# dfm/george

Hardware: NVIDIA H100
Metric: gp.compute+log_likelihood N-points/sec (higher is better)
Workload: dtype f64

## Files before the change

george_b200/_lib.py:

```python

import ctypes as C
import os

import numpy as np

from ._spec import HodlrNodeInfo, HodlrOpts, KernelSpec

_HERE = os.path.dirname(os.path.abspath(__file__))
LIB_PATH = os.path.join(_HERE, "lib", "libbgp_b200.so")

BGP_OK, BGP_ERR_INVALID, BGP_ERR_DIM, BGP_ERR_NOT_COMPUTED, BGP_ERR_LINALG = 0, 1, 2, 3, 4
BGP_ERR_CUDA, BGP_ERR_NO_DEVICE, BGP_ERR_RANK_CAPACITY, BGP_ERR_INDEX, BGP_ERR_NOMEM = 5, 6, 7, 8, 9
BGP_PREDICT_VAR, BGP_PREDICT_COV = 0, 1
BGP_SAMPLE_DMMA_ROWS = 8


class BGPError(RuntimeError):
    """CUDA / device failure inside libbgp_b200 (there is no fallback path)."""


class RankCapacityError(BGPError):
    """The ACA rank of a node exceeded the configured per-level capacity."""


_lib = None

_p = C.c_void_p
_dp = C.POINTER(C.c_double)
_i64 = C.c_int64
_i32 = C.c_int32
_specp = C.POINTER(KernelSpec)

SIGNATURES = {
    "bgp_last_error": (C.c_char_p, []),
    "bgp_version": (C.c_int, []),
    "bgp_device_count": (C.c_int, []),
    "bgp_set_device": (C.c_int, [C.c_int]),
    "bgp_launch_count": (C.c_uint64, []),
    "bgp_spec_validate": (C.c_int, [_specp]),
    "bgp_spec_num_params": (C.c_int, [_specp, C.POINTER(C.c_int)]),
    "bgp_spec_paths": (C.c_int, [_specp, C.POINTER(_i32)]),
    "bgp_kmat_symmetric": (C.c_int, [_specp, _p, _i64, _p]),
    "bgp_kmat_general": (C.c_int, [_specp, _p, _i64, _p, _i64, _p]),
    "bgp_kmat_diagonal": (C.c_int, [_specp, _p, _p, _i64, _p]),
    "bgp_kmat_gradient_symmetric": (C.c_int, [_specp, _p, _p, _i64, _p]),
    "bgp_kmat_gradient_general": (C.c_int, [_specp, _p, _p, _i64, _p, _i64, _p]),
    "bgp_kmat_x1_gradient_general": (C.c_int, [_specp, _p, _i64, _p, _i64, _p]),
    "bgp_kmat_x2_gradient_general": (C.c_int, [_specp, _p, _i64, _p, _i64, _p]),
    "bgp_kmat_symmetric_dev": (C.c_int, [_specp, _p, _i64, _p, _p, _i64]),
    "bgp_kmat_general_dev": (C.c_int, [_specp, _p, _i64, _p, _i64, _p, _i64]),
    "bgp_kmat_matvec": (C.c_int, [_specp, _p, _i64, _p, _i64, _p, _p, _i64, _p]),
    "bgp_kmat_matvec_dev": (C.c_int, [_specp, _p, _i64, _p, _i64, _p, _p, _i64, _p]),
    "bgp_kmat_gradient_contract": (C.c_int, [_specp, _p, _p, _i64, _p, _p]),
    "bgp_kmat_x1_gradient_matvec": (C.c_int, [_specp, _p, _i64, _p, _i64, _p, _i64, C.c_double, _i32, _p]),
    "bgp_kmat_x1_gradient_matvec_dev": (C.c_int, [_specp, _p, _i64, _p, _i64, _p, _i64, C.c_double, _i32, _p]),
    "bgp_dense_grad_terms": (C.c_int, [_p, _p, _p, _p, _p, _p]),
    "bgp_hodlr_grad_terms": (C.c_int, [_p, _p, _p, _p, _p, _p]),
    "bgp_hodlr_grad_terms_local_dev": (C.c_int, [_p, _p, _p, _p, _p]),
    "bgp_dense_predict": (C.c_int, [_p, _specp, _p, _i64, _i32, _p]),
    "bgp_hodlr_predict": (C.c_int, [_p, _specp, _p, _i64, _i32, _p]),
    "bgp_dense_predict_grad": (C.c_int, [_p, _specp, _p, _i64, _p, _p]),
    "bgp_hodlr_predict_grad": (C.c_int, [_p, _specp, _p, _i64, _p, _p]),
    "bgp_hodlr_predict_local_dev": (C.c_int, [_p, _specp, _p, _i64, _i32, _p, _i64, _i32, _p]),
    "bgp_mvn_sample": (C.c_int, [_p, _i64, _p, _p, _i64, C.c_double, _p]),
    "bgp_dense_sample": (C.c_int, [_p, _specp, _p, _i64, _p, _p, _i64, C.c_double, _p]),
    "bgp_hodlr_sample": (C.c_int, [_p, _specp, _p, _i64, _p, _p, _i64, C.c_double, _p]),
    "bgp_sample_last_timing": (C.c_int, [_dp]),
    "bgp_dense_batch_create": (C.c_int, [C.POINTER(_p)]),
    "bgp_dense_batch_destroy": (None, [_p]),
    "bgp_dense_batch_log_likelihood": (C.c_int, [_p, _specp, _p, _i64, _i64, _p, _i64, _i32, _p, _p, _p, _p, _p]),
    "bgp_dense_batch_predict": (C.c_int, [_p, _specp, _p, _i64, _i64, _p, _i64, _i32, _p, _p, _p, _i64, _i32, _p, _p,
                                          _p]),
    "bgp_dense_batch_sample": (C.c_int, [_p, _specp, _p, _i64, _i64, _p, _i64, _i32, _p, _p, _p, _i64, _p, _p, _i64,
                                         C.c_double, _p, _p, _p]),
    "bgp_dense_batch_grad_terms": (C.c_int, [_p, _specp, _p, _i64, _i64, _p, _i64, _i32, _p, _p, _p, _p, _p, _p, _p,
                                             _p, _p]),
    "bgp_dense_create": (C.c_int, [C.POINTER(_p)]),
    "bgp_dense_destroy": (None, [_p]),
    "bgp_dense_compute": (C.c_int, [_p, _specp, _p, _i64, _i32, _p]),
    "bgp_dense_computed": (C.c_int, [_p]),
    "bgp_dense_log_determinant": (C.c_int, [_p, _dp]),
    "bgp_dense_apply_inverse": (C.c_int, [_p, _p, _i64, _i64]),
    "bgp_dense_dot_solve": (C.c_int, [_p, _p, _dp]),
    "bgp_dense_apply_sqrt": (C.c_int, [_p, _p, _i64, _p]),
    "bgp_dense_get_inverse": (C.c_int, [_p, _p]),
    "bgp_dense_export_factor": (C.c_int, [_p, _p]),
    "bgp_dense_import_factor": (C.c_int, [_p, _p, _i64, C.c_double]),
    "bgp_dense_last_timing": (C.c_int, [_p, _dp]),
    "bgp_hodlr_default_opts": (None, [C.POINTER(HodlrOpts)]),
    "bgp_hodlr_create": (C.c_int, [C.POINTER(_p)]),
    "bgp_hodlr_destroy": (None, [_p]),
    "bgp_hodlr_compute": (C.c_int, [_p, _specp, _p, _i64, _i32, _p, C.POINTER(HodlrOpts)]),
    "bgp_hodlr_compute_dev": (C.c_int, [_p, _specp, _p, _i64, _i32, _p, C.POINTER(HodlrOpts)]),
    "bgp_hodlr_computed": (C.c_int, [_p]),
    "bgp_hodlr_log_determinant": (C.c_int, [_p, _dp]),
    "bgp_hodlr_apply_inverse": (C.c_int, [_p, _p, _i64, _i64]),
    "bgp_hodlr_dot_solve": (C.c_int, [_p, _p, _dp]),
    "bgp_hodlr_dot_solve_dev": (C.c_int, [_p, _p, _dp]),
    "bgp_hodlr_get_inverse": (C.c_int, [_p, _p]),
    "bgp_hodlr_num_nodes": (C.c_int, [_p, C.POINTER(_i64)]),
    "bgp_hodlr_node_info": (C.c_int, [_p, C.POINTER(HodlrNodeInfo)]),
    "bgp_hodlr_node_pivots": (C.c_int, [_p, _i64, _p, _p]),
    "bgp_hodlr_node_factors": (C.c_int, [_p, _i64, _p]),
    "bgp_hodlr_last_draw_paths": (C.c_int, [_p, C.POINTER(C.c_uint64)]),
    "bgp_hodlr_last_eval_units": (C.c_int, [_p, C.POINTER(C.c_uint64)]),
    "bgp_hodlr_last_timing": (C.c_int, [_p, _dp]),
    "bgp_hodlr_last_grad_timing": (C.c_int, [_p, _dp]),
    "bgp_hodlr_last_work": (C.c_int, [_p, _dp]),
    "bgp_hodlr_set_profiling": (C.c_int, [_p, C.c_int]),
    "bgp_hodlr_last_aca_profile": (C.c_int, [_p, _dp]),
    "bgp_selftest_lu": (C.c_int, [_i32, _i32, _p, _p, _p]),
    "bgp_selftest_gemm": (C.c_int, [_i32, _i32, _i32, _i32, _i32, _p, _i64, _p, _i64, _p, _i64, _i32]),
    "bgp_hodlr_top_panel": (C.c_int, [_p, C.POINTER(_p), C.POINTER(_i64), C.POINTER(_i64), C.POINTER(_i64),
                                      C.POINTER(_i64)]),
    "bgp_hodlr_export_top": (C.c_int, [_p, _p, _i64]),
    "bgp_hodlr_import_top": (C.c_int, [_p, _p, _i64]),
    "bgp_hodlr_shard_rows": (C.c_int, [_p, _i32, C.POINTER(_i64), C.POINTER(_i64)]),
    "bgp_hodlr_finish_top": (C.c_int, [_p]),
    "bgp_comm_unique_id": (C.c_int, [_p, C.c_char_p]),
    "bgp_comm_init": (C.c_int, [_p, C.c_int, C.c_int, C.c_char_p]),
    "bgp_comm_destroy": (C.c_int, []),
    "bgp_comm_size": (C.c_int, []),
    "bgp_hodlr_solve_local_dev": (C.c_int, [_p, _p, _i64, _i64]),
    "bgp_hodlr_solve_top_dev": (C.c_int, [_p, _p, _i64, _i64]),
    "bgp_dev_alloc": (C.c_int, [C.POINTER(_p), C.c_size_t]),
    "bgp_dev_free": (C.c_int, [_p]),
    "bgp_dev_upload": (C.c_int, [_p, _p, C.c_size_t]),
    "bgp_dev_download": (C.c_int, [_p, _p, C.c_size_t]),
    "bgp_dev_synchronize": (C.c_int, []),
    "bgp_host_alloc_pinned": (C.c_int, [C.POINTER(_p), C.c_size_t]),
    "bgp_host_free_pinned": (C.c_int, [_p]),
}


def load():
    global _lib
    if _lib is not None:
        return _lib
    if not os.path.exists(LIB_PATH):
        raise ImportError(
            "george_b200: the CUDA library {0} is missing. Build it with "
            "`python -c 'import __graft_entry__ as g; g.build()'` (nvcc, sm_90a). "
            "There is no CPU fallback.".format(LIB_PATH))
    lib = C.CDLL(LIB_PATH)
    for name, (res, args) in SIGNATURES.items():
        fn = getattr(lib, name)
        fn.restype = res
        fn.argtypes = args
    _lib = lib
    return lib


def last_error():
    msg = load().bgp_last_error()
    return msg.decode("utf-8", "replace") if msg else ""


def check(status):
    if status == BGP_OK:
        return
    msg = last_error()
    if status == BGP_ERR_INVALID:
        raise ValueError(msg or "invalid kernel")
    if status in (BGP_ERR_DIM, BGP_ERR_NOT_COMPUTED):
        raise RuntimeError(msg or "dimension mismatch")
    if status == BGP_ERR_LINALG:
        raise np.linalg.LinAlgError(msg or "matrix is not positive definite")
    if status == BGP_ERR_INDEX:
        raise IndexError(msg)
    if status == BGP_ERR_NOMEM:
        raise MemoryError(msg)
    if status == BGP_ERR_RANK_CAPACITY:
        raise RankCapacityError(msg)
    raise BGPError("libbgp_b200 status {0}: {1}".format(status, msg))


def ptr(a):
    return C.c_void_p(a.ctypes.data)
```

george_b200/csrc/hodlr.cu:

```cuda
#include <algorithm>
#include <cmath>
#include <cstdlib>
#include <cstring>
#include <vector>

#include "common.cuh"
#include "hodlr_kernels.cuh"
#include "hodlr_lu.cuh"
#include "hodlr_aca2.cuh"
#include "hodlr_leaf.cuh"
#include "linalg.cuh"
#include "kernel_eval.cuh"

namespace bgp {
int upload_program(const DevProgram& P, DevBuf<DevProgram>& buf, cudaStream_t s);
int kmat_grad_contract_launch(const DevProgram* dprog, int nd, int np, const unsigned* which_dev, const double* x,
                              int64_t n, const double* M, int64_t ldm, const double* alpha, double ca, double cm,
                              double* g_dev, double* diag_dev, DevBuf<double>& scratch, cudaStream_t s);
int fill_identity_launch(double* A, int64_t n, cudaStream_t s);
int64_t grad_slab_partial_size(int64_t n, int64_t c, int np);
int64_t grad_slab_tile_size(int64_t n, int np);
int kmat_grad_slab_launch(const DevProgram* dprog, int nd, int np, const unsigned* which_dev, const double* x, int64_t n,
                          const double* W, int64_t j0, int64_t nc, int64_t jlo, int64_t jhi, const double* alpha,
                          double* partial, double* tile_part, double* diag_dev, cudaStream_t s);
int kmat_grad_slab_finish(int np, int64_t jlo, int64_t jhi, const double* tile_part, double* g_dev, cudaStream_t s);
int kmat_symmetric_launch_auto(const DevProgram& P, const DevProgram* dprog, const double* x, int64_t n,
                               const double* diag_add, double* out, int64_t ld, cudaStream_t s);
int kmat_general_launch_auto(const DevProgram& P, const DevProgram* dprog, const double* x1, int64_t n1, const double* x2,
                             int64_t n2, double* out, int64_t ld, cudaStream_t s);
int kmat_diagonal_launch(const DevProgram* dprog, const double* x1, const double* x2, int64_t n, double* out,
                         cudaStream_t s, int members = 1, int64_t ostride = 0);
int64_t predict_chunk_cols(int64_t n, int64_t multiple);
int64_t predict_var_partial_size(int64_t n, int64_t c);
int predict_var_launch(const double* B, int64_t ldb, const double* W, int64_t ldw, int64_t n, int64_t c,
                       const double* kdiag, double* var, DevBuf<double>& scratch, cudaStream_t s);
int kmat_x1_grad_matvec_launch(const DevProgram& P, const DevProgram* dprog, const double* x1, int64_t n1,
                               const double* x2, int64_t n2, const double* V, int64_t ldv, double scale, int add_prior,
                               double* out, DevBuf<double>& scratch, cudaStream_t s);
void predict_gemm_plan(int64_t m, int64_t nn, int64_t K, int64_t* nsplit_out, int64_t* klen_out);
int predict_gemm_sub(const double* A, int64_t lda, const double* B, int64_t ldb, int64_t m, int64_t nn, int64_t K,
                     bool lower, double* C, int64_t ldc, DevBuf<double>& slices, DevBuf<GemmDesc>& descs, cudaStream_t s);
bool comm_ready();
int comm_rank();
int comm_world();
int comm_allreduce_sum_f64(double* buf, size_t count, cudaStream_t s);
int comm_allgather_f64(const double* send, double* recv, size_t count, cudaStream_t s);
}
using namespace bgp;

struct HNode {
  int start, size, half, is_leaf, parent, dir, depth;
  int slot;
  int rank = 0, draws = 0, fallback = 0;
  int owned = 1;
  int top = 0;
};

struct PanelSet {
  DevBuf<double> V, U;
  int64_t ld = 0, row_off = 0;
  int vcols = 0, ucols = 0;
  double* vbase() const { return V.p - row_off; }
  double* ubase() const { return U.p - row_off; }
};

struct LevelInfo {
  std::vector<int> nodes;
  int set = 1;
  int cap = 0, max_cap = 0, vcol = 0, r = 0, ucol = 0;
  int max_half = 0, grow = 0;
  int desc_off = 0;
};

struct AcaGraphKey {
  A2Args a;
  int nn, ncc, nrc, shape, grid;
};

struct bgp_hodlr {
  cudaStream_t sA = nullptr, sB = nullptr;
  cudaEvent_t ev[8] = {nullptr};
  int64_t n = 0;
  int ndim = 0;
  bgp_hodlr_opts_t opts;
  bool computed = false;
  double log_det = 0.0;
  DevProgram prog;

  std::vector<HNode> nodes;
  std::vector<int> leaves;
  std::vector<LevelInfo> levels;
  std::vector<int> piv_off;
  std::vector<int> h_piv_rows, h_piv_cols;
  int max_leaf = 0, rtot = 0, vcols = 0, cut_depth = 0;
  int64_t row0 = 0, nloc = 0;
  std::vector<int64_t> shard_row0, shard_rows;
  bool top_pending = false;

  DevBuf<DevProgram> d_prog;
  DevBuf<double> d_x, d_yerr, d_diag, d_L, d_leaf_logdet, d_node_logdet, d_S, d_W, d_scalar, d_rhs;
  PanelSet top, loc;
  const PanelSet& pset(const LevelInfo& L) const { return L.set == 0 ? top : loc; }
  DevBuf<double> d_inv, d_gscratch;
  DevBuf<double> d_xsend, d_xrecv;
  DevBuf<unsigned> d_which;
  LuWorkspace lu_ws;
  DevBuf<GemmDesc> d_gram_desc, d_upd_desc;
  std::vector<NodeDesc> h_nodes;
  std::vector<int> cap_hint;
  int64_t cap_hint_n = -1;
  int cap_hint_min_size = -1;
  DevBuf<LeafDesc> d_leaves;
  DevBuf<AcaDesc> d_aca;
  DevBuf<AcaOut> d_aca_out;
  DevBuf<NodeDesc> d_nodes;
  DevBuf<PanelTile> d_ptiles;
  int small_limit = SS_MAX_N;
  bool leaf_cols_wide = false;
  DevBuf<int> d_idx, d_piv_rows, d_piv_cols, d_ticket, d_chain_done, d_ncols_by_depth;
  DevBuf<uint32_t> d_chain_state;
  DevBuf<A2Node> d_a2nodes;
  DevBuf<A2State> d_a2states;
  DevBuf<MT19937> d_a2rngs;
  DevBuf<A2EPart> d_epart;
  DevBuf<int> d_cand, d_cand_k, d_cand_words, d_cand_L, d_cand_next, d_cand_live, d_cchunk_node, d_rchunk_node, d_nactive;
  DevBuf<double> d_node_box;
  DevBuf<double2> d_cand_xu, d_gbox, d_cbox;
  DevBuf<unsigned long long> d_cmax, d_stats;
  DevBuf<int4> d_work;
  DevBuf<int> d_work_count, d_iter;
  AcaGraphKey aca_key;
  cudaGraph_t aca_graph = nullptr;
  cudaGraphExec_t aca_exec = nullptr;
  cudaStream_t sC = nullptr;
  bool profile = false;
  std::vector<cudaEvent_t> prof_events;
  double prof[12] = {0, 0, 0, 0, 0, 0, 0, 0, 0, 0, 0, 0};
  uint64_t draw_paths[4] = {0, 0, 0, 0};
  uint64_t eval_units[2] = {0, 0};
  DevBuf<double> d_vpart, d_upart, d_vmax;
  int aca_iters = 0;
  size_t w_cap = 0;

  double t_ms[5] = {0, 0, 0, 0, 0};
  double grad_t[4] = {0, 0, 0, 0};
  double work[6] = {0, 0, 0, 0, 0, 0};
};

static int ensure_streams(bgp_hodlr* h) {
  if (!h->sA) {
    BGP_CUDA(cudaStreamCreateWithFlags(&h->sA, cudaStreamNonBlocking));
    BGP_CUDA(cudaStreamCreateWithFlags(&h->sB, cudaStreamNonBlocking));
    for (int i = 0; i < 8; ++i) BGP_CUDA(cudaEventCreate(&h->ev[i]));
  }
  return BGP_OK;
}

static void build_tree(bgp_hodlr* h, int start, int size, int dir, int parent, int depth) {
  HNode nd;
  nd.start = start; nd.size = size; nd.half = size / 2; nd.dir = dir; nd.parent = parent; nd.depth = depth;
  nd.is_leaf = !(nd.half >= h->opts.min_size);
  nd.slot = 0;
  const int id = (int)h->nodes.size();
  h->nodes.push_back(nd);
  if (!nd.is_leaf) {
    build_tree(h, start, nd.half, 0, id, depth + 1);
    build_tree(h, start + nd.half, size - nd.half, 1, id, depth + 1);
  }
}

static int hodlr_solve_dev(bgp_hodlr* h, double* b, int64_t nrhs, int64_t ldb, cudaStream_t s, int part,
                           int64_t eye_row0 = -1);
static int hodlr_exchange_finish(bgp_hodlr* h);

static bool host_exchange(const bgp_hodlr* h) {
  return h->opts.shard_count > 1 &&
         !(comm_ready() && comm_world() == h->opts.shard_count && comm_rank() == h->opts.shard_rank);
}

static int reject_host_exchange(const bgp_hodlr* h, const char* what) {
  if (!host_exchange(h)) return BGP_OK;
  set_error("%s is not available on a host-exchange shard (shard %d of %d without a matching communicator): use "
            "bgp_hodlr_solve_local_dev / bgp_hodlr_solve_top_dev", what, h->opts.shard_rank, h->opts.shard_count);
  return BGP_ERR_INVALID;
}
static int hodlr_finish_top_impl(bgp_hodlr* h, bool allreduce);

constexpr size_t LS_SMEM_MAX = 200 * 1024;
constexpr int LS_MAX_LEAF = (int)(LS_SMEM_MAX / sizeof(double));

static bool leaf_solve_fits(int max_leaf, int cols) { return sizeof(double) * (size_t)max_leaf * cols <= LS_SMEM_MAX; }

static void set_sweep_func_attrs() {
  static std::atomic<uint64_t> done{0};
  int dev = 0;
  cudaGetDevice(&dev);
  const uint64_t bit = dev < 64 ? (1ull << dev) : 0;
  if (bit && (done.load(std::memory_order_relaxed) & bit)) return;
  cudaFuncSetAttribute(leaf_solve_kernel<1>, cudaFuncAttributeMaxDynamicSharedMemorySize, (int)LS_SMEM_MAX);
  cudaFuncSetAttribute(leaf_solve_kernel<2>, cudaFuncAttributeMaxDynamicSharedMemorySize, (int)LS_SMEM_MAX);
  cudaFuncSetAttribute(leaf_solve_kernel<4>, cudaFuncAttributeMaxDynamicSharedMemorySize, (int)LS_SMEM_MAX);
  cudaFuncSetAttribute(leaf_solve_kernel<LS_COLS>, cudaFuncAttributeMaxDynamicSharedMemorySize, (int)LS_SMEM_MAX);
  cudaFuncSetAttribute(leaf_solve_kernel<LS_COLS_WIDE>, cudaFuncAttributeMaxDynamicSharedMemorySize, (int)LS_SMEM_MAX);
  cudaFuncSetAttribute(small_solve_kernel, cudaFuncAttributeMaxDynamicSharedMemorySize, 160 * 1024);
  done.fetch_or(bit, std::memory_order_relaxed);
}

template <int COLS>
static int leaf_solve_launch(bgp_hodlr* h, double* X, int64_t ldx, const int* ncols_by_depth, int ncols_fixed,
                             int max_cols, cudaStream_t s, int l0, int l1) {
  const int ngroups = (max_cols + COLS - 1) / COLS;
  const dim3 grid((unsigned)((size_t)(l1 - l0) * (size_t)ngroups));
  const size_t smem = sizeof(double) * (size_t)h->max_leaf * COLS;
  leaf_solve_kernel<COLS><<<grid, LS_THREADS, smem, s>>>(h->d_leaves.p + l0, h->d_L.p, X, ldx, ncols_by_depth,
                                                         ncols_fixed, h->max_leaf, ngroups);
  BGP_LAUNCH_CHECK();
  return BGP_OK;
}

static int launch_leaf_solve(bgp_hodlr* h, double* X, int64_t ldx, const int* ncols_by_depth, int ncols_fixed,
                             int max_cols, cudaStream_t s, int l0 = 0, int l1 = -1) {
  if (l1 < 0) l1 = (int)h->leaves.size();
  const int nl = l1 - l0;
  if (nl <= 0 || max_cols == 0) return BGP_OK;
  const int m = h->max_leaf;
  if (h->leaf_cols_wide && max_cols > LS_COLS && leaf_solve_fits(m, LS_COLS_WIDE))
    return leaf_solve_launch<LS_COLS_WIDE>(h, X, ldx, ncols_by_depth, ncols_fixed, max_cols, s, l0, l1);
  int cols = max_cols <= 1 ? 1 : max_cols <= 2 ? 2 : max_cols <= 4 ? 4 : LS_COLS;
  while (cols > 1 && !leaf_solve_fits(m, cols)) cols /= 2;
  if (!leaf_solve_fits(m, cols)) {
    set_error("leaf size %d too large for the leaf solve kernel (at most %d rows)", m, LS_MAX_LEAF);
    return BGP_ERR_INVALID;
  }
  switch (cols) {
    case LS_COLS: return leaf_solve_launch<LS_COLS>(h, X, ldx, ncols_by_depth, ncols_fixed, max_cols, s, l0, l1);
    case 4: return leaf_solve_launch<4>(h, X, ldx, ncols_by_depth, ncols_fixed, max_cols, s, l0, l1);
    case 2: return leaf_solve_launch<2>(h, X, ldx, ncols_by_depth, ncols_fixed, max_cols, s, l0, l1);
    default: return leaf_solve_launch<1>(h, X, ldx, ncols_by_depth, ncols_fixed, max_cols, s, l0, l1);
  }
}

static int launch_level_big(bgp_hodlr* h, const LevelInfo& L, double* X, int64_t ldx, int ncolsW, int own_off, int factor,
                            int col_lo, int col_hi, cudaStream_t s, int b0, int b1);

static int launch_level(bgp_hodlr* h, const LevelInfo& L, double* X, int64_t ldx, int ncolsW, int own_off, int factor,
                        int col_lo, int col_hi, cudaStream_t s, int b0 = 0, int b1 = -1) {
  if (b1 < 0) b1 = (int)L.nodes.size();
  const int nn = b1 - b0;
  if (nn <= 0 || L.r == 0) {
    return BGP_OK;
  }
  const int r = L.r;
  const int64_t stride = (int64_t)2 * r * ncolsW;
  const size_t need = (size_t)nn * stride;
  if (need > h->w_cap) { set_error("internal: W workspace too small (%zu > %zu)", need, h->w_cap); return BGP_ERR_CUDA; }
  BGP_CUDA(cudaMemsetAsync(h->d_W.p, 0, sizeof(double) * need, s));
  if (2 * r > h->small_limit) return launch_level_big(h, L, X, ldx, ncolsW, own_off, factor, col_lo, col_hi, s, b0, b1);
  const NodeDesc* nd = h->d_nodes.p + L.desc_off + b0;
  const int max_nh = L.max_half + 1;
  if (r <= GTS_MAX_R) {
    dim3 grid((max_nh + GTS_ROWS - 1) / GTS_ROWS, nn * 2, (ncolsW + GTS_TC - 1) / GTS_TC);
    const double* vb = h->pset(L).vbase();
    const int64_t ldv = h->pset(L).ld;
    if (r <= 2) gram_tn_small_kernel<2><<<grid, GTS_THREADS, 0, s>>>(nd, vb, ldv, X, ldx, ncolsW, h->d_W.p, stride);
    else if (r <= 4) gram_tn_small_kernel<4><<<grid, GTS_THREADS, 0, s>>>(nd, vb, ldv, X, ldx, ncolsW, h->d_W.p, stride);
    else gram_tn_small_kernel<GTS_MAX_R><<<grid, GTS_THREADS, 0, s>>>(nd, vb, ldv, X, ldx, ncolsW, h->d_W.p, stride);
    BGP_LAUNCH_CHECK();
  } else {
    dim3 grid((max_nh + GT_CHUNK - 1) / GT_CHUNK, nn * 2, (ncolsW + GT_TC - 1) / GT_TC);
    gram_tn_kernel<<<grid, GT_THREADS, 0, s>>>(nd, h->pset(L).vbase(), h->pset(L).ld, X, ldx, ncolsW, h->d_W.p, stride);
    BGP_LAUNCH_CHECK();
  }
  {
    const size_t sbytes = sizeof(double) * (size_t)(2 * r) * (2 * r);
    small_solve_kernel<<<nn, SS_THREADS, sbytes, s>>>(nd, h->d_W.p, stride, ncolsW, own_off, factor, h->d_S.p,
                                                      h->d_node_logdet.p, L.desc_off + b0);
    BGP_LAUNCH_CHECK();
  }
  if (col_hi > col_lo) {
    dim3 grid((max_nh + UP_ROWS - 1) / UP_ROWS, nn * 2, (col_hi - col_lo + UP_TC - 1) / UP_TC);
    update_nn_kernel<<<grid, UP_THREADS, 0, s>>>(nd, h->pset(L).ubase(), h->pset(L).ld, X, ldx, col_lo, col_hi, h->d_W.p, stride, 0);
    BGP_LAUNCH_CHECK();
  }
  return BGP_OK;
}

static int launch_level_big(bgp_hodlr* h, const LevelInfo& L, double* X, int64_t ldx, int ncolsW, int own_off, int factor,
                            int col_lo, int col_hi, cudaStream_t s, int b0, int b1) {
  const int nn = b1 - b0;
  const int r = L.r, n2 = 2 * r;
  const int64_t stride = (int64_t)n2 * ncolsW;
  const int64_t ldv = h->pset(L).ld, ldu = h->pset(L).ld;
  double* W = h->d_W.p;
  constexpr int KCHUNK = 4096;
  std::vector<LuNode> lun(nn);
  std::vector<GemmDesc> gram, upd;
  int max_nh = 0;
  for (int k = 0; k < nn; ++k) {
    const int b = b0 + k;
    const HNode& nd = h->nodes[L.nodes[b]];
    const int64_t s_off = h->h_nodes[L.desc_off + b].s_off;
    lun[k].S = h->d_S.p + s_off;
    lun[k].piv = reinterpret_cast<int*>(lun[k].S + (int64_t)n2 * n2);
    lun[k].logdet = h->d_node_logdet.p + L.desc_off + b;
    double* Wn = W + (int64_t)k * stride;
    for (int hh = 0; hh < 2; ++hh) {
      const int rs = nd.start + (hh ? nd.half : 0), nh = hh ? (nd.size - nd.half) : nd.half;
      max_nh = std::max(max_nh, nh);
      for (int k0 = 0; k0 < nh; k0 += KCHUNK) {
        GemmDesc g;
        g.A = h->pset(L).vbase() + (int64_t)L.vcol * ldv + rs + k0; g.lda = ldv;
        g.B = X + rs + k0; g.ldb = ldx;
        g.C = Wn + (hh ? 0 : r); g.ldc = n2;
        g.M = r; g.N = ncolsW; g.K = std::min(KCHUNK, nh - k0); g.mode = GD_ATOMIC_ADD;
        gram.push_back(g);
      }
      if (col_hi > col_lo) {
        GemmDesc g;
        g.A = h->pset(L).ubase() + (int64_t)L.ucol * ldu + rs; g.lda = ldu;
        g.B = Wn + (hh ? r : 0) + (int64_t)col_lo * n2; g.ldb = n2;
        g.C = X + rs + (int64_t)col_lo * ldx; g.ldc = ldx;
        g.M = nh; g.N = col_hi - col_lo; g.K = r; g.mode = GD_SUB;
        upd.push_back(g);
      }
    }
  }
  BGP_TRY(lu_upload(h->d_gram_desc, gram, s));
  BGP_TRY((gemm_dmma_launch<true, true>(h->d_gram_desc.p, (int)gram.size(), r, ncolsW, nullptr, s)));
  if (factor) {
    BGP_TRY(lu_upload(h->lu_ws.d_nodes, lun, s));
    dim3 grid((unsigned)std::min<int64_t>(((int64_t)n2 * n2 + 255) / 256, 4096), nn);
    lu_assemble_kernel<<<grid, 256, 0, s>>>(h->lu_ws.d_nodes.p, W, stride, r, own_off);
    BGP_LAUNCH_CHECK();
    BGP_TRY(lu_factor_batch(h->lu_ws, lun, n2, s));
    if (col_hi > col_lo)
      BGP_TRY(lu_solve_batch(h->lu_ws, lun, n2, W + (int64_t)col_lo * n2, stride, n2, col_hi - col_lo, false, s));
  } else {
    BGP_TRY(lu_solve_batch(h->lu_ws, lun, n2, W, stride, n2, ncolsW, true, s));
  }
  if (!upd.empty()) {
    BGP_TRY(lu_upload(h->d_upd_desc, upd, s));
    BGP_TRY((gemm_dmma_launch<false, true>(h->d_upd_desc.p, (int)upd.size(), max_nh, col_hi - col_lo, nullptr, s)));
  }
  return BGP_OK;
}

static int run_aca2(bgp_hodlr* h, const std::vector<AcaDesc>& descs, std::vector<AcaOut>& houts, cudaStream_t s) {
  const int nn = (int)descs.size();
  if (nn == 0) return BGP_OK;
  std::vector<A2Node> hn(nn);
  std::vector<int> cchunk_node, rchunk_node;
  int64_t cand_total = 0, top_cand_total = 0;
  (void)top_cand_total;
  const bool dist_top = false;
  int capmax = 1;
  for (int i = 0; i < nn; ++i) {
    const AcaDesc& d = descs[i];
    A2Node& a = hn[i];
    a.row0 = d.row0; a.n_rows = d.n_rows; a.col0 = d.col0; a.n_cols = d.n_cols;
    a.vcol = d.vcol; a.cap = d.cap; a.pre_id = d.pre_id; a.node = d.node;
    {
      const PanelSet& ps = h->pset(h->levels[h->nodes[d.pre_id].depth]);
      a.ld = ps.ld;
      a.vbase = ps.vbase() + (int64_t)d.vcol * ps.ld;
    }
    a.idx_off = d.idx_off; a.piv_off = d.piv_off;
    a.cchunk0 = (int)cchunk_node.size(); a.n_cchunks = (d.n_cols + A2_CHUNK - 1) / A2_CHUNK;
    a.rchunk0 = (int)rchunk_node.size(); a.n_rchunks = (d.n_rows + A2_CHUNK - 1) / A2_CHUNK;
    for (int c = 0; c < a.n_cchunks; ++c) cchunk_node.push_back(i);
    for (int c = 0; c < a.n_rchunks; ++c) rchunk_node.push_back(i);
    a.bmax = std::min(A2_BMAX, d.n_rows);
    a.cand_off = cand_total; cand_total += a.bmax;
    a.is_top = (dist_top && h->nodes[d.pre_id].top) ? 1 : 0;
    if (a.is_top) top_cand_total = cand_total;
    capmax = std::max(capmax, d.cap);
  }
  const int ncc = (int)cchunk_node.size(), nrc = (int)rchunk_node.size();
  BGP_TRY(h->d_a2nodes.reserve(nn, s));
  BGP_TRY(h->d_a2states.reserve(nn, s));
  BGP_TRY(h->d_a2rngs.reserve((size_t)2 * nn, s));
  BGP_TRY(h->d_cand.reserve((size_t)cand_total, s));
  BGP_TRY(h->d_cand_k.reserve((size_t)cand_total, s));
  BGP_TRY(h->d_cand_words.reserve((size_t)cand_total, s));
  BGP_TRY(h->d_cand_L.reserve((size_t)cand_total, s));
  BGP_TRY(h->d_cand_next.reserve((size_t)cand_total, s));
  BGP_TRY(h->d_cand_live.reserve((size_t)cand_total, s));
  BGP_TRY(h->d_node_box.reserve((size_t)2 * nn, s));
  BGP_TRY(h->d_cmax.reserve((size_t)cand_total, s));
  BGP_TRY(h->d_epart.reserve((size_t)std::max(ncc, 1) * A2_NSUB, s));
  BGP_TRY(h->d_cchunk_node.reserve(ncc, s));
  BGP_TRY(h->d_rchunk_node.reserve(nrc, s));
  BGP_TRY(h->d_vpart.reserve((size_t)ncc * A2_NSUB * (capmax + 1), s));
  BGP_TRY(h->d_upart.reserve((size_t)nrc * A2_NSUB * (capmax + 1), s));
  const bool cull = shape_has_bound(h->prog.shape) && !getenv("BGP_NO_CULL");
  if (cull) {
    BGP_TRY(h->d_vmax.reserve((size_t)ncc * A2_NGROUP, s));
    BGP_TRY(h->d_cand_xu.reserve((size_t)cand_total, s));
    BGP_TRY(h->d_gbox.reserve((size_t)ncc * A2_NGROUP, s));
    BGP_TRY(h->d_cbox.reserve((size_t)ncc, s));
  }
  BGP_TRY(h->d_nactive.reserve(2, s));
  int n_top = 0;
  for (int i = 0; i < nn; ++i) n_top += hn[i].is_top;
  BGP_TRY(h->d_stats.reserve(A2_NSTATS, s));
  int64_t work_cap = 0;
  for (int i = 0; i < nn; ++i) {
    const int big = (hn[i].bmax + A2_CG * A2_ITEM_CB - 1) / (A2_CG * A2_ITEM_CB);
    const int small = (std::min(hn[i].bmax, 256) + A2_CG - 1) / A2_CG;
    work_cap += (int64_t)hn[i].n_cchunks * std::max(big, small);
  }
  BGP_TRY(h->d_work.reserve((size_t)(2 * work_cap), s));
  BGP_TRY(h->d_work_count.reserve(4, s));
  BGP_TRY(h->d_iter.reserve(1, s));
  BGP_CUDA(cudaMemsetAsync(h->d_iter.p, 0, sizeof(int), s));
  BGP_CUDA(cudaMemsetAsync(h->d_work_count.p, 0, sizeof(int) * 4, s));
  BGP_CUDA(cudaMemsetAsync(h->d_stats.p, 0, sizeof(unsigned long long) * A2_NSTATS, s));
  BGP_CUDA(cudaMemcpyAsync(h->d_a2nodes.p, hn.data(), sizeof(A2Node) * nn, cudaMemcpyHostToDevice, s));
  BGP_CUDA(cudaMemcpyAsync(h->d_cchunk_node.p, cchunk_node.data(), sizeof(int) * ncc, cudaMemcpyHostToDevice, s));
  BGP_CUDA(cudaMemcpyAsync(h->d_rchunk_node.p, rchunk_node.data(), sizeof(int) * nrc, cudaMemcpyHostToDevice, s));
  BGP_CUDA(cudaMemcpyAsync(h->d_nactive.p, &nn, sizeof(int), cudaMemcpyHostToDevice, s));
  A2Args a;
  memset(&a, 0, sizeof(a));
  a.prog = h->d_prog.p; a.x = h->d_x.p; a.nodes = h->d_a2nodes.p; a.states = h->d_a2states.p; a.rngs = h->d_a2rngs.p; a.n_nodes = nn;
  a.tol = h->opts.tol; a.seed = (uint32_t)h->opts.seed; a.exhaust_mode = h->opts.exhaust_mode;
  a.idx_ws = h->d_idx.p; a.piv_rows = h->d_piv_rows.p; a.piv_cols = h->d_piv_cols.p;
  a.cand = h->d_cand.p; a.cand_k = h->d_cand_k.p; a.cand_words = h->d_cand_words.p; a.cmax = h->d_cmax.p; a.epart = h->d_epart.p;
  a.cchunk_node = h->d_cchunk_node.p; a.rchunk_node = h->d_rchunk_node.p; a.vpart = h->d_vpart.p; a.upart = h->d_upart.p;
  a.vmax = cull ? h->d_vmax.p : nullptr;
  a.cand_xu = cull ? h->d_cand_xu.p : nullptr;
  a.gbox = cull ? h->d_gbox.p : nullptr;
  a.cbox = cull ? h->d_cbox.p : nullptr;
  a.cand_L = h->d_cand_L.p; a.cand_next = h->d_cand_next.p; a.cand_live = h->d_cand_live.p; a.node_box = h->d_node_box.p;
  a.capmax = capmax; a.n_active = h->d_nactive.p; a.stats = h->d_stats.p;
  a.work = h->d_work.p; a.work_count = h->d_work_count.p; a.work_cursor = h->d_work_count.p + 2; a.work_cap = (int)work_cap; a.iter_ptr = h->d_iter.p;
  a.shard_rank = dist_top ? h->opts.shard_rank : 0; a.shard_count = dist_top ? h->opts.shard_count : 1;
  if (dist_top) BGP_CUDA(cudaMemcpyAsync(h->d_nactive.p + 1, &n_top, sizeof(int), cudaMemcpyHostToDevice, s));
  cudaFuncSetAttribute(a2_init_kernel, cudaFuncAttributeMaxDynamicSharedMemorySize, (int)sizeof(A2NodeSmem));
    cudaFuncSetAttribute(a2_decide_kernel, cudaFuncAttributeMaxDynamicSharedMemorySize, (int)sizeof(A2NodeSmem));
    cudaFuncSetAttribute(a2_finish_kernel, cudaFuncAttributeMaxDynamicSharedMemorySize, (int)sizeof(A2NodeSmem));
  a2_init_kernel<<<nn, A2_NODE_THREADS, sizeof(A2NodeSmem), s>>>(a);
  BGP_LAUNCH_CHECK();
  int active = nn, iters = 0;
  int eval_minb = A2_EVAL_MINB_DEFAULT;
  if (const char* e = getenv("BGP_EVAL_MINB")) eval_minb = atoi(e) == 3 ? 3 : 2;
  const int eval_grid = num_sms() * 6;
  auto launch_iteration = [&](cudaStream_t st, cudaGraphConditionalHandle hnd, int use_hnd, int it_prof) -> int {
    auto mark = [&](int slot) -> int {
      if (it_prof < 0) return BGP_OK;
      const size_t need = (size_t)7 * (it_prof + 1);
      while (h->prof_events.size() < need) {
        cudaEvent_t e;
        BGP_CUDA(cudaEventCreate(&e));
        h->prof_events.push_back(e);
      }
      BGP_CUDA(cudaEventRecord(h->prof_events[(size_t)7 * it_prof + slot], st));
      return BGP_OK;
    };
    BGP_TRY(mark(0));
    a2_eval_launch(h->prog.shape, dim3(eval_grid), st, a, eval_minb);
    BGP_LAUNCH_CHECK();
    BGP_TRY(mark(1));
    a2_decide_kernel<<<nn, A2_NODE_THREADS, sizeof(A2NodeSmem), st>>>(a);
    BGP_LAUNCH_CHECK();
    BGP_TRY(mark(2));
    a2_vrow_launch(h->prog.shape, dim3(ncc, A2_NSUB), st, a);
    BGP_LAUNCH_CHECK();
    BGP_TRY(mark(3));
    a2_pivot_kernel<<<nn, 32, 0, st>>>(a);
    BGP_LAUNCH_CHECK();
    BGP_TRY(mark(4));
    a2_vnorm_ucol_launch(h->prog.shape, dim3(ncc + nrc, A2_NSUB), st, a, ncc);
    BGP_LAUNCH_CHECK();
    BGP_TRY(mark(5));
    a2_finish_kernel<<<nn, A2_NODE_THREADS, sizeof(A2NodeSmem), st>>>(a);
    BGP_LAUNCH_CHECK();
    BGP_TRY(mark(6));
    a2_tick_kernel<<<1, 1, 0, st>>>(a.iter_ptr, a.n_active, hnd, use_hnd);
    BGP_LAUNCH_CHECK();
    return BGP_OK;
  };
  const bool use_graph = !h->profile && !getenv("BGP_NO_GRAPH");
  if (use_graph) {
    AcaGraphKey key;
    memset(&key, 0, sizeof(key));
    key.a = a; key.nn = nn; key.ncc = ncc; key.nrc = nrc; key.shape = h->prog.shape; key.grid = eval_grid * 4 + eval_minb;
    if (!h->aca_exec || memcmp(&key, &h->aca_key, sizeof(key)) != 0) {
      if (h->aca_exec) { cudaGraphExecDestroy(h->aca_exec); h->aca_exec = nullptr; }
      if (h->aca_graph) { cudaGraphDestroy(h->aca_graph); h->aca_graph = nullptr; }
      BGP_CUDA(cudaGraphCreate(&h->aca_graph, 0));
      cudaGraphConditionalHandle hnd;
      BGP_CUDA(cudaGraphConditionalHandleCreate(&hnd, h->aca_graph, 1, cudaGraphCondAssignDefault));
      cudaGraphNodeParams cp = {};
      cp.type = cudaGraphNodeTypeConditional;
      cp.conditional.handle = hnd;
      cp.conditional.type = cudaGraphCondTypeWhile;
      cp.conditional.size = 1;
      cudaGraphNode_t wnode;
      BGP_CUDA(cudaGraphAddNode(&wnode, h->aca_graph, nullptr, 0, &cp));
      cudaGraph_t body = cp.conditional.phGraph_out[0];
      if (!h->sC) BGP_CUDA(cudaStreamCreateWithFlags(&h->sC, cudaStreamNonBlocking));
      BGP_CUDA(cudaStreamBeginCaptureToGraph(h->sC, body, nullptr, nullptr, 0, cudaStreamCaptureModeRelaxed));
      const int rc = launch_iteration(h->sC, hnd, 1, -1);
      cudaGraph_t captured = nullptr;
      const cudaError_t ce = cudaStreamEndCapture(h->sC, &captured);
      if (rc != BGP_OK) return rc;
      if (ce != cudaSuccess) { set_error("ACA graph capture failed: %s", cudaGetErrorString(ce)); return BGP_ERR_CUDA; }
      BGP_CUDA(cudaGraphInstantiate(&h->aca_exec, h->aca_graph, 0));
      h->aca_key = key;
    }
    BGP_CUDA(cudaGraphLaunch(h->aca_exec, s));
    int it_host = 0, act2[2] = {0, 0};
    BGP_CUDA(cudaMemcpyAsync(&it_host, h->d_iter.p, sizeof(int), cudaMemcpyDeviceToHost, s));
    BGP_CUDA(cudaMemcpyAsync(act2, h->d_nactive.p, sizeof(int) * 2, cudaMemcpyDeviceToHost, s));
    BGP_CUDA(cudaStreamSynchronize(s));
    iters = it_host;
    g_launches.fetch_add((uint64_t)7 * (uint64_t)std::max(iters - 1, 0), std::memory_order_relaxed);
    if (act2[0] > 0) { set_error("ACA did not terminate"); return BGP_ERR_CUDA; }
  } else {
    while (active > 0) {
      for (int rep = 0; rep < 8; ++rep) {
        BGP_TRY(launch_iteration(s, 0, 0, h->profile ? iters : -1));
        iters++;
      }
      int act2[2] = {0, 0};
      BGP_CUDA(cudaMemcpyAsync(act2, h->d_nactive.p, sizeof(int) * 2, cudaMemcpyDeviceToHost, s));
      BGP_CUDA(cudaStreamSynchronize(s));
      active = act2[0];
      if (iters > (1 << 22)) { set_error("ACA did not terminate"); return BGP_ERR_CUDA; }
    }
  }
  h->aca_iters = iters;
  {
    unsigned long long st4[A2_NSTATS] = {0};
    BGP_CUDA(cudaMemcpyAsync(st4, h->d_stats.p, sizeof(st4), cudaMemcpyDeviceToHost, s));
    BGP_CUDA(cudaStreamSynchronize(s));
    for (int k = 0; k < 4; ++k) h->draw_paths[k] = st4[A2_PATH_REDO + k];
    h->eval_units[0] = st4[A2_UNITS_PULLED]; h->eval_units[1] = st4[A2_UNITS_LIVE];
    h->prof[1] = iters; h->prof[2] = (double)st4[0]; h->prof[3] = (double)st4[1]; h->prof[4] = (double)st4[2];
    h->prof[5] = (double)st4[3];
    if (h->profile) {
      double tot[6] = {0, 0, 0, 0, 0, 0};
      for (int i = 0; i < iters; ++i)
        for (int k = 0; k < 6; ++k) {
          float ms = 0;
          cudaEventElapsedTime(&ms, h->prof_events[(size_t)7 * i + k], h->prof_events[(size_t)7 * i + k + 1]);
          tot[k] += ms;
        }
      h->prof[0] = tot[0];
      for (int k = 0; k < 6; ++k) h->prof[6 + k] = tot[k];
    }
  }
  if (h->opts.exhaust_mode == BGP_EXHAUST_DENSE) {
    a2_dense_fill_kernel<<<dim3(nn, 64), 256, 0, s>>>(a);
    BGP_LAUNCH_CHECK();
    a2_dense_rank_kernel<<<(nn + 127) / 128, 128, 0, s>>>(a);
    BGP_LAUNCH_CHECK();
  }
  std::vector<A2State> hs(nn);
  BGP_CUDA(cudaMemcpyAsync(hs.data(), h->d_a2states.p, sizeof(A2State) * nn, cudaMemcpyDeviceToHost, s));
  BGP_CUDA(cudaStreamSynchronize(s));
  for (int i = 0; i < nn; ++i) {
    AcaOut o;
    o.rank = hs[i].rank; o.draws = hs[i].draws; o.fallback = hs[i].fallback; o.status = hs[i].status;
    houts[descs[i].node] = o;
  }
  return BGP_OK;
}

static int hodlr_compute_dev_impl(bgp_hodlr* h, const bgp_kernel_spec_t* spec, const double* x_dev, int64_t n,
                                  int32_t ndim, const double* yerr_dev, const bgp_hodlr_opts_t* opts_in) {
  h->computed = false;
  h->top_pending = false;
  for (uint64_t& c : h->draw_paths) c = 0;
  for (uint64_t& c : h->eval_units) c = 0;
  h->shard_row0.clear(); h->shard_rows.clear();
  BGP_TRY(require_device());
  BGP_TRY(ensure_streams(h));
  BGP_TRY(build_dev_program(spec, &h->prog));
  if (h->prog.ndim != ndim) { set_error("dimension mismatch: kernel ndim %d, input ndim %d", h->prog.ndim, ndim); return BGP_ERR_DIM; }
  if (ndim > ACA_MAX_NDIM) { set_error("HODLR supports at most %d input dimensions", ACA_MAX_NDIM); return BGP_ERR_INVALID; }
  if (n <= 0 || n > (int64_t)0x7fffffff) { set_error("invalid number of points %lld", (long long)n); return BGP_ERR_INVALID; }
  bgp_hodlr_opts_t o;
  if (opts_in) o = *opts_in; else bgp_hodlr_default_opts(&o);
  if (o.min_size < 1) { set_error("min_size must be >= 1"); return BGP_ERR_INVALID; }
  if (o.shard_count < 1) o.shard_count = 1;
  if (o.shard_count & (o.shard_count - 1)) { set_error("shard_count must be a power of two"); return BGP_ERR_INVALID; }
  if (o.shard_rank < 0 || o.shard_rank >= o.shard_count) { set_error("invalid shard_rank"); return BGP_ERR_INVALID; }
  if (o.shard_count > 1 && o.rng_mode == BGP_RNG_REFERENCE) { set_error("rng_mode=reference serialises the tree and cannot be sharded"); return BGP_ERR_INVALID; }
  h->opts = o;
  h->n = n;
  h->ndim = ndim;
  cudaStream_t sA = h->sA, sB = h->sB;
  set_sweep_func_attrs();
  h->small_limit = SS_MAX_N;
  if (const char* e = getenv("BGP_SMALL_RANK_LIMIT")) h->small_limit = std::min(SS_MAX_N, atoi(e));
  h->leaf_cols_wide = false;
  if (const char* e = getenv("BGP_LEAF_COLS")) h->leaf_cols_wide = atoi(e) > LS_COLS;

  h->nodes.clear(); h->leaves.clear(); h->levels.clear();
  h->nodes.reserve(2 * (size_t)(n / std::max(1, o.min_size)) + 8);
  build_tree(h, 0, (int)n, 0, -1, 0);
  int cut = 0;
  while ((1 << cut) < o.shard_count) cut++;
  h->cut_depth = cut;
  int max_depth = 0;
  for (auto& nd : h->nodes) max_depth = std::max(max_depth, nd.depth);
  h->row0 = 0; h->nloc = n;
  if (o.shard_count > 1) {
    int seen = 0; bool found = false;
    for (size_t i = 0; i < h->nodes.size(); ++i) {
      HNode& nd = h->nodes[i];
      if (nd.depth == cut) {
        if (seen == o.shard_rank) { h->row0 = nd.start; h->nloc = nd.size; found = true; }
        h->shard_row0.push_back(nd.start); h->shard_rows.push_back(nd.size);
        seen++;
      }
    }
    if (!found || seen != o.shard_count) {
      h->shard_row0.clear(); h->shard_rows.clear();
      set_error("tree too shallow to shard %d ways (N=%lld, min_size=%d)", o.shard_count, (long long)n, o.min_size);
      return BGP_ERR_INVALID;
    }
    for (auto& nd : h->nodes) {
      nd.top = nd.depth < cut;
      nd.owned = !nd.top && nd.start >= h->row0 && nd.start + nd.size <= h->row0 + h->nloc;
    }
  }
  h->levels.assign(max_depth + 1, LevelInfo());
  for (size_t i = 0; i < h->nodes.size(); ++i) {
    HNode& nd = h->nodes[i];
    if (nd.is_leaf) { if (nd.owned) { nd.slot = (int)h->leaves.size(); h->leaves.push_back((int)i); } continue; }
    if (!(nd.owned || nd.top)) continue;
    LevelInfo& L = h->levels[nd.depth];
    nd.slot = (int)L.nodes.size();
    L.nodes.push_back((int)i);
    L.max_half = std::max(L.max_half, nd.size - nd.half);
  }
  while (!h->levels.empty() && h->levels.back().nodes.empty()) h->levels.pop_back();
  const int nlev = (int)h->levels.size();
  for (int l = 0; l < nlev; ++l) h->levels[l].set = (o.shard_count > 1 && l < cut) ? 0 : 1;
  h->top.ld = n; h->top.row_off = 0;
  h->loc.ld = h->nloc; h->loc.row_off = h->row0;

  const int rcap0 = o.rank_capacity > 0 ? o.rank_capacity : 128;
  for (auto& L : h->levels) {
    int mh = 0;
    for (int id : L.nodes) mh = std::max(mh, h->nodes[id].half);
    L.max_cap = std::max(1, mh);
    L.cap = std::min(rcap0, L.max_cap);
  }
  if (o.rank_capacity <= 0 && h->cap_hint_n == n && h->cap_hint_min_size == o.min_size && (int)h->cap_hint.size() == nlev)
    for (int l = 0; l < nlev; ++l) h->levels[l].cap = std::min(h->levels[l].max_cap, std::max(h->levels[l].cap, h->cap_hint[l]));

  BGP_TRY(upload_program(h->prog, h->d_prog, sA));
  BGP_TRY(h->d_x.reserve((size_t)n * ndim, sA));
  BGP_TRY(h->d_diag.reserve((size_t)n, sA));
  if (x_dev != h->d_x.p) BGP_CUDA(cudaMemcpyAsync(h->d_x.p, x_dev, sizeof(double) * n * ndim, cudaMemcpyDeviceToDevice, sA));
  square_kernel<<<(unsigned)std::min<int64_t>((n + 255) / 256, 1184), 256, 0, sA>>>(yerr_dev, h->d_diag.p, n);
  BGP_LAUNCH_CHECK();
  BGP_CUDA(cudaEventRecord(h->ev[0], sA));

  const int nl = (int)h->leaves.size();
  std::vector<LeafDesc> hleaves(nl);
  int64_t loff = 0;
  h->max_leaf = 0;
  for (int i = 0; i < nl; ++i) {
    const HNode& nd = h->nodes[h->leaves[i]];
    hleaves[i].start = nd.start; hleaves[i].size = nd.size; hleaves[i].depth = nd.depth; hleaves[i]._pad = 0;
    hleaves[i].off = loff;
    loff += (int64_t)nd.size * nd.size;
    h->max_leaf = std::max(h->max_leaf, nd.size);
  }
  if (h->max_leaf > LS_MAX_LEAF) {
    set_error("leaf size %d too large: the leaf solve handles at most %d rows (N=%lld, min_size=%d); lower min_size",
              h->max_leaf, LS_MAX_LEAF, (long long)n, o.min_size);
    return BGP_ERR_INVALID;
  }
  BGP_TRY(h->d_leaves.reserve(std::max(nl, 1), sA));
  BGP_TRY(h->d_L.reserve((size_t)std::max<int64_t>(loff, 1), sA));
  BGP_TRY(h->d_leaf_logdet.reserve(std::max(nl, 1), sA));
  if (nl) {
    BGP_CUDA(cudaMemcpyAsync(h->d_leaves.p, hleaves.data(), sizeof(LeafDesc) * nl, cudaMemcpyHostToDevice, sA));
    const char* lf_env = getenv("BGP_LEAF_FACTOR");
    const bool generic = lf_env && strcmp(lf_env, "generic") == 0;
    if (h->max_leaf <= LF_MAX_LEAF && !generic) {
      leaf_factor_launch(h->prog.shape, nl, h->max_leaf, sA, h->d_prog.p, h->d_x.p, h->d_diag.p, h->d_leaves.p, h->d_L.p,
                         h->d_leaf_logdet.p);
    } else {
      leaf_build_factor_kernel<<<nl, LEAF_THREADS, 0, sA>>>(h->d_prog.p, h->d_x.p, h->d_diag.p, h->d_leaves.p, h->d_L.p,
                                                            h->d_leaf_logdet.p);
    }
    BGP_LAUNCH_CHECK();
  }
  BGP_CUDA(cudaEventRecord(h->ev[1], sA));

  std::vector<AcaDesc> hdesc;
  std::vector<int> desc_node;
  std::vector<AcaOut> houts;
  int64_t idx_total = 0, piv_total = 0;
  int nint = 0;
  BGP_CUDA(cudaStreamWaitEvent(sB, h->ev[1], 0));
  for (int attempt = 0;; ++attempt) {
// ... 239 lines not shown
}

template <class StartSize>
static void rows_meeting(int count, const StartSize& start_size, int64_t lo, int64_t hi, int* first, int* last) {
  int a = 0, b = count;
  while (a < b) {
    const int m = (a + b) / 2;
    int st, sz;
    start_size(m, &st, &sz);
    if ((int64_t)st + sz <= lo) a = m + 1; else b = m;
  }
  *first = a;
  b = count;
  while (a < b) {
    const int m = (a + b) / 2;
    int st, sz;
    start_size(m, &st, &sz);
    if (st < hi) a = m + 1; else b = m;
  }
  *last = a;
}

static bool rows_ordered(const bgp_hodlr* h) {
  auto ordered = [&](const std::vector<int>& ids) {
    for (size_t k = 1; k < ids.size(); ++k) {
      const HNode& a = h->nodes[ids[k - 1]];
      if (a.start + a.size > h->nodes[ids[k]].start) return false;
    }
    return true;
  };
  if (!ordered(h->leaves)) return false;
  for (const LevelInfo& L : h->levels)
    if (!ordered(L.nodes)) return false;
  return true;
}

static int hodlr_solve_dev(bgp_hodlr* h, double* b, int64_t nrhs, int64_t ldb, cudaStream_t s, int part,
                           int64_t eye_row0) {
  const int nlev = (int)h->levels.size();
  const int cut = h->opts.shard_count > 1 ? h->cut_depth : 0;
  const bool native_x = part == 0 && h->opts.shard_count > 1 && !host_exchange(h);
  if (eye_row0 >= 0 && part != 0) {
    set_error("internal: a row-restricted solve runs every part of the solve");
    return BGP_ERR_INVALID;
  }
  for (int64_t c0 = 0; c0 < nrhs; c0 += 64) {
    const int nc = (int)std::min<int64_t>(64, nrhs - c0);
    double* X = b + c0 * ldb;
    if (eye_row0 >= 0) {
      const int64_t lo = std::max(eye_row0 + c0, h->row0), hi = std::min(eye_row0 + c0 + nc, h->row0 + h->nloc);
      if (lo >= hi) continue;
      int l0, l1;
      rows_meeting((int)h->leaves.size(), [&](int k, int* st, int* sz) {
        const HNode& nd = h->nodes[h->leaves[k]]; *st = nd.start; *sz = nd.size; }, lo, hi, &l0, &l1);
      BGP_TRY(launch_leaf_solve(h, X, ldb, nullptr, nc, nc, s, l0, l1));
      for (int l = nlev - 1; l >= 0; --l) {
        const LevelInfo& L = h->levels[l];
        int b0, b1;
        rows_meeting((int)L.nodes.size(), [&](int k, int* st, int* sz) {
          const HNode& nd = h->nodes[L.nodes[k]]; *st = nd.start; *sz = nd.size; }, lo, hi, &b0, &b1);
        BGP_TRY(launch_level(h, L, X, ldb, nc, 0, 0, 0, nc, s, b0, b1));
      }
      continue;
    }
    if (part != 2) {
      BGP_TRY(launch_leaf_solve(h, X, ldb, nullptr, nc, nc, s));
      for (int l = nlev - 1; l >= cut; --l) BGP_TRY(launch_level(h, h->levels[l], X, ldb, nc, 0, 0, 0, nc, s));
    }
    if (native_x) BGP_TRY(exchange_rows(h, X, ldb, nc, s));
    if (part != 1) {
      for (int l = std::min(cut, nlev) - 1; l >= 0; --l) BGP_TRY(launch_level(h, h->levels[l], X, ldb, nc, 0, 0, 0, nc, s));
    }
  }
  return BGP_OK;
}

static int64_t top_cols(const bgp_hodlr_t* h) {
  const int cut = std::min<int>(h->cut_depth, (int)h->levels.size());
  (void)cut;
  return h->top.ucols;
}

static int hodlr_finish_top_impl(bgp_hodlr* h, bool allreduce) {
  cudaStream_t s = h->sA;
  const int nlev = (int)h->levels.size();
  const int cut = std::min(h->cut_depth, nlev);
  for (int l = cut - 1; l >= 0; --l) {
    const LevelInfo& L = h->levels[l];
    BGP_TRY(launch_level(h, L, h->top.U.p, h->n, L.ucol + L.r, L.ucol, 1, 0, L.ucol, s));
  }
  const int nl = (int)h->leaves.size();
  int ndesc = 0;
  for (auto& L : h->levels) ndesc += (int)L.nodes.size();
  std::vector<double> ld_leaf(nl), ld_node(ndesc);
  if (nl) BGP_CUDA(cudaMemcpyAsync(ld_leaf.data(), h->d_leaf_logdet.p, sizeof(double) * nl, cudaMemcpyDeviceToHost, s));
  if (ndesc) BGP_CUDA(cudaMemcpyAsync(ld_node.data(), h->d_node_logdet.p, sizeof(double) * ndesc, cudaMemcpyDeviceToHost, s));
  BGP_CUDA(cudaStreamSynchronize(s));
  double ld = 0.0;
  for (double v : ld_leaf) ld += v;
  for (int l = 0; l < nlev; ++l) {
    const LevelInfo& L = h->levels[l];
    if (l < cut && h->opts.shard_rank != 0) continue;
    for (size_t i = 0; i < L.nodes.size(); ++i) ld += ld_node[L.desc_off + i];
  }
  if (allreduce) {
    BGP_CUDA(cudaMemcpyAsync(h->d_scalar.p, &ld, sizeof(double), cudaMemcpyHostToDevice, s));
    BGP_TRY(comm_allreduce_sum_f64(h->d_scalar.p, 1, s));
    BGP_CUDA(cudaMemcpyAsync(&ld, h->d_scalar.p, sizeof(double), cudaMemcpyDeviceToHost, s));
    BGP_CUDA(cudaStreamSynchronize(s));
  }
  h->log_det = ld;
  h->computed = true;
  return BGP_OK;
}

static int hodlr_exchange_finish(bgp_hodlr* h) {
  BGP_TRY(exchange_rows(h, h->top.U.p, h->n, top_cols(h), h->sA));
  BGP_TRY(hodlr_finish_top_impl(h, true));
  float ms = 0;
  cudaEventElapsedTime(&ms, h->ev[0], h->ev[1]); h->t_ms[0] = ms;
  cudaEventElapsedTime(&ms, h->ev[0], h->ev[2]); h->t_ms[1] = ms;
  cudaEventElapsedTime(&ms, h->ev[6], h->ev[3]); h->t_ms[2] = ms;
  cudaEventElapsedTime(&ms, h->ev[0], h->ev[3]); h->t_ms[3] = ms;
  return BGP_OK;
}

extern "C" {

void bgp_hodlr_default_opts(bgp_hodlr_opts_t* o) {
  o->min_size = 100; o->seed = 42; o->tol = 0.1;
  o->rng_mode = BGP_RNG_REFERENCE;
  o->rank_capacity = 0; o->shard_rank = 0; o->shard_count = 1; o->exhaust_mode = BGP_EXHAUST_DENSE;
}

int bgp_hodlr_create(bgp_hodlr_t** out) {
  *out = new (std::nothrow) bgp_hodlr();
  if (!*out) { set_error("out of host memory"); return BGP_ERR_NOMEM; }
  bgp_hodlr_default_opts(&(*out)->opts);
  return BGP_OK;
}

void bgp_hodlr_destroy(bgp_hodlr_t* h) {
  if (!h) return;
  if (h->sA) {
    cudaStreamSynchronize(h->sA); cudaStreamSynchronize(h->sB);
  }
  h->d_prog.release(); h->d_x.release(); h->d_yerr.release(); h->d_diag.release(); h->d_L.release();
  h->d_leaf_logdet.release(); h->d_node_logdet.release(); h->top.V.release(); h->top.U.release(); h->loc.V.release(); h->loc.U.release(); h->d_S.release();
  h->d_W.release(); h->d_scalar.release(); h->d_rhs.release(); h->d_leaves.release(); h->d_aca.release();
  h->d_aca_out.release(); h->d_nodes.release(); h->d_ptiles.release(); h->d_idx.release(); h->d_piv_rows.release(); h->d_piv_cols.release();
  h->lu_ws.d_nodes.release(); h->lu_ws.d_trsm.release(); h->lu_ws.d_gemm.release(); h->d_gram_desc.release(); h->d_upd_desc.release();
  h->d_ticket.release(); h->d_chain_done.release(); h->d_ncols_by_depth.release(); h->d_chain_state.release();
  h->d_a2nodes.release(); h->d_a2states.release(); h->d_a2rngs.release(); h->d_epart.release(); h->d_cand.release(); h->d_cand_k.release();
  h->d_cand_words.release(); h->d_cand_L.release(); h->d_cand_next.release(); h->d_cand_live.release(); h->d_node_box.release(); h->d_cand_xu.release(); h->d_gbox.release(); h->d_cbox.release(); h->d_cchunk_node.release(); h->d_rchunk_node.release(); h->d_nactive.release();
  h->d_inv.release(); h->d_gscratch.release(); h->d_which.release(); h->d_xsend.release(); h->d_xrecv.release();
  h->d_vpart.release(); h->d_upart.release(); h->d_vmax.release(); h->d_cmax.release(); h->d_stats.release(); h->d_work.release(); h->d_work_count.release();
  for (cudaEvent_t e : h->prof_events) cudaEventDestroy(e);
  h->d_iter.release();
  if (h->aca_exec) cudaGraphExecDestroy(h->aca_exec);
  if (h->aca_graph) cudaGraphDestroy(h->aca_graph);
  if (h->sC) cudaStreamDestroy(h->sC);
  if (h->sA) {
    cudaStreamSynchronize(h->sA); cudaStreamSynchronize(h->sB);
    for (int i = 0; i < 8; ++i) cudaEventDestroy(h->ev[i]);
    cudaStreamDestroy(h->sA); cudaStreamDestroy(h->sB);
  }
  delete h;
}

int bgp_hodlr_compute_dev(bgp_hodlr_t* h, const bgp_kernel_spec_t* spec, const double* x_dev, int64_t n, int32_t ndim,
                          const double* yerr_dev, const bgp_hodlr_opts_t* opts) {
  if (!h) { set_error("null handle"); return BGP_ERR_INVALID; }
  return hodlr_compute_dev_impl(h, spec, x_dev, n, ndim, yerr_dev, opts);
}

int bgp_hodlr_compute(bgp_hodlr_t* h, const bgp_kernel_spec_t* spec, const double* x, int64_t n, int32_t ndim,
                      const double* yerr, const bgp_hodlr_opts_t* opts) {
  if (!h) { set_error("null handle"); return BGP_ERR_INVALID; }
  h->computed = false;
  h->top_pending = false;
  h->shard_row0.clear(); h->shard_rows.clear();
  BGP_TRY(require_device());
  BGP_TRY(ensure_streams(h));
  if (n <= 0 || ndim <= 0) { set_error("invalid input shape (%lld, %d)", (long long)n, ndim); return BGP_ERR_INVALID; }
  BGP_TRY(h->d_x.reserve((size_t)n * ndim, h->sA));
  BGP_TRY(h->d_yerr.reserve((size_t)n, h->sA));
  BGP_CUDA(cudaMemcpyAsync(h->d_x.p, x, sizeof(double) * n * ndim, cudaMemcpyHostToDevice, h->sA));
  BGP_CUDA(cudaMemcpyAsync(h->d_yerr.p, yerr, sizeof(double) * n, cudaMemcpyHostToDevice, h->sA));
  return hodlr_compute_dev_impl(h, spec, h->d_x.p, n, ndim, h->d_yerr.p, opts);
}

int bgp_hodlr_computed(const bgp_hodlr_t* h) { return h && h->computed ? 1 : 0; }

int bgp_hodlr_log_determinant(const bgp_hodlr_t* h, double* out) {
  if (!h || !h->computed) { set_error("the solver has not been computed"); return BGP_ERR_NOT_COMPUTED; }
  *out = h->log_det;
  return BGP_OK;
}

int bgp_hodlr_apply_inverse(bgp_hodlr_t* h, double* b, int64_t nrhs, int64_t ldb) {
  if (!h || !h->computed) { set_error("the solver has not been computed"); return BGP_ERR_NOT_COMPUTED; }
  BGP_TRY(reject_host_exchange(h, "apply_inverse"));
  if (nrhs <= 0) return BGP_OK;
  if (ldb < h->n) { set_error("dimension mismatch: ldb < n"); return BGP_ERR_DIM; }
  cudaStream_t s = h->sA;
  const int64_t n = h->n;
  const int64_t slab = std::max<int64_t>(1, std::min<int64_t>(nrhs, (int64_t)(1ull << 28) / n));
  BGP_TRY(h->d_rhs.reserve((size_t)n * slab, s));
  for (int64_t c0 = 0; c0 < nrhs; c0 += slab) {
    const int64_t nc = std::min(slab, nrhs - c0);
    BGP_CUDA(cudaMemcpy2DAsync(h->d_rhs.p, sizeof(double) * n, b + c0 * ldb, sizeof(double) * ldb, sizeof(double) * n, nc, cudaMemcpyHostToDevice, s));
    BGP_CUDA(cudaEventRecord(h->ev[4], s));
    BGP_TRY(hodlr_solve_dev(h, h->d_rhs.p, nc, n, s, 0));
    BGP_CUDA(cudaEventRecord(h->ev[5], s));
    BGP_CUDA(cudaMemcpy2DAsync(b + c0 * ldb, sizeof(double) * ldb, h->d_rhs.p, sizeof(double) * n, sizeof(double) * n, nc, cudaMemcpyDeviceToHost, s));
    BGP_CUDA(cudaStreamSynchronize(s));
  }
  float ms = 0; cudaEventElapsedTime(&ms, h->ev[4], h->ev[5]); h->t_ms[4] = ms;
  return BGP_OK;
}

int bgp_hodlr_dot_solve_dev(bgp_hodlr_t* h, const double* y_dev, double* out) {
  if (!h || !h->computed) { set_error("the solver has not been computed"); return BGP_ERR_NOT_COMPUTED; }
  BGP_TRY(reject_host_exchange(h, "dot_solve"));
  cudaStream_t s = h->sA;
  const int64_t n = h->n;
  BGP_TRY(h->d_rhs.reserve((size_t)n, s));
  BGP_CUDA(cudaEventRecord(h->ev[4], s));
  BGP_CUDA(cudaMemcpyAsync(h->d_rhs.p, y_dev, sizeof(double) * n, cudaMemcpyDeviceToDevice, s));
  BGP_TRY(hodlr_solve_dev(h, h->d_rhs.p, 1, n, s, 0));
  BGP_CUDA(cudaMemsetAsync(h->d_scalar.p, 0, sizeof(double), s));
  dot_kernel<<<(unsigned)std::min<int64_t>((n + 255) / 256, 592), 256, 0, s>>>(y_dev, h->d_rhs.p, n, h->d_scalar.p);
  BGP_LAUNCH_CHECK();
  BGP_CUDA(cudaEventRecord(h->ev[5], s));
  BGP_CUDA(cudaMemcpyAsync(out, h->d_scalar.p, sizeof(double), cudaMemcpyDeviceToHost, s));
  BGP_CUDA(cudaStreamSynchronize(s));
  float ms = 0; cudaEventElapsedTime(&ms, h->ev[4], h->ev[5]); h->t_ms[4] = ms;
  return BGP_OK;
}

int bgp_hodlr_dot_solve(bgp_hodlr_t* h, const double* y, double* out) {
  if (!h || !h->computed) { set_error("the solver has not been computed"); return BGP_ERR_NOT_COMPUTED; }
  BGP_TRY(reject_host_exchange(h, "dot_solve"));
  cudaStream_t s = h->sA;
  BGP_TRY(h->d_yerr.reserve((size_t)h->n, s));
  BGP_CUDA(cudaMemcpyAsync(h->d_yerr.p, y, sizeof(double) * h->n, cudaMemcpyHostToDevice, s));
  return bgp_hodlr_dot_solve_dev(h, h->d_yerr.p, out);
}

int bgp_hodlr_get_inverse(bgp_hodlr_t* h, double* out) {
  if (!h || !h->computed) { set_error("the solver has not been computed"); return BGP_ERR_NOT_COMPUTED; }
  BGP_TRY(reject_host_exchange(h, "get_inverse"));
  const int64_t n = h->n;
  for (int64_t j = 0; j < n; ++j) {
    double* c = out + j * n;
    memset(c, 0, sizeof(double) * n);
    c[j] = 1.0;
  }
  return bgp_hodlr_apply_inverse(h, out, n, n);
}

__global__ void eye_slab_kernel(double* __restrict__ W, int64_t n, int64_t j0, int64_t nc, int64_t jlo, int64_t jhi) {
  for (int64_t k = (int64_t)blockIdx.x * blockDim.x + threadIdx.x; k < nc; k += (int64_t)gridDim.x * blockDim.x)
    if (j0 + k >= jlo && j0 + k < jhi) W[k * n + j0 + k] = 1.0;
}

constexpr int64_t GRAD_RESIDENT_MAX = (int64_t)1 << 32;
constexpr int64_t GRAD_SLAB_BUDGET = (int64_t)1 << 27;

static int64_t grad_slab_cols(int64_t n, bool* forced) {
  int64_t c = std::max<int64_t>(64, (GRAD_SLAB_BUDGET / std::max<int64_t>(n, 1)) / 64 * 64);
  *forced = false;
  if (const char* e = getenv("BGP_GRAD_CHUNK")) {
    const long v = atol(e);
    if (v >= 1) { c = (v + 63) / 64 * 64; *forced = true; }
  }
  return std::min(c, (n + 63) / 64 * 64);
}

static float event_ms(cudaEvent_t a, cudaEvent_t b) {
  float ms = 0;
  cudaEventElapsedTime(&ms, a, b);
  return ms;
}

static int grad_stream_own_columns(bgp_hodlr* h, int np, const double* alpha, int64_t c, double* dg, double* ddiag,
                                   double* t_solve, double* t_contract) {
  cudaStream_t s = h->sA;
  const int64_t n = h->n, jlo = h->row0, jhi = h->row0 + h->nloc;
  const bool prof = h->profile;
  const int64_t tsize = grad_slab_tile_size(n, np), psize = grad_slab_partial_size(n, c, np);
  BGP_TRY(h->d_inv.reserve((size_t)n * c, s));
  BGP_TRY(h->d_gscratch.reserve((size_t)(tsize + psize), s));
  double* W = h->d_inv.p;
  double* tile_part = h->d_gscratch.p;
  double* partial = h->d_gscratch.p + tsize;
  int64_t slabs = 0;
  for (int64_t j0 = jlo / 64 * 64; j0 < jhi; j0 += c, ++slabs) {
    const int64_t nc = std::min(c, jhi - j0);
    if (prof) BGP_CUDA(cudaEventRecord(h->ev[4], s));
    BGP_CUDA(cudaMemsetAsync(W, 0, sizeof(double) * n * nc, s));
    eye_slab_kernel<<<(unsigned)std::min<int64_t>((nc + 255) / 256, 1184), 256, 0, s>>>(W, n, j0, nc, jlo, jhi);
    BGP_LAUNCH_CHECK();
    BGP_TRY(hodlr_solve_dev(h, W, nc, n, s, 0, j0));
    if (prof) BGP_CUDA(cudaEventRecord(h->ev[5], s));
    BGP_TRY(kmat_grad_slab_launch(h->d_prog.p, h->ndim, np, h->d_which.p, h->d_x.p, n, W, j0, nc, jlo, jhi, alpha,
                                  partial, tile_part, ddiag, s));
    if (prof) {
      BGP_CUDA(cudaEventRecord(h->ev[7], s));
// ... 276 lines not shown
    for (int64_t j0 = 0; j0 < ns; j0 += c) {
      const int64_t nc = std::min(c, ns - j0);
      BGP_CUDA(cudaMemcpyAsync(dxs.p, xs + j0 * nd, sizeof(double) * nc * nd, cudaMemcpyHostToDevice, s));
      BGP_TRY(kmat_general_launch_auto(P, dprog.p, dxs.p, nc, h->d_x.p, n, dB.p, n, s));
      BGP_CUDA(cudaMemcpyAsync(dW.p, dB.p, sizeof(double) * n * nc, cudaMemcpyDeviceToDevice, s));
      BGP_TRY(hodlr_solve_dev(h, dW.p, nc, n, s, 0));
      BGP_TRY(kmat_diagonal_launch(dprog.p, dxs.p, dxs.p, nc, dkd.p, s));
      BGP_TRY(predict_var_launch(dB.p, n, dW.p, n, n, nc, dkd.p, dvar.p, scratch, s));
      BGP_CUDA(cudaMemcpyAsync(out + j0, dvar.p, sizeof(double) * nc, cudaMemcpyDeviceToHost, s));
    }
  } else {
    BGP_TRY(hodlr_predict_cov_dev(h, P, xs, ns, dC));
    BGP_CUDA(cudaMemcpyAsync(out, dC.p, sizeof(double) * ns * ns, cudaMemcpyDeviceToHost, s));
  }
  BGP_CUDA(cudaStreamSynchronize(s));
  return BGP_OK;
}

int bgp_hodlr_predict_grad(bgp_hodlr_t* h, const bgp_kernel_spec_t* spec, const double* xs, int64_t ns, double* var,
                           double* dvar) {
  if (!h || !h->computed) { set_error("the solver has not been computed"); return BGP_ERR_NOT_COMPUTED; }
  if (host_exchange(h) || h->opts.shard_count > 1) { set_error("predict_grad is not available on a sharded factorisation"); return BGP_ERR_INVALID; }
  if (ns < 0) { set_error("negative number of test points"); return BGP_ERR_INVALID; }
  DevProgram P;
  BGP_TRY(build_dev_program(spec, &P));
  if (P.ndim != h->ndim) { set_error("dimension mismatch: kernel ndim %d, input ndim %d", P.ndim, h->ndim); return BGP_ERR_DIM; }
  if (P.ndim > BGP_MAX_DIM) { set_error("input-coordinate gradients support at most %d dimensions (got %d)", BGP_MAX_DIM, P.ndim); return BGP_ERR_INVALID; }
  if (ns == 0) return BGP_OK;
  const int64_t n = h->n;
  const int nd = h->ndim;
  cudaStream_t s = h->sA;
  DevBuf<DevProgram> dprog;
  DevBuf<double> dxs, dB, dW, dkd, dvar_c, ddvar, scratch;
  BGP_TRY(upload_program(P, dprog, s));
  const int64_t c = std::min(ns, predict_chunk_cols(n, 64));
  BGP_TRY(dW.alloc((size_t)n * c, s));
  BGP_TRY(dxs.alloc((size_t)c * nd, s));
  BGP_TRY(dB.alloc((size_t)n * c, s));
  BGP_TRY(dkd.alloc((size_t)c, s));
  BGP_TRY(dvar_c.alloc((size_t)c, s));
  BGP_TRY(ddvar.alloc((size_t)c * nd, s));
  for (int64_t j0 = 0; j0 < ns; j0 += c) {
    const int64_t nc = std::min(c, ns - j0);
    BGP_CUDA(cudaMemcpyAsync(dxs.p, xs + j0 * nd, sizeof(double) * nc * nd, cudaMemcpyHostToDevice, s));
    BGP_TRY(kmat_general_launch_auto(P, dprog.p, dxs.p, nc, h->d_x.p, n, dB.p, n, s));
    BGP_CUDA(cudaMemcpyAsync(dW.p, dB.p, sizeof(double) * n * nc, cudaMemcpyDeviceToDevice, s));
    BGP_TRY(hodlr_solve_dev(h, dW.p, nc, n, s, 0));
    BGP_TRY(kmat_diagonal_launch(dprog.p, dxs.p, dxs.p, nc, dkd.p, s));
    BGP_TRY(predict_var_launch(dB.p, n, dW.p, n, n, nc, dkd.p, dvar_c.p, scratch, s));
    BGP_CUDA(cudaMemcpyAsync(var + j0, dvar_c.p, sizeof(double) * nc, cudaMemcpyDeviceToHost, s));
    BGP_TRY(kmat_x1_grad_matvec_launch(P, dprog.p, dxs.p, nc, h->d_x.p, n, dW.p, n, -2.0, 1, ddvar.p, scratch, s));
    BGP_CUDA(cudaMemcpyAsync(dvar + j0 * nd, ddvar.p, sizeof(double) * nc * nd, cudaMemcpyDeviceToHost, s));
  }
  BGP_CUDA(cudaStreamSynchronize(s));
  return BGP_OK;
}

int bgp_hodlr_sample(bgp_hodlr_t* h, const bgp_kernel_spec_t* spec, const double* xs, int64_t ns, const double* mean,
                     const double* z, int64_t size, double jitter, double* out) {
  if (!h || !h->computed) { set_error("the solver has not been computed"); return BGP_ERR_NOT_COMPUTED; }
  if (h->opts.shard_count > 1) { set_error("sample is not available on a sharded factorisation"); return BGP_ERR_INVALID; }
  BGP_TRY(mvn_sample_check(ns, size, jitter));
  DevProgram P;
  BGP_TRY(build_dev_program(spec, &P));
  if (P.ndim != h->ndim) { set_error("dimension mismatch: kernel ndim %d, input ndim %d", P.ndim, h->ndim); return BGP_ERR_DIM; }
  if (ns == 0 || size == 0) return BGP_OK;
  DevBuf<double> dC;
  BGP_TRY(sample_mark(0, h->sA));
  BGP_TRY(hodlr_predict_cov_dev(h, P, xs, ns, dC));
  return mvn_draw_host_io(dC.p, ns, mean, z, size, jitter, out, h->sA);
}

int bgp_hodlr_num_nodes(const bgp_hodlr_t* h, int64_t* out) {
  if (!h) { set_error("null handle"); return BGP_ERR_INVALID; }
  *out = (int64_t)h->nodes.size();
  return BGP_OK;
}

int bgp_hodlr_node_info(const bgp_hodlr_t* h, bgp_hodlr_node_info_t* out) {
  if (!h) { set_error("null handle"); return BGP_ERR_INVALID; }
  for (size_t i = 0; i < h->nodes.size(); ++i) {
    const HNode& nd = h->nodes[i];
    out[i].start = nd.start; out[i].size = nd.size; out[i].half = nd.half; out[i].is_leaf = nd.is_leaf;
    out[i].parent = nd.parent; out[i].direction = nd.dir; out[i].depth = nd.depth; out[i].rank = nd.rank;
    out[i].rng_draws = nd.draws; out[i].dense_fallback = nd.fallback;
  }
  return BGP_OK;
}

int bgp_hodlr_node_pivots(const bgp_hodlr_t* hc, int64_t node, int32_t* rows, int32_t* cols) {
  bgp_hodlr_t* h = const_cast<bgp_hodlr_t*>(hc);
  if (!h || node < 0 || node >= (int64_t)h->nodes.size()) { set_error("node index out of range"); return BGP_ERR_INDEX; }
  const HNode& nd = h->nodes[node];
  if (nd.is_leaf || h->piv_off[node] < 0 || nd.rank == 0 ||
      (nd.fallback && h->opts.exhaust_mode == BGP_EXHAUST_DENSE))
    return BGP_OK;
  BGP_CUDA(cudaMemcpy(rows, h->d_piv_rows.p + h->piv_off[node], sizeof(int) * nd.rank, cudaMemcpyDeviceToHost));
  BGP_CUDA(cudaMemcpy(cols, h->d_piv_cols.p + h->piv_off[node], sizeof(int) * nd.rank, cudaMemcpyDeviceToHost));
  return BGP_OK;
}

int bgp_hodlr_node_factors(const bgp_hodlr_t* h, int64_t node, double* out) {
  if (!h) { set_error("null handle"); return BGP_ERR_INVALID; }
  if (!h->computed) { set_error("the solver has not been computed"); return BGP_ERR_NOT_COMPUTED; }
  if (h->opts.shard_count > 1) { set_error("node factors are not available on a sharded factorisation"); return BGP_ERR_INVALID; }
  if (node < 0 || node >= (int64_t)h->nodes.size() || h->nodes[node].is_leaf) {
    set_error("node %lld is not an internal node", (long long)node);
    return BGP_ERR_INDEX;
  }
  const HNode& nd = h->nodes[node];
  if (nd.rank == 0) return BGP_OK;
  const LevelInfo& L = h->levels[nd.depth];
  const PanelSet& ps = h->pset(L);
  const double* src = ps.vbase() + (int64_t)L.vcol * ps.ld + nd.start;
  BGP_CUDA(cudaMemcpy2D(out, sizeof(double) * nd.size, src, sizeof(double) * ps.ld, sizeof(double) * nd.size, nd.rank,
                        cudaMemcpyDeviceToHost));
  return BGP_OK;
}

int bgp_hodlr_last_draw_paths(const bgp_hodlr_t* h, uint64_t* out4) {
  if (!h) { set_error("null handle"); return BGP_ERR_INVALID; }
  if (!h->computed) { set_error("the solver has not been computed"); return BGP_ERR_NOT_COMPUTED; }
  for (int i = 0; i < 4; ++i) out4[i] = h->draw_paths[i];
  return BGP_OK;
}

int bgp_hodlr_last_eval_units(const bgp_hodlr_t* h, uint64_t* out2) {
  if (!h) { set_error("null handle"); return BGP_ERR_INVALID; }
  if (!h->computed) { set_error("the solver has not been computed"); return BGP_ERR_NOT_COMPUTED; }
  for (int i = 0; i < 2; ++i) out2[i] = h->eval_units[i];
  return BGP_OK;
}

int bgp_hodlr_last_timing(const bgp_hodlr_t* h, double* ms5) {
  if (!h) { set_error("null handle"); return BGP_ERR_INVALID; }
  for (int i = 0; i < 5; ++i) ms5[i] = h->t_ms[i];
  return BGP_OK;
}
int bgp_hodlr_last_grad_timing(const bgp_hodlr_t* h, double* out4) {
  if (!h) { set_error("null handle"); return BGP_ERR_INVALID; }
  for (int i = 0; i < 4; ++i) out4[i] = h->grad_t[i];
  return BGP_OK;
}
int bgp_hodlr_set_profiling(bgp_hodlr_t* h, int on) {
  if (!h) { set_error("null handle"); return BGP_ERR_INVALID; }
  h->profile = on != 0;
  return BGP_OK;
}
int bgp_hodlr_last_aca_profile(const bgp_hodlr_t* h, double* p12) {
  if (!h) { set_error("null handle"); return BGP_ERR_INVALID; }
  for (int i = 0; i < 12; ++i) p12[i] = h->prof[i];
  return BGP_OK;
}
int bgp_hodlr_last_work(const bgp_hodlr_t* h, double* w6) {
  if (!h) { set_error("null handle"); return BGP_ERR_INVALID; }
  for (int i = 0; i < 6; ++i) w6[i] = h->work[i];
  return BGP_OK;
}

int bgp_selftest_lu(int32_t n, int32_t nrhs, const double* S_host, double* R_host, double* logdet) {
  BGP_TRY(require_device());
  if (n <= 0 || nrhs < 0) { set_error("bgp_selftest_lu: bad sizes"); return BGP_ERR_INVALID; }
  cudaStream_t s = 0;
  DevBuf<double> dS, dR, dld;
  LuWorkspace ws;
  BGP_TRY(dS.alloc((size_t)n * n + n, s));
  BGP_TRY(dR.alloc(std::max<size_t>((size_t)n * nrhs, 1), s));
  BGP_TRY(dld.alloc(1, s));
  BGP_CUDA(cudaMemcpyAsync(dS.p, S_host, sizeof(double) * n * n, cudaMemcpyHostToDevice, s));
  if (nrhs) BGP_CUDA(cudaMemcpyAsync(dR.p, R_host, sizeof(double) * n * nrhs, cudaMemcpyHostToDevice, s));
  std::vector<LuNode> nodes(1);
  nodes[0].S = dS.p; nodes[0].piv = reinterpret_cast<int*>(dS.p + (size_t)n * n); nodes[0].logdet = dld.p;
  BGP_TRY(lu_factor_batch(ws, nodes, n, s));
  BGP_TRY(lu_solve_batch(ws, nodes, n, dR.p, 0, n, nrhs, false, s));
  if (nrhs) BGP_CUDA(cudaMemcpyAsync(R_host, dR.p, sizeof(double) * n * nrhs, cudaMemcpyDeviceToHost, s));
  BGP_CUDA(cudaMemcpyAsync(logdet, dld.p, sizeof(double), cudaMemcpyDeviceToHost, s));
  BGP_CUDA(cudaStreamSynchronize(s));
  return BGP_OK;
}

int bgp_selftest_gemm(int32_t a_kcontig, int32_t b_kcontig, int32_t m, int32_t n, int32_t k, const double* A_host,
                      int64_t lda, const double* B_host, int64_t ldb, double* C_host, int64_t ldc, int32_t mode) {
  BGP_TRY(require_device());
  if (m <= 0 || n <= 0 || k <= 0) { set_error("bgp_selftest_gemm: bad sizes"); return BGP_ERR_INVALID; }
  if (mode & ~(GD_ATOMIC_ADD | GD_LOWER)) { set_error("bgp_selftest_gemm: bad mode %d", mode); return BGP_ERR_INVALID; }
  if (a_kcontig && !b_kcontig) { set_error("bgp_selftest_gemm: the (A K-contiguous) x (B N-contiguous) variant is not built"); return BGP_ERR_INVALID; }
  cudaStream_t s = 0;
  const size_t na = (size_t)(a_kcontig ? m : k) * lda, nb = (size_t)(b_kcontig ? n : k) * ldb, nc = (size_t)n * ldc;
  DevBuf<double> dA, dB, dC;
  DevBuf<GemmDesc> dd;
  BGP_TRY(dA.alloc(na, s)); BGP_TRY(dB.alloc(nb, s)); BGP_TRY(dC.alloc(nc, s)); BGP_TRY(dd.alloc(1, s));
  BGP_CUDA(cudaMemcpyAsync(dA.p, A_host, sizeof(double) * na, cudaMemcpyHostToDevice, s));
  BGP_CUDA(cudaMemcpyAsync(dB.p, B_host, sizeof(double) * nb, cudaMemcpyHostToDevice, s));
  BGP_CUDA(cudaMemcpyAsync(dC.p, C_host, sizeof(double) * nc, cudaMemcpyHostToDevice, s));
  GemmDesc g;
  g.A = dA.p; g.B = dB.p; g.C = dC.p; g.M = m; g.N = n; g.K = k; g.mode = mode;
  g.lda = lda; g.ldb = ldb; g.ldc = ldc;
  BGP_CUDA(cudaMemcpyAsync(dd.p, &g, sizeof(g), cudaMemcpyHostToDevice, s));
  if (a_kcontig) BGP_TRY((gemm_dmma_launch<true, true>(dd.p, 1, m, n, nullptr, s)));
  else if (b_kcontig) BGP_TRY((gemm_dmma_launch<false, true>(dd.p, 1, m, n, nullptr, s)));
  else BGP_TRY((gemm_dmma_launch<false, false>(dd.p, 1, m, n, nullptr, s)));
  BGP_CUDA(cudaMemcpyAsync(C_host, dC.p, sizeof(double) * nc, cudaMemcpyDeviceToHost, s));
  BGP_CUDA(cudaStreamSynchronize(s));
  return BGP_OK;
}

int bgp_hodlr_top_panel(bgp_hodlr_t* h, double** ptr_dev, int64_t* row0, int64_t* rows, int64_t* cols, int64_t* ld) {
  if (!h) { set_error("null handle"); return BGP_ERR_INVALID; }
  const int cut = std::min<int>(h->cut_depth, (int)h->levels.size());
  *ptr_dev = h->top.U.p;
  *row0 = h->row0; *rows = h->nloc;
  (void)cut;
  *cols = h->top.ucols;
  *ld = h->n;
  return BGP_OK;
}


int bgp_hodlr_shard_rows(const bgp_hodlr_t* h, int32_t s, int64_t* row0, int64_t* rows) {
  if (!h || s < 0 || s >= (int)h->shard_rows.size()) { set_error("shard index out of range"); return BGP_ERR_INDEX; }
  *row0 = h->shard_row0[s]; *rows = h->shard_rows[s];
  return BGP_OK;
}

static int require_top_pending(const bgp_hodlr* h, const char* what) {
  if (h->top_pending) return BGP_OK;
  if (!h->computed) {
    set_error("%s: no sharded factorisation is waiting for its top levels (the solver has not been computed)", what);
    return BGP_ERR_NOT_COMPUTED;
  }
  set_error("%s: the factorisation is complete (unsharded, or finish_top was already called)", what);
  return BGP_ERR_INVALID;
}

int bgp_hodlr_export_top(bgp_hodlr_t* h, double* buf_dev, int64_t rows_pad) {
  if (!h) { set_error("null handle"); return BGP_ERR_INVALID; }
  BGP_TRY(require_top_pending(h, "export_top"));
  if (rows_pad < h->nloc) {
    set_error("rows_pad %lld smaller than this shard (%lld rows)", (long long)rows_pad, (long long)h->nloc);
    return BGP_ERR_INVALID;
  }
  const int64_t cols = top_cols(h);
  if (cols == 0 || h->nloc == 0) return BGP_OK;
  pack_rows_kernel<<<1184, 256, 0, h->sA>>>(h->top.U.p, h->n, h->row0, h->nloc, cols, buf_dev, rows_pad);
  BGP_LAUNCH_CHECK();
  BGP_CUDA(cudaStreamSynchronize(h->sA));
  return BGP_OK;
}

int bgp_hodlr_import_top(bgp_hodlr_t* h, const double* all_buf_dev, int64_t rows_pad) {
  if (!h) { set_error("null handle"); return BGP_ERR_INVALID; }
  BGP_TRY(require_top_pending(h, "import_top"));
  int64_t max_rows = 0;
  for (int64_t r : h->shard_rows) max_rows = std::max(max_rows, r);
  if (rows_pad < max_rows) {
    set_error("rows_pad %lld smaller than the largest shard (%lld rows)", (long long)rows_pad, (long long)max_rows);
    return BGP_ERR_INVALID;
  }
  const int64_t cols = top_cols(h);
  if (cols == 0) return BGP_OK;
  for (size_t s = 0; s < h->shard_rows.size(); ++s) {
    if ((int)s == h->opts.shard_rank) continue;
    unpack_rows_kernel<<<1184, 256, 0, h->sA>>>(h->top.U.p, h->n, h->shard_row0[s], h->shard_rows[s], cols,
                                                all_buf_dev + (int64_t)s * cols * rows_pad, rows_pad);
    BGP_LAUNCH_CHECK();
  }
  BGP_CUDA(cudaStreamSynchronize(h->sA));
  return BGP_OK;
}

int bgp_hodlr_finish_top(bgp_hodlr_t* h) {
  if (!h) { set_error("null handle"); return BGP_ERR_INVALID; }
  BGP_TRY(require_top_pending(h, "finish_top"));
  h->top_pending = false;
  return hodlr_finish_top_impl(h, false);
}

int bgp_hodlr_solve_local_dev(bgp_hodlr_t* h, double* b_dev, int64_t nrhs, int64_t ldb) {
  if (!h || !h->computed) { set_error("the solver has not been computed"); return BGP_ERR_NOT_COMPUTED; }
  BGP_TRY(hodlr_solve_dev(h, b_dev, nrhs, ldb, h->sA, 1));
  BGP_CUDA(cudaStreamSynchronize(h->sA));
  return BGP_OK;
}
int bgp_hodlr_solve_top_dev(bgp_hodlr_t* h, double* b_dev, int64_t nrhs, int64_t ldb) {
  if (!h || !h->computed) { set_error("the solver has not been computed"); return BGP_ERR_NOT_COMPUTED; }
  BGP_TRY(hodlr_solve_dev(h, b_dev, nrhs, ldb, h->sA, 2));
  BGP_CUDA(cudaStreamSynchronize(h->sA));
  return BGP_OK;
}

}
```

george_b200/csrc/hodlr_aca2.cuh:

```cuda
#pragma once

#include "hodlr_kernels.cuh"

namespace bgp {

constexpr int A2_CHUNK = 1024;
constexpr int A2_THREADS = 256;
constexpr int A2_NODE_THREADS = 1024;
constexpr int A2_EPT = A2_CHUNK / A2_THREADS;
constexpr int A2_CG = 4;
constexpr int A2_ITEM_CB = 8;
constexpr int A2_BMAX = 8192;
constexpr int A2_EVAL_MINB_DEFAULT = 3;
constexpr int A2_BGROW = 8;
constexpr int A2_NSUB = 4;
constexpr int A2_GROUP = A2_CHUNK / (A2_THREADS / 32);
constexpr int A2_NGROUP = A2_CHUNK / A2_GROUP;
static_assert(A2_NSUB * A2_THREADS == A2_CHUNK, "sub-chunks tile a chunk");
constexpr int A2_HASH = 16384;
static_assert(A2_BMAX <= 65536, "multimap values are 16-bit draw numbers");
constexpr int A2_XWORDS = 64;
constexpr int A2_PUB_BLOCKS = A2_BMAX / (A2_CG * A2_ITEM_CB);
static_assert(256 / A2_CG <= A2_PUB_BLOCKS, "blocks of A2_CG candidates (batches of up to 256 live ones) fit too");

struct A2Node {
  int row0, n_rows, col0, n_cols;
  int vcol, cap, pre_id, node;
  int cchunk0, n_cchunks, rchunk0, n_rchunks;
  int bmax, is_top;
  int64_t idx_off, piv_off, cand_off;
  double* vbase;
  int64_t ld;
};

struct A2State {
  int rank, draws, n_index, fallback, status, active;
  int phase;
  int B, ncand, piv_i, piv_j;
  int end_words;
  int deferred;
  double pivot, norm;
};

struct A2EPart {
  double val;
  int idx;
  int _pad;
};

enum { A2_SELECT = 0, A2_ACCEPT = 1, A2_DONE = 2, A2_LATE_REJECT = 3 };

__device__ __forceinline__ void mt_copy(MT19937* dst, const MT19937* src) {
  const uint32_t* s = reinterpret_cast<const uint32_t*>(src);
  uint32_t* d = reinterpret_cast<uint32_t*>(dst);
  for (int i = threadIdx.x; i < (int)(sizeof(MT19937) / 4); i += blockDim.x) d[i] = s[i];
}

__device__ __forceinline__ void mt_twist_coop(MT19937& g) {
  auto value = [&](uint32_t a, uint32_t b, uint32_t m) {
    const uint32_t y = (a & 0x80000000u) | (b & 0x7fffffffu);
    return m ^ (y >> 1) ^ ((y & 1u) ? 0x9908b0dfu : 0u);
  };
  auto phase = [&](int lo, int hi, int moff) {
    for (int base = lo; base < hi; base += blockDim.x) {
      const int i = base + threadIdx.x;
      uint32_t v = 0;
      if (i < hi) v = value(g.mt[i], g.mt[i + 1], g.mt[i + moff]);
      __syncthreads();
      if (i < hi) g.mt[i] = v;
      __syncthreads();
    }
  };
  phase(0, 227, 397);
  phase(227, 454, -227);
  phase(454, 623, -227);
  if (threadIdx.x == 0) { g.mt[623] = value(g.mt[623], g.mt[0], g.mt[396]); g.idx = 0; }
  __syncthreads();
}
__device__ __forceinline__ uint32_t mt_temper(uint32_t y) {
  y ^= (y >> 11);
  y ^= (y << 7) & 0x9d2c5680u;
  y ^= (y << 15) & 0xefc60000u;
  y ^= (y >> 18);
  return y;
}
__device__ inline void mt_fill_coop(MT19937& g, uint32_t* out, int n) {
  int done = 0;
  __syncthreads();
  while (done < n) {
    if (g.idx >= 624) mt_twist_coop(g);
    const int idx = g.idx;
    const int take = min(n - done, 624 - idx);
    for (int t = threadIdx.x; t < take; t += blockDim.x) out[done + t] = mt_temper(g.mt[idx + t]);
    __syncthreads();
    if (threadIdx.x == 0) g.idx = idx + take;
    __syncthreads();
    done += take;
  }
}
__device__ inline void mt_skip_coop(MT19937& g, int n) {
  __syncthreads();
  while (n > 0) {
    if (g.idx >= 624) mt_twist_coop(g);
    const int idx = g.idx;
    const int take = min(n, 624 - idx);
    __syncthreads();
    if (threadIdx.x == 0) g.idx = idx + take;
    __syncthreads();
    n -= take;
  }
}

struct A2Args {
  const DevProgram* prog;
  const double* x;
  const A2Node* nodes;
  A2State* states;
  MT19937* rngs;
  int n_nodes;
  double tol;
  uint32_t seed;
  int exhaust_mode;
  int* idx_ws;
  int* piv_rows;
  int* piv_cols;
  int* cand;
  int* cand_k;
  int* cand_words;
  int* cand_L;
  int* cand_next;
  int* cand_live;
  double* node_box;
  unsigned long long* cmax;
  A2EPart* epart;
  const int* cchunk_node;
  const int* rchunk_node;
  double* vpart;
  double* upart;
  double* vmax;
  double2* cand_xu;
  double2* gbox;
  double2* cbox;
  int capmax;
  int* n_active;
  int4* work;
  int* work_count;
  int* work_cursor;
  int work_cap;
  int* iter_ptr;
  int shard_rank, shard_count;
  unsigned long long* stats;
};
enum {
  A2_PATH_REDO = 4,
  A2_PATH_TRUNCATED = 5,
  A2_PATH_SEQUENTIAL = 6,
  A2_PATH_PARTIAL = 7,
  A2_UNITS_PULLED = 8,
  A2_UNITS_LIVE = 9,
  A2_NSTATS = 10
};

struct A2NodeSmem {
  MT19937 rng;
  int k[A2_BMAX];
  int ol[A2_BMAX];
  int hkey[A2_HASH];
  unsigned short hval[A2_HASH];
  uint32_t raw[A2_BMAX + A2_XWORDS];
  double red[32];
  int redi[32];
  int flag;
  int n_live;
  int extra;
};
static_assert(sizeof(int) * A2_HASH >= sizeof(double) * (3 * A2_PUB_BLOCKS + 1), "a2_generate's per-block ranges fit in hkey");

__device__ __forceinline__ unsigned a2_hash(int pos) { return ((unsigned)pos * 2654435761u) & (A2_HASH - 1); }
__device__ __forceinline__ int a2_prev_writer(const A2NodeSmem& S, int pos, int c) {
  int best = -1;
  unsigned h = a2_hash(pos);
  while (true) {
    const int key = S.hkey[h];
    if (key == -1) break;
    if (key == pos) { const int v = S.hval[h]; if (v < c && v > best) best = v; }
    h = (h + 1) & (A2_HASH - 1);
  }
  return best;
}
__device__ __forceinline__ int a2_next_writer(const A2NodeSmem& S, int pos, int c) {
  int best = 0x7fffffff;
  unsigned h = a2_hash(pos);
  while (true) {
    const int key = S.hkey[h];
    if (key == -1) break;
    if (key == pos) { const int v = S.hval[h]; if (v > c && v < best) best = v; }
    h = (h + 1) & (A2_HASH - 1);
  }
  return best;
}

__device__ __forceinline__ double program_bound(const DevProgram* g, double gap, double far) {
  switch (g->shape) {
    case BGP_SHAPE_EXPSQ: return ScaledProfile1D<BGP_SHAPE_EXPSQ>(*g).bound(gap, far);
    case BGP_SHAPE_M32: return ScaledProfile1D<BGP_SHAPE_M32>(*g).bound(gap, far);
    case BGP_SHAPE_M52: return ScaledProfile1D<BGP_SHAPE_M52>(*g).bound(gap, far);
    case BGP_SHAPE_EXP: return ScaledProfile1D<BGP_SHAPE_EXP>(*g).bound(gap, far);
    case BGP_SHAPE_PROD_EXPSQ_ES2: return ScaledProfile1D<BGP_SHAPE_PROD_EXPSQ_ES2>(*g).bound(gap, far);
    case BGP_SHAPE_PROD_M32_ES2: return ScaledProfile1D<BGP_SHAPE_PROD_M32_ES2>(*g).bound(gap, far);
    default: return __longlong_as_double(0x7ff0000000000000ll);
  }
}

__device__ __forceinline__ int a2_block_scan(int v, int* s_warp, int& total) {
  const int lane = threadIdx.x & 31, warp = threadIdx.x >> 5, nw = blockDim.x >> 5;
  int inc = v;
#pragma unroll
  for (int o = 1; o < 32; o <<= 1) {
    const int t = __shfl_up_sync(0xffffffffu, inc, o);
    if (lane >= o) inc += t;
  }
  __syncthreads();
  if (lane == 31) s_warp[warp] = inc;
  __syncthreads();
  int before = 0;
  total = 0;
  for (int w = 0; w < nw; ++w) {
    const int t = s_warp[w];
    before += (w < warp) ? t : 0;
    total += t;
  }
  return before + inc - v;
}

__device__ inline void a2_generate(const A2Args& a, A2State& st, A2NodeSmem& S, const A2Node& nd, int nid, int nb) {
  int* __restrict__ index = a.idx_ws + nd.idx_off;
  int* __restrict__ cand = a.cand + nd.cand_off;
  int* __restrict__ cand_k = a.cand_k + nd.cand_off;
  int* __restrict__ words = a.cand_words + nd.cand_off;
  int* __restrict__ cand_L = a.cand_L + nd.cand_off;
  int* __restrict__ cand_next = a.cand_next + nd.cand_off;
  int* __restrict__ live = a.cand_live + nd.cand_off;
  unsigned long long* __restrict__ cmax = a.cmax + nd.cand_off;
  const int n_index = st.n_index;
  int B = min(min(st.B, nd.bmax), n_index);
  MT19937* rng_commit = a.rngs + 2 * (int64_t)nid;
  MT19937* rng_end = rng_commit + 1;
  if (threadIdx.x == 0) { S.flag = 0x7fffffff; S.n_live = 0; S.extra = 0; }
  mt_fill_coop(S.rng, S.raw, B);
  int start = 0;
  bool truncated = false;
  while (true) {
    const int extra = S.extra;
    for (int c = start + threadIdx.x; c < B; c += blockDim.x) {
      const uint32_t srange = (uint32_t)(n_index - c);
      const uint64_t prod = (uint64_t)S.raw[c + extra] * (uint64_t)srange;
      const uint32_t low = (uint32_t)prod;
      if (low < srange && low < (0u - srange) % srange) atomicMin(&S.flag, c);
      S.k[c] = (int)(prod >> 32);
      words[c] = c + 1 + extra;
      cmax[c] = 0ull;
    }
    __syncthreads();
    const int c0 = S.flag;
    if (c0 == 0x7fffffff) break;
    __syncthreads();
    if (threadIdx.x == 0) {
      atomicAdd(a.stats + A2_PATH_REDO, 1ull);
      const uint32_t srange = (uint32_t)(n_index - c0);
      const uint32_t thr = (0u - srange) % srange;
      int e = extra;
      int kk = -1;
      while (e + 1 < A2_XWORDS && c0 + e + 1 < B + extra) {
        ++e;
        const uint64_t prod = (uint64_t)S.raw[c0 + e] * (uint64_t)srange;
        if ((uint32_t)prod >= thr) { kk = (int)(prod >> 32); break; }
      }
      if (kk >= 0) { S.k[c0] = kk; words[c0] = c0 + 1 + e; S.extra = e; S.flag = 0x7fffffff; }
      else S.flag = -1 - c0;
    }
    __syncthreads();
    if (S.flag < 0) {
      const int c0t = -1 - S.flag;
      __syncthreads();
      if (c0t > 0) {
        if (threadIdx.x == 0) atomicAdd(a.stats + A2_PATH_TRUNCATED, 1ull);
        B = c0t; truncated = true; break;
      }
      mt_copy(&S.rng, rng_commit);
      __syncthreads();
      if (threadIdx.x == 0) {
        atomicAdd(a.stats + A2_PATH_SEQUENTIAL, 1ull);
        int w = 0; S.k[0] = mt_uniform(S.rng, (uint32_t)n_index, &w); words[0] = w; cmax[0] = 0ull; S.extra = -1;
      }
      __syncthreads();
      B = 1;
      break;
    }
    {
      const int grown = S.extra - extra;
      mt_fill_coop(S.rng, S.raw + B + extra, grown);
    }
    start = c0 + 1;
  }
  __syncthreads();
  mt_copy(rng_end, &S.rng);
  if (threadIdx.x == 0) {
    st.ncand = B;
    st.end_words = (!truncated && S.extra >= 0 && B > 0 && words[B - 1] == B + S.extra) ? B + S.extra : -1;
  }
  for (int t = threadIdx.x; t < A2_HASH; t += blockDim.x) S.hkey[t] = -1;
  __syncthreads();
  for (int c = threadIdx.x; c < B; c += blockDim.x) {
    const int pos = S.k[c];
    S.ol[c] = index[n_index - 1 - c];
    unsigned h = a2_hash(pos);
    while (atomicCAS(&S.hkey[h], -1, pos) != -1) h = (h + 1) & (A2_HASH - 1);
    S.hval[h] = (unsigned short)c;
  }
  __syncthreads();
  int* wl = reinterpret_cast<int*>(S.raw);
  for (int c = threadIdx.x; c < B; c += blockDim.x) wl[c] = a2_prev_writer(S, n_index - 1 - c, c);
  __syncthreads();
  auto last_value = [&](int c) {
    int w = wl[c];
    while (w >= 0) { c = w; w = wl[c]; }
    return S.ol[c];
  };
  for (int c = threadIdx.x; c < B; c += blockDim.x) {
    const int pos = S.k[c];
    const int wk = a2_prev_writer(S, pos, c);
    const int row = (wk < 0) ? index[pos] : last_value(wk);
    cand[c] = row;
    cand_k[c] = pos;
    cand_L[c] = last_value(c);
    cand_next[c] = a2_next_writer(S, pos, c);
  }
  const bool cull = a.vmax != nullptr;
  const int rank = st.rank;
  if (!cull) {
    for (int c = threadIdx.x; c < B; c += blockDim.x) live[c] = c;
    if (threadIdx.x == 0) S.n_live = B;
  } else {
    const double clo = a.node_box[2 * nid], chi = a.node_box[2 * nid + 1];
    const double* Ucol = nd.vbase + nd.row0;
    const double* xr = a.x + nd.row0;
    constexpr int G = 4;
    for (int t0 = 0; t0 < B; t0 += G * blockDim.x) {
      const int c0 = t0 + threadIdx.x;
      int row[G];
      double xi[G], b[G];
#pragma unroll
      for (int j = 0; j < G; ++j) { const int c = c0 + j * blockDim.x; row[j] = (c < B) ? cand[c] : 0; }
#pragma unroll
      for (int j = 0; j < G; ++j) xi[j] = xr[row[j]];
#pragma unroll
      for (int j = 0; j < G; ++j) b[j] = 0.0;
      for (int q = 0; q < rank; ++q) {
        double u[G];
#pragma unroll
        for (int j = 0; j < G; ++j) u[j] = __ldcg(Ucol + (int64_t)q * nd.ld + row[j]);
#pragma unroll
        for (int j = 0; j < G; ++j) b[j] += fabs(u[j]);
      }
      unsigned keep = 0u;
#pragma unroll
      for (int j = 0; j < G; ++j) {
        const int c = c0 + j * blockDim.x;
        if (c < B) {
          const double bb = b[j] + program_bound(a.prog, fmax(0.0, fmax(clo - xi[j], xi[j] - chi)), fmax(xi[j] - clo, chi - xi[j]));
          if (!(bb * 1.000001 < 1e-14)) keep |= 1u << j;
        }
      }
      const int base = S.n_live;
      int total;
      int pos = base + a2_block_scan(__popc(keep), S.redi, total);
#pragma unroll
      for (int j = 0; j < G; ++j) {
        if (keep & (1u << j)) {
          const int c = c0 + j * blockDim.x;
          live[pos++] = c;
          a.cand_xu[nd.cand_off + c] = make_double2(xi[j], b[j]);
        }
      }
      if (threadIdx.x == 0) S.n_live = base + total;
      __syncthreads();
    }
  }
  __syncthreads();
  {
    int n_live = S.n_live;
    const bool defer = (B == 1 && n_live == 1);
    if (threadIdx.x == 0) st.deferred = defer ? 1 : 0;
    if (defer) n_live = 0;
    const int ipc = (n_live <= 256) ? A2_CG : A2_CG * A2_ITEM_CB;
    const int per_chunk = (n_live + ipc - 1) / ipc;
    int my_chunks = nd.n_cchunks;
    const bool split = nd.is_top && a.shard_count > 1;
    if (split) my_chunks = (nd.n_cchunks - a.shard_rank + a.shard_count - 1) / a.shard_count;
    const int n_items = my_chunks * per_chunk;
    int4* work_next = a.work + (int64_t)nb * a.work_cap;
    auto item = [&](int t) {
      const int ci = t / per_chunk, pi = t % per_chunk;
      const int lc = split ? (a.shard_rank + ci * a.shard_count) : ci;
      const int c0 = pi * ipc;
      return make_int4(nd.cchunk0 + lc, c0, min(ipc, n_live - c0), nid);
    };
    __syncthreads();
    if (!cull) {
      if (threadIdx.x == 0) {
        S.flag = n_items ? atomicAdd(a.work_count + nb, n_items) : 0;
        if (S.flag + n_items > a.work_cap) st.status = 2;
      }
      __syncthreads();
      const int base = S.flag;
      for (int t = threadIdx.x; t < n_items; t += blockDim.x)
        if (base + t < a.work_cap) work_next[base + t] = item(t);
    } else {
      double* s_blo = reinterpret_cast<double*>((reinterpret_cast<uintptr_t>(S.hkey) + 7) & ~uintptr_t(7));
      double* s_bhi = s_blo + A2_PUB_BLOCKS;
      double* s_bu = s_bhi + A2_PUB_BLOCKS;
      for (int p0 = 0; p0 < per_chunk * ipc; p0 += blockDim.x) {
        const int p = p0 + threadIdx.x;
        double lo = __longlong_as_double(0x7ff0000000000000ll), hi = -lo, u = 0.0;
        bool bnan = false;
        if (p < n_live) {
          const double2 xu = a.cand_xu[nd.cand_off + live[p]];
          lo = hi = xu.x; u = xu.y;
          bnan = (xu.x != xu.x) || (xu.y != xu.y);
        }
        for (int o = 1; o < ipc; o <<= 1) {
          lo = fmin(lo, __shfl_xor_sync(0xffffffffu, lo, o));
          hi = fmax(hi, __shfl_xor_sync(0xffffffffu, hi, o));
          u = fmax(u, __shfl_xor_sync(0xffffffffu, u, o));
          bnan |= __shfl_xor_sync(0xffffffffu, (int)bnan, o) != 0;
        }
        if (bnan) lo = hi = u = __longlong_as_double(0x7ff8000000000000ll);
        if (p % ipc == 0 && p < n_live) { s_blo[p / ipc] = lo; s_bhi[p / ipc] = hi; s_bu[p / ipc] = u; }
      }
      __syncthreads();
      constexpr int R = 32;
      for (int r0 = 0; r0 < n_items; r0 += R * blockDim.x) {
        unsigned keep = 0u;
        for (int k = 0; k < R; ++k) {
          const int t = r0 + k * blockDim.x + threadIdx.x;
          if (t >= n_items) break;
          const int4 w = item(t);
          const int lc = w.x - nd.cchunk0, pi = w.y / ipc;
          const double2 cb = __ldcg(a.cbox + w.x);
          double vm = 0.0;
          bool vnan = false;
          for (int g = 0; g < A2_NGROUP && lc * A2_CHUNK + g * A2_GROUP < nd.n_cols; ++g) {
            const double v = __ldcg(a.vmax + ((int64_t)w.x * A2_NGROUP + g));
            vm = fmax(vm, v); vnan |= (v != v);
          }
          if (vnan) vm = __longlong_as_double(0x7ff8000000000000ll);
          const double lo = s_blo[pi], hi = s_bhi[pi];
          const double bb = program_bound(a.prog, fmax(0.0, fmax(cb.x - hi, lo - cb.y)), fmax(hi - cb.x, cb.y - lo)) + s_bu[pi] * vm;
          if (!(bb * 1.00001 < 1e-14)) keep |= 1u << k;
        }
        int total;
        const int off = a2_block_scan(__popc(keep), S.redi, total);
        if (threadIdx.x == 0) {
          S.flag = total ? atomicAdd(a.work_count + nb, total) : 0;
          if (S.flag + total > a.work_cap) st.status = 2;
        }
        __syncthreads();
        int q = S.flag + off;
        for (int k = 0; k < R; ++k) {
          if (keep & (1u << k)) {
            if (q < a.work_cap) work_next[q] = item(r0 + k * blockDim.x + threadIdx.x);
            ++q;
          }
        }
        __syncthreads();
      }
    }
  }
  __syncthreads();
}

__global__ void __launch_bounds__(A2_NODE_THREADS) a2_init_kernel(A2Args a) {
  extern __shared__ __align__(16) unsigned char a2_smem_raw[];
  A2NodeSmem& S = *reinterpret_cast<A2NodeSmem*>(a2_smem_raw);
  const int nid = blockIdx.x;
  const A2Node nd = a.nodes[nid];
  A2State& st = a.states[nid];
  int* index = a.idx_ws + nd.idx_off;
  for (int n = threadIdx.x; n < nd.n_rows; n += blockDim.x) index[n] = n;
  if (threadIdx.x == 0) {
    mt_seed(S.rng, node_seed(a.seed, nd.pre_id));
    st.rank = 0; st.draws = 0; st.n_index = nd.n_rows; st.fallback = 0; st.status = 0; st.active = 1;
    st.phase = A2_SELECT; st.B = 4; st.norm = 0.0; st.pivot = 0.0; st.piv_i = 0; st.piv_j = 0; st.ncand = 0;
  }
  __syncthreads();
  mt_copy(a.rngs + 2 * (int64_t)nid, &S.rng);
  __syncthreads();
  if (nd.cap <= 0) {
    if (threadIdx.x == 0) { st.status = 1; st.phase = A2_DONE; st.active = 0; { atomicSub(a.n_active, 1); if (nd.is_top) atomicSub(a.n_active + 1, 1); } }
    return;
  }
  if (a.vmax) {
    double lo = __longlong_as_double(0x7ff0000000000000ll), hi = -lo;
    bool has_nan = false;
    for (int n = threadIdx.x; n < nd.n_cols; n += blockDim.x) { const double xv = a.x[nd.col0 + n]; lo = fmin(lo, xv); hi = fmax(hi, xv); has_nan |= (xv != xv); }
    lo = -block_max_signed(-lo, S.red);
    hi = block_max_signed(hi, S.red);
    if (__syncthreads_or(has_nan)) lo = hi = __longlong_as_double(0x7ff8000000000000ll);
    if (threadIdx.x == 0) { a.node_box[2 * nid] = lo; a.node_box[2 * nid + 1] = hi; }
    const int lane = threadIdx.x & 31, nw = blockDim.x >> 5;
    for (int g = threadIdx.x >> 5; g < nd.n_cchunks * A2_NGROUP; g += nw) {
      const int w_lo = g * A2_GROUP;
      const int w_n = min(A2_GROUP, nd.n_cols - w_lo);
      if (w_n <= 0) break;
      double glo = __longlong_as_double(0x7ff0000000000000ll), ghi = -glo;
      bool gnan = false;
      for (int n = lane; n < w_n; n += 32) { const double xv = a.x[nd.col0 + w_lo + n]; glo = fmin(glo, xv); ghi = fmax(ghi, xv); gnan |= (xv != xv); }
#pragma unroll
      for (int o = 16; o > 0; o >>= 1) {
        glo = fmin(glo, __shfl_xor_sync(0xffffffffu, glo, o));
        ghi = fmax(ghi, __shfl_xor_sync(0xffffffffu, ghi, o));
      }
      if (__any_sync(0xffffffffu, gnan)) glo = ghi = __longlong_as_double(0x7ff8000000000000ll);
      if (lane == 0) a.gbox[(int64_t)nd.cchunk0 * A2_NGROUP + g] = make_double2(glo, ghi);
    }
    __syncthreads();
    for (int c = threadIdx.x; c < nd.n_cchunks; c += blockDim.x) {
      double clo = __longlong_as_double(0x7ff0000000000000ll), chi = -clo;
      bool cnan = false;
      for (int g = 0; g < A2_NGROUP && c * A2_CHUNK + g * A2_GROUP < nd.n_cols; ++g) {
        const double2 b = a.gbox[(int64_t)(nd.cchunk0 + c) * A2_NGROUP + g];
        clo = fmin(clo, b.x); chi = fmax(chi, b.y); cnan |= (b.x != b.x);
      }
      if (cnan) clo = chi = __longlong_as_double(0x7ff8000000000000ll);
      a.cbox[nd.cchunk0 + c] = make_double2(clo, chi);
    }
    __syncthreads();
  }
  a2_generate(a, st, S, nd, nid, 0);
}

template <class KFn, bool CULL>
__device__ __forceinline__ void a2_eval_body(const A2Args& a, const A2Node& nd, int rank, int chunk, int c_first,
                                             int c_count, int ndim, KFn fn, int warp, unsigned long long& n_eval,
                                             unsigned long long& n_fma, unsigned& n_live_units) {
  const int lc = chunk - nd.cchunk0;
  const int lane = threadIdx.x & 31;
  const int w_lo = lc * A2_CHUNK + warp * A2_GROUP;
  const int w_n = min(A2_GROUP, nd.n_cols - w_lo);
  if (w_n <= 0) return;
  const double* Vcols = nd.vbase;
  const double* xr = a.x + (int64_t)nd.row0 * ndim;
  const double* xc = a.x + (int64_t)(nd.col0 + w_lo) * ndim;
  const int* cand = a.cand + nd.cand_off;
  const int* live_list = a.cand_live + nd.cand_off;
  unsigned long long* cmax = a.cmax + nd.cand_off;
  int ncol[A2_EPT];
#pragma unroll
  for (int e = 0; e < A2_EPT; ++e) ncol[e] = min(lane + 32 * e, w_n - 1);

  double glo = 0.0, ghi = 0.0;
  const double* vmaxg = nullptr;
  const bool cull = CULL && a.vmax != nullptr;
  double vg = 0.0;
  if constexpr (CULL) if (cull) {
    const double2 gb = __ldcg(a.gbox + ((int64_t)chunk * A2_NGROUP + warp));
    glo = gb.x; ghi = gb.y;
    vmaxg = a.vmax + ((int64_t)chunk * A2_NGROUP + warp);
    vg = __ldcg(vmaxg);
  }

  const int ncand = c_first + c_count;
  bool unit_live = false;
  for (int cb0 = c_first; cb0 < ncand; cb0 += 32) {
    const bool valid = cb0 + lane < ncand;
    const int myc = valid ? live_list[cb0 + lane] : 0;
    const int myrow = valid ? cand[myc] : 0;
    unsigned live = __ballot_sync(0xffffffffu, valid);
    if constexpr (CULL) if (cull) {
      bool keep = valid;
      if (valid) {
        const double2 xu = __ldcg(a.cand_xu + nd.cand_off + myc);
        const double gap = fmax(0.0, fmax(glo - xu.x, xu.x - ghi));
        const double b = fn.bound(gap, fmax(xu.x - glo, ghi - xu.x)) + xu.y * vg;
        keep = !(b * 1.000001 < 1e-14);
      }
      live = __ballot_sync(0xffffffffu, keep);
    }
    unit_live |= (live != 0u);
    n_eval += (unsigned long long)__popc(live) * (unsigned long long)w_n;
    n_fma += (unsigned long long)__popc(live) * (unsigned long long)w_n * (unsigned long long)rank;
    while (live) {
      int sel[A2_CG], row[A2_CG], cidx[A2_CG];
      int ncb = 0;
#pragma unroll
      for (int c = 0; c < A2_CG; ++c) {
        if (live) { sel[c] = __ffs(live) - 1; live &= live - 1; ncb = c + 1; }
        else sel[c] = sel[0];
        row[c] = __shfl_sync(0xffffffffu, myrow, sel[c]);
        cidx[c] = __shfl_sync(0xffffffffu, myc, sel[c]);
      }
      double vals[A2_CG][A2_EPT];
#pragma unroll
      for (int e = 0; e < A2_EPT; ++e) {
        const double* x2 = xc + (int64_t)ncol[e] * ndim;
#pragma unroll
        for (int c = 0; c < A2_CG; ++c) vals[c][e] = fn(xr + (int64_t)row[c] * ndim, x2);
      }
      int k = 0;
      for (; k + 2 <= rank; k += 2) {
        const double* vc0 = Vcols + (int64_t)k * nd.ld;
        const double* vc1 = vc0 + nd.ld;
        double vk0[A2_EPT], vk1[A2_EPT], u0[A2_CG], u1[A2_CG];
#pragma unroll
        for (int c = 0; c < A2_CG; ++c) { u0[c] = __ldcg(vc0 + nd.row0 + row[c]); u1[c] = __ldcg(vc1 + nd.row0 + row[c]); }
#pragma unroll
        for (int e = 0; e < A2_EPT; ++e) { vk0[e] = vc0[nd.col0 + w_lo + ncol[e]]; vk1[e] = vc1[nd.col0 + w_lo + ncol[e]]; }
#pragma unroll
        for (int c = 0; c < A2_CG; ++c)
#pragma unroll
          for (int e = 0; e < A2_EPT; ++e) { vals[c][e] -= u0[c] * vk0[e]; vals[c][e] -= u1[c] * vk1[e]; }
      }
      for (; k < rank; ++k) {
        const double* vcol = Vcols + (int64_t)k * nd.ld;
        double vk[A2_EPT], u[A2_CG];
#pragma unroll
        for (int c = 0; c < A2_CG; ++c) u[c] = __ldcg(vcol + nd.row0 + row[c]);
#pragma unroll
        for (int e = 0; e < A2_EPT; ++e) vk[e] = vcol[nd.col0 + w_lo + ncol[e]];
#pragma unroll
        for (int c = 0; c < A2_CG; ++c)
#pragma unroll
          for (int e = 0; e < A2_EPT; ++e) vals[c][e] -= u[c] * vk[e];
      }
#pragma unroll
      for (int c = 0; c < A2_CG; ++c) {
        double best = 0.0;
        bool isnan_any = false;
#pragma unroll
        for (int e = 0; e < A2_EPT; ++e) {
          const double av = fabs(vals[c][e]);
          if (lane + 32 * e < w_n) { best = fmax(best, av); isnan_any |= (av != av); }
        }
        if (isnan_any) best = __longlong_as_double(0x7ff8000000000000ll);
        unsigned long long bits = (unsigned long long)__double_as_longlong(best);
#pragma unroll
        for (int o = 16; o > 0; o >>= 1) {
          const unsigned long long ob = __shfl_xor_sync(0xffffffffu, bits, o);
          bits = ob > bits ? ob : bits;
        }
        if (lane == 0 && c < ncb && bits != 0ull) atomicMax(cmax + cidx[c], bits);
      }
    }
  }
  n_live_units += unit_live ? 1u : 0u;
}

template <int SHAPE, int MINB>
__global__ void __launch_bounds__(A2_THREADS, MINB) a2_eval_kernel(A2Args a) {
  __shared__ DevProgram P;
  const int buf = *a.iter_ptr & 1;
  const int n_items = min(a.work_count[buf], a.work_cap);
  const int4* items = a.work + (int64_t)buf * a.work_cap;
  if (blockIdx.x == 0 && threadIdx.x == 0) a.work_count[buf ^ 1] = 0;
  if constexpr (SHAPE == BGP_SHAPE_GENERIC) {
    stage_program(&P, a.prog);
    __syncthreads();
  }
  const auto fn = ShapeEval<SHAPE>::make(&P, a.prog);
  constexpr bool CULL = shape_has_bound(SHAPE);
  unsigned long long n_eval = 0ull, n_fma = 0ull;
  unsigned n_pulled = 0u, n_live_units = 0u;
  int* cursor = a.work_cursor + buf;
  if (blockIdx.x == 0 && threadIdx.x == 0) a.work_cursor[buf ^ 1] = 0;
  const int n_units = n_items * A2_NGROUP;
  while (true) {
    int u = 0;
    if ((threadIdx.x & 31) == 0) u = atomicAdd(cursor, 1);
    u = __shfl_sync(0xffffffffu, u, 0);
    if (u >= n_units) break;
    ++n_pulled;
    const int4 w = items[u / A2_NGROUP];
    const int grp = u % A2_NGROUP;
    const A2Node& nd = a.nodes[w.w];
    const int rank = a.states[w.w].rank;
    if constexpr (SHAPE == BGP_SHAPE_GENERIC) a2_eval_body<decltype(fn), false>(a, nd, rank, w.x, w.y, w.z, P.ndim, fn, grp, n_eval, n_fma, n_live_units);
    else a2_eval_body<decltype(fn), CULL>(a, nd, rank, w.x, w.y, w.z, 1, fn, grp, n_eval, n_fma, n_live_units);
  }
  if ((threadIdx.x & 31) == 0 && n_eval) { atomicAdd(a.stats + 3, n_eval); atomicAdd(a.stats + 1, n_fma); }
  if ((threadIdx.x & 31) == 0 && n_pulled) {
    atomicAdd(a.stats + A2_UNITS_PULLED, (unsigned long long)n_pulled);
    atomicAdd(a.stats + A2_UNITS_LIVE, (unsigned long long)n_live_units);
  }
}
inline void a2_eval_launch(int shape, dim3 grid, cudaStream_t s, const A2Args& a, int minb) {
  if (minb == 3 && shape != BGP_SHAPE_GENERIC) {
    BGP_SHAPE_SWITCH(shape, (a2_eval_kernel<SHAPE, (SHAPE == BGP_SHAPE_GENERIC ? 2 : 3)><<<grid, A2_THREADS, 0, s>>>(a)));
  } else {
    BGP_SHAPE_SWITCH(shape, (a2_eval_kernel<SHAPE, 2><<<grid, A2_THREADS, 0, s>>>(a)));
  }
}

__global__ void __launch_bounds__(A2_NODE_THREADS) a2_decide_kernel(A2Args a) {
  extern __shared__ __align__(16) unsigned char a2_smem_raw[];
  A2NodeSmem& S = *reinterpret_cast<A2NodeSmem*>(a2_smem_raw);
  __shared__ int s_winner;
  const int nid = blockIdx.x;
  A2State& st = a.states[nid];
  if (st.phase != A2_SELECT || !st.active) return;
  const A2Node nd = a.nodes[nid];
  const int ncand = st.ncand;
  int* cand = a.cand + nd.cand_off;
  int* cand_k = a.cand_k + nd.cand_off;
  int* words = a.cand_words + nd.cand_off;
  int* index = a.idx_ws + nd.idx_off;
  const int lane = threadIdx.x & 31, warp = threadIdx.x >> 5;
  if (threadIdx.x == 0) {
    s_winner = 0x7fffffff;
  }
  __syncthreads();
  const bool deferred = st.deferred != 0;
  if (deferred) {
    if (threadIdx.x == 0) { s_winner = 0; atomicAdd(a.stats + 3, (unsigned long long)nd.n_cols); }
  } else {
    const unsigned long long* cmax = a.cmax + nd.cand_off;
    int mine = 0x7fffffff;
    for (int c = threadIdx.x; c < ncand; c += blockDim.x) {
      const double m = __longlong_as_double((long long)cmax[c]);
      if (!(m < 1e-14)) { mine = c; break; }
    }
    if (mine != 0x7fffffff) atomicMin(&s_winner, mine);
  }
  __syncthreads();
  const int p = s_winner;
  {
    MT19937* rng_commit = a.rngs + 2 * (int64_t)nid;
    const int w = (p != 0x7fffffff) ? words[p] : (ncand > 0 ? words[ncand - 1] : 0);
    if (w == st.end_words) {
      mt_copy(&S.rng, rng_commit + 1);
    } else {
      if (threadIdx.x == 0) atomicAdd(a.stats + A2_PATH_PARTIAL, 1ull);
      mt_copy(&S.rng, rng_commit);
      __syncthreads();
      mt_skip_coop(S.rng, w);
    }
    if (threadIdx.x == 0) st.draws += w;
    __syncthreads();
    mt_copy(rng_commit, &S.rng);
  }
  {
    const int last = (p != 0x7fffffff) ? p : ncand - 1;
    if (threadIdx.x == 0) {
      atomicAdd(a.stats + 0, (unsigned long long)(last + 1) * (unsigned long long)nd.n_cols);
      atomicAdd(a.stats + 2, (unsigned long long)(last + 1));
    }
    const int* cand_L = a.cand_L + nd.cand_off;
    const int* cand_next = a.cand_next + nd.cand_off;
    for (int c = threadIdx.x; c <= last; c += blockDim.x)
      if (cand_next[c] > last) index[cand_k[c]] = cand_L[c];
  }
  __syncthreads();
  if (p != 0x7fffffff) {
    if (threadIdx.x == 0) {
      st.n_index -= (p + 1);
      st.piv_i = cand[p];
      st.phase = A2_ACCEPT;
      st.B = (p == 0) ? 1 : max(1, min(st.B, 2 * (p + 1)));
    }
    return;
  }
  if (threadIdx.x == 0) {
    st.n_index -= ncand;
    st.B = min(A2_BGROW * st.B, A2_BMAX);
    if (st.n_index == 0) {
      st.fallback = 1;
      st.phase = A2_DONE; st.active = 0;
      { atomicSub(a.n_active, 1); if (nd.is_top) atomicSub(a.n_active + 1, 1); }
    }
  }
  __syncthreads();
  if (st.n_index == 0) return;
  a2_generate(a, st, S, nd, nid, (*a.iter_ptr + 1) & 1);
}

constexpr int A2_KU = 8;
template <class KFn>
__device__ __forceinline__ double a2_resid_entry(const KFn& fn, const double* xa, const double* xb, int rank,
                                                 const double* __restrict__ pcol,
                                                 int64_t ld, const double* __restrict__ coef_g,
                                                 double* s_coef, bool active) {
  double val = active ? fn(xa, xb) : 0.0;
  for (int k0 = 0; k0 < rank; k0 += 128) {
    const int nk = min(128, rank - k0);
    __syncthreads();
    for (int k = threadIdx.x; k < nk; k += A2_THREADS) s_coef[k] = __ldcg(coef_g + (int64_t)(k0 + k) * ld);
    __syncthreads();
    if (active) {
      const double* pc = pcol + (int64_t)k0 * ld;
      int k = 0;
      for (; k + A2_KU <= nk; k += A2_KU) {
        double pv[A2_KU];
#pragma unroll
        for (int q = 0; q < A2_KU; ++q) pv[q] = pc[(int64_t)(k + q) * ld];
#pragma unroll
        for (int q = 0; q < A2_KU; ++q) val -= s_coef[k + q] * pv[q];
      }
      for (; k < nk; ++k) val -= s_coef[k] * pc[(int64_t)k * ld];
    }
  }
  return val;
}

__device__ __forceinline__ bool a2_pivot_better(double v, int i, double bv, int bi) {
  const double k = aca_pivot_key(v), bk = aca_pivot_key(bv);
  return bi == 0x7fffffff || k > bk || (k == bk && i < bi);
}

template <int SHAPE>
__global__ void __launch_bounds__(A2_THREADS) a2_vrow_kernel(A2Args a) {
  __shared__ DevProgram P;
  __shared__ double s_x[ACA_MAX_NDIM];
  __shared__ double s_u[128];
  __shared__ double s_red[A2_THREADS / 32];
  __shared__ int s_redi[A2_THREADS / 32];
  const int chunk = blockIdx.x, sub = blockIdx.y;
  const int nid = a.cchunk_node[chunk];
  const A2State& st = a.states[nid];
  if (st.phase != A2_ACCEPT || !st.active) return;
  const A2Node nd = a.nodes[nid];
  const int lc = chunk - nd.cchunk0;
  const int c_lo = lc * A2_CHUNK + sub * A2_THREADS;
  if (c_lo >= nd.n_cols) return;
  if constexpr (SHAPE == BGP_SHAPE_GENERIC) stage_program(&P, a.prog);
  const int ndim = a.prog->ndim;
  const int rank = st.rank;
  const int c_n = min(A2_THREADS, nd.n_cols - c_lo);
  double* Vcols = nd.vbase;
  const int i = st.piv_i;
  for (int q = threadIdx.x; q < ndim; q += A2_THREADS) s_x[q] = a.x[(int64_t)(nd.row0 + i) * ndim + q];
  __syncthreads();
  const auto fn = ShapeEval<SHAPE>::make(&P, a.prog);
  const int n = threadIdx.x;
  const bool act = n < c_n;
  const int nn = act ? n : 0;
  const double val = a2_resid_entry(fn, s_x, a.x + (int64_t)(nd.col0 + c_lo + nn) * ndim, rank, Vcols + nd.col0 + c_lo + nn,
                                    nd.ld, Vcols + nd.row0 + i, s_u, act);
  double best = -1.0, bval = 0.0;
  int bidx = 0x7fffffff;
  if (act) {
    Vcols[(int64_t)rank * nd.ld + nd.col0 + c_lo + n] = val;
    best = aca_pivot_key(val); bidx = c_lo + n; bval = val;
  }
  const int lane = threadIdx.x & 31, warp = threadIdx.x >> 5;
#pragma unroll
  for (int o = 16; o > 0; o >>= 1) {
    const double ob = __shfl_xor_sync(0xffffffffu, best, o);
    const double ov = __shfl_xor_sync(0xffffffffu, bval, o);
    const int oi = __shfl_xor_sync(0xffffffffu, bidx, o);
    if (ob > best || (ob == best && oi < bidx)) { best = ob; bidx = oi; bval = ov; }
  }
  if (lane == 0) { s_red[warp] = bval; s_redi[warp] = bidx; }
  __syncthreads();
  if (threadIdx.x == 0) {
    for (int w = 1; w < A2_THREADS / 32; ++w) {
      const double ov = s_red[w];
      const int oi = s_redi[w];
      if (oi == 0x7fffffff) continue;
      if (a2_pivot_better(ov, oi, bval, bidx)) { bval = ov; bidx = oi; }
    }
    A2EPart p;
    p.val = bval; p.idx = bidx; p._pad = 0;
    a.epart[(int64_t)(nd.cchunk0 + lc) * A2_NSUB + sub] = p;
  }
}

__global__ void __launch_bounds__(32) a2_pivot_kernel(A2Args a) {
  const int nid = blockIdx.x;
  A2State& st = a.states[nid];
  if (st.phase != A2_ACCEPT || !st.active) return;
  const A2Node nd = a.nodes[nid];
  const int lane = threadIdx.x;
  double bval = 0.0;
  int bidx = 0x7fffffff;
  const int nsub = (nd.n_cols + A2_THREADS - 1) / A2_THREADS;
  for (int ch = lane; ch < nsub; ch += 32) {
    const A2EPart q = a.epart[(int64_t)nd.cchunk0 * A2_NSUB + ch];
    if (q.idx == 0x7fffffff) continue;
    if (a2_pivot_better(q.val, q.idx, bval, bidx)) { bval = q.val; bidx = q.idx; }
  }
#pragma unroll
  for (int o = 16; o > 0; o >>= 1) {
    const double ov = __shfl_xor_sync(0xffffffffu, bval, o);
    const int oi = __shfl_xor_sync(0xffffffffu, bidx, o);
    if (oi == 0x7fffffff) continue;
    if (a2_pivot_better(ov, oi, bval, bidx)) { bval = ov; bidx = oi; }
  }
  if (lane == 0) {
    st.piv_j = bidx; st.pivot = bval;
    if (a.vmax && !(fabs(bval) <= DBL_MAX)) a.node_box[2 * nid] = a.node_box[2 * nid + 1] = __longlong_as_double(0x7ff8000000000000ll);
    if (st.deferred && fabs(bval) < 1e-14) st.phase = A2_LATE_REJECT;
  }
}

__device__ __forceinline__ void a2_partial_dots(const double* __restrict__ pbase, int64_t ld, int rank, const double* s_vec,
                                                int cnt, double* __restrict__ part) {
  const int lane = threadIdx.x & 31, warp = threadIdx.x >> 5;
  constexpr int W = A2_THREADS / 32, QU = 4;
  for (int q0 = warp * QU; q0 < rank; q0 += W * QU) {
    double acc[QU];
#pragma unroll
    for (int u = 0; u < QU; ++u) acc[u] = 0.0;
    for (int n = lane; n < cnt; n += 32) {
      const double sv = s_vec[n];
      double pv[QU];
#pragma unroll
      for (int u = 0; u < QU; ++u) pv[u] = (q0 + u < rank) ? pbase[(int64_t)(q0 + u) * ld + n] : 0.0;
#pragma unroll
      for (int u = 0; u < QU; ++u) acc[u] += pv[u] * sv;
    }
#pragma unroll
    for (int u = 0; u < QU; ++u) {
      const double r = warp_sum(acc[u]);
      if (lane == 0 && q0 + u < rank) part[1 + q0 + u] = r;
    }
  }
}

__device__ __forceinline__ void a2_vnorm_body(const A2Args& a, int chunk, int sub, double* s_v, double* red) {
  const int nid = a.cchunk_node[chunk];
  const A2State& st = a.states[nid];
  if (st.phase != A2_ACCEPT || !st.active) return;
  const A2Node nd = a.nodes[nid];
  const int rank = st.rank;
  const int lc = chunk - nd.cchunk0;
  const int c_lo = lc * A2_CHUNK + sub * A2_THREADS;
  if (c_lo >= nd.n_cols) return;
  const int c_n = min(A2_THREADS, nd.n_cols - c_lo);
  double* Vcols = nd.vbase;
  const double pivot = st.pivot;
  const int lane = threadIdx.x & 31, warp = threadIdx.x >> 5;
  double vn2 = 0.0, av = 0.0;
  {
    const int n = threadIdx.x;
    double v = 0.0;
    if (n < c_n) {
      double* pv = Vcols + (int64_t)rank * nd.ld + nd.col0 + c_lo + n;
      v = *pv / pivot;
      *pv = v;
      vn2 = v * v;
      av = fabs(v);
      if (v != v) av = __longlong_as_double(0x7ff0000000000000ll);
    }
    s_v[n] = v;
  }
  if (a.vmax) {
    av = warp_max(av);
    if (lane == 0) red[16 + warp] = av;
  }
  vn2 = block_sum(vn2, red);
  if (a.vmax && threadIdx.x < 2) {
    const int g = threadIdx.x;
    const double m = fmax(fmax(red[16 + 4 * g], red[17 + 4 * g]), fmax(red[18 + 4 * g], red[19 + 4 * g]));
    double* slot = a.vmax + ((int64_t)chunk * A2_NGROUP + sub * 2 + g);
    if (rank == 0 || m > *slot || m != m) *slot = m;
  }
  double* part = a.vpart + ((int64_t)chunk * A2_NSUB + sub) * (a.capmax + 1);
  if (threadIdx.x == 0) part[0] = vn2;
  a2_partial_dots(Vcols + nd.col0 + c_lo, nd.ld, rank, s_v, c_n, part);
}

template <int SHAPE>
__global__ void __launch_bounds__(A2_THREADS) a2_vnorm_ucol_kernel(A2Args a, int n_cchunks_total) {
  __shared__ DevProgram P;
  __shared__ double s_x[ACA_MAX_NDIM];
  __shared__ double s_vr[128];
  __shared__ double s_u[A2_THREADS];
  __shared__ double red[32];
  const int sub = blockIdx.y;
  if ((int)blockIdx.x < n_cchunks_total) { a2_vnorm_body(a, blockIdx.x, sub, s_u, red); return; }
  const int chunk = blockIdx.x - n_cchunks_total;
  const int nid = a.rchunk_node[chunk];
  const A2State& st = a.states[nid];
  if (st.phase != A2_ACCEPT || !st.active) return;
  const A2Node nd = a.nodes[nid];
  const int lr = chunk - nd.rchunk0;
  const int r_lo = lr * A2_CHUNK + sub * A2_THREADS;
  if (r_lo >= nd.n_rows) return;
  if constexpr (SHAPE == BGP_SHAPE_GENERIC) stage_program(&P, a.prog);
  const int ndim = a.prog->ndim;
  const int rank = st.rank;
  const int r_n = min(A2_THREADS, nd.n_rows - r_lo);
  double* Vcols = nd.vbase;
  const int j = st.piv_j;
  for (int q = threadIdx.x; q < ndim; q += A2_THREADS) s_x[q] = a.x[(int64_t)(nd.col0 + j) * ndim + q];
  __syncthreads();
  const auto fn = ShapeEval<SHAPE>::make(&P, a.prog);
  const int n = threadIdx.x;
  const bool act = n < r_n;
  const int nn = act ? n : 0;
  const double val = a2_resid_entry(fn, a.x + (int64_t)(nd.row0 + r_lo + nn) * ndim, s_x, rank, Vcols + nd.row0 + r_lo + nn, nd.ld,
                                    Vcols + nd.col0 + j, s_vr, act);
  double un2 = 0.0;
  if (act) {
    Vcols[(int64_t)rank * nd.ld + nd.row0 + r_lo + n] = val;
    un2 = val * val;
  }
  s_u[n] = act ? val : 0.0;
  un2 = block_sum(un2, red);
  double* part = a.upart + ((int64_t)chunk * A2_NSUB + sub) * (a.capmax + 1);
  if (threadIdx.x == 0) part[0] = un2;
  a2_partial_dots(Vcols + nd.row0 + r_lo, nd.ld, rank, s_u, r_n, part);
}
inline void a2_vrow_launch(int shape, dim3 grid, cudaStream_t s, const A2Args& a) {
  BGP_SHAPE_SWITCH(shape, (a2_vrow_kernel<SHAPE><<<grid, A2_THREADS, 0, s>>>(a)));
}
inline void a2_vnorm_ucol_launch(int shape, dim3 grid, cudaStream_t s, const A2Args& a, int ncc) {
  BGP_SHAPE_SWITCH(shape, (a2_vnorm_ucol_kernel<SHAPE><<<grid, A2_THREADS, 0, s>>>(a, ncc)));
}

__global__ void __launch_bounds__(A2_NODE_THREADS) a2_finish_kernel(A2Args a) {
  extern __shared__ __align__(16) unsigned char a2_smem_raw[];
  A2NodeSmem& S = *reinterpret_cast<A2NodeSmem*>(a2_smem_raw);
  __shared__ int s_done;
  const int nid = blockIdx.x;
  A2State& st = a.states[nid];
  if (!st.active) return;
  if (st.phase == A2_LATE_REJECT) {
    const A2Node nd = a.nodes[nid];
    __syncthreads();
    if (threadIdx.x == 0) {
      st.B = min(A2_BGROW * st.B, A2_BMAX);
      if (st.n_index == 0) {
        st.fallback = 1;
        st.phase = A2_DONE; st.active = 0;
        { atomicSub(a.n_active, 1); if (nd.is_top) atomicSub(a.n_active + 1, 1); }
      } else {
        st.phase = A2_SELECT;
      }
    }
    __syncthreads();
    if (st.phase == A2_DONE) return;
    mt_copy(&S.rng, a.rngs + 2 * (int64_t)nid);
    __syncthreads();
    a2_generate(a, st, S, nd, nid, (*a.iter_ptr + 1) & 1);
    return;
  }
  if (st.phase != A2_ACCEPT) return;
  const A2Node nd = a.nodes[nid];
  const int rank = st.rank;
  double vn2 = 0.0, un2 = 0.0;
  const int nvs = (nd.n_cols + A2_THREADS - 1) / A2_THREADS, nus = (nd.n_rows + A2_THREADS - 1) / A2_THREADS;
  const double* vp0 = a.vpart + (int64_t)nd.cchunk0 * A2_NSUB * (a.capmax + 1);
  const double* up0 = a.upart + (int64_t)nd.rchunk0 * A2_NSUB * (a.capmax + 1);
  for (int c = threadIdx.x; c < nvs; c += blockDim.x) vn2 += vp0[(int64_t)c * (a.capmax + 1)];
  for (int c = threadIdx.x; c < nus; c += blockDim.x) un2 += up0[(int64_t)c * (a.capmax + 1)];
  vn2 = block_sum(vn2, S.red);
  un2 = block_sum(un2, S.red);
  double vdot = 0.0, udot = 0.0;
  for (int k = threadIdx.x; k < rank; k += blockDim.x) {
    double sv = 0.0, su = 0.0;
    for (int c = 0; c < nvs; ++c) sv += vp0[(int64_t)c * (a.capmax + 1) + 1 + k];
    for (int c = 0; c < nus; ++c) su += up0[(int64_t)c * (a.capmax + 1) + 1 + k];
    vdot = fmax(vdot, fabs(sv));
    udot = fmax(udot, fabs(su));
  }
  vdot = block_max(vdot, S.red);
  udot = block_max(udot, S.red);
  mt_copy(&S.rng, a.rngs + 2 * (int64_t)nid);
  if (threadIdx.x == 0) {
    a.piv_rows[nd.piv_off + rank] = st.piv_i;
    a.piv_cols[nd.piv_off + rank] = st.piv_j;
    const int new_rank = rank + 1;
    st.rank = new_rank;
    const int max_rank = min(nd.n_rows, nd.n_cols);
    bool done = false;
    if (new_rank >= max_rank) done = true;
    else {
      const double rowcol = un2 * vn2;
      if (rowcol < a.tol * a.tol * st.norm) done = true;
      else {
        st.norm += rowcol;
        if (new_rank > 1) st.norm += 2.0 * udot + 2.0 * vdot;
        if (new_rank >= nd.cap) { st.status = 1; done = true; }
        else if (st.n_index == 0) { st.fallback = 1; done = true; }
      }
    }
    if (done) {
      st.phase = A2_DONE; st.active = 0;
      { atomicSub(a.n_active, 1); if (nd.is_top) atomicSub(a.n_active + 1, 1); }
    } else {
      st.phase = A2_SELECT;
    }
    s_done = done ? 1 : 0;
  }
  __syncthreads();
  if (s_done) return;
  a2_generate(a, st, S, nd, nid, (*a.iter_ptr + 1) & 1);
}

__global__ void a2_tick_kernel(int* iter_ptr, const int* n_active, cudaGraphConditionalHandle handle, int use_handle) {
  const int it = *iter_ptr + 1;
  *iter_ptr = it;
  if (use_handle) cudaGraphSetConditional(handle, (*n_active > 0 && it < (1 << 22)) ? 1u : 0u);
}

__global__ void __launch_bounds__(256) a2_dense_fill_kernel(A2Args a) {
  __shared__ DevProgram P;
  const int nid = blockIdx.x;
  A2State& st = a.states[nid];
  if (!st.fallback || a.exhaust_mode != BGP_EXHAUST_DENSE || st.status) return;
  const A2Node nd = a.nodes[nid];
  const int max_rank = min(nd.n_rows, nd.n_cols);
  if (max_rank > nd.cap) {
    if (blockIdx.y == 0 && threadIdx.x == 0) st.status = 1;
    return;
  }
  stage_program(&P, a.prog);
  __syncthreads();
  const int ndim = P.ndim;
  const double* xr = a.x + (int64_t)nd.row0 * ndim;
  const double* xc = a.x + (int64_t)nd.col0 * ndim;
  for (int m = blockIdx.y; m < nd.n_cols; m += gridDim.y) {
    double* vc = nd.vbase + (int64_t)m * nd.ld;
    for (int n = threadIdx.x; n < nd.n_cols; n += blockDim.x) vc[nd.col0 + n] = (n == m) ? 1.0 : 0.0;
    for (int n = threadIdx.x; n < nd.n_rows; n += blockDim.x)
      vc[nd.row0 + n] = kernel_value(P, xr + (int64_t)n * ndim, xc + (int64_t)m * ndim);
  }
}
__global__ void a2_dense_rank_kernel(A2Args a) {
  const int nid = blockIdx.x * blockDim.x + threadIdx.x;
  if (nid >= a.n_nodes) return;
  A2State& st = a.states[nid];
  if (st.fallback && a.exhaust_mode == BGP_EXHAUST_DENSE && !st.status) {
    const A2Node nd = a.nodes[nid];
    st.rank = min(nd.n_rows, nd.n_cols);
  }
}

}
```

george_b200/solvers/_hodlr.py:

```python

import ctypes as C

import numpy as np

from .. import _lib
from .._spec import HodlrNodeInfo, HodlrOpts, flatten
from .basic import BasicSolver

RNG_MODES = {"pernode": 0, "reference": 1}


def resolve_rng_mode(rng_mode, tol):
    if rng_mode is None:
        return "reference" if tol > 1e-6 else "pernode"
    return rng_mode
EXHAUST_MODES = {"dense": 0, "lowrank": 1}


class HODLRSolver(object):

    _parked = []
    _max_parked = 2

    def __init__(self):
# ... 23 lines not shown
        lib = _lib.load()
        while cls._parked:
            lib.bgp_hodlr_destroy(cls._parked.pop())

    @property
    def computed(self):
        if self._fresh:
            return 0
        return int(self._lib.bgp_hodlr_computed(self._ptr))

    @property
    def log_determinant(self):
        if self._fresh:
            raise RuntimeError("the solver has not been computed")
        out = C.c_double()
        _lib.check(self._lib.bgp_hodlr_log_determinant(self._ptr, C.byref(out)))
        return out.value

    def _opts(self, min_size, tol, seed, rng_mode, rank_capacity, shard_rank=0, shard_count=1, exhaust="dense"):
        o = HodlrOpts()
        self._lib.bgp_hodlr_default_opts(C.byref(o))
        o.min_size, o.tol, o.seed = int(min_size), float(tol), int(seed)
        o.rng_mode = RNG_MODES[rng_mode] if isinstance(rng_mode, str) else int(rng_mode)
        o.rank_capacity = int(rank_capacity)
        o.shard_rank, o.shard_count = int(shard_rank), int(shard_count)
        o.exhaust_mode = EXHAUST_MODES[exhaust] if isinstance(exhaust, str) else int(exhaust)
        return o

    def compute(self, kernel_spec, x, yerr, min_size=100, tol=0.1, seed=42, rng_mode=None, rank_capacity=0,
                shard_rank=0, shard_count=1, exhaust="dense"):
        rng_mode = "pernode" if shard_count > 1 and rng_mode is None else resolve_rng_mode(rng_mode, tol)
        x = np.ascontiguousarray(x, dtype=np.float64)
        if x.ndim != 2:
            raise ValueError("array has incorrect number of dimensions: {0}; expected 2".format(x.ndim))
        yerr = np.ascontiguousarray(yerr, dtype=np.float64)
        if yerr.shape != (x.shape[0],):
            raise ValueError("dimension mismatch")
        spec = flatten(kernel_spec)
        o = self._opts(min_size, tol, seed, rng_mode, rank_capacity, shard_rank, shard_count, exhaust)
        self._n = x.shape[0]
        self.shard_count = int(shard_count)
        self._fresh = False
        _lib.check(self._lib.bgp_hodlr_compute(self._ptr, C.byref(spec), _lib.ptr(x), x.shape[0], x.shape[1],
                                               _lib.ptr(yerr), C.byref(o)))
        return 0

    def _require_computed(self):
        if self._fresh:
            raise RuntimeError("the solver has not been computed")

    def apply_inverse(self, x, in_place=False):
        self._require_computed()
        x = np.asarray(x)
        if in_place and x.dtype == np.float64 and x.flags.f_contiguous and x.flags.writeable and x.ndim == 2:
            b = x
        else:
            b = np.array(x, dtype=np.float64, order="F")
            if b.ndim == 1:
                b = b.reshape(-1, 1, order="F")
        if b.shape[0] != self._n:
            raise ValueError("dimension mismatch")
        _lib.check(self._lib.bgp_hodlr_apply_inverse(self._ptr, _lib.ptr(b), b.shape[1], self._n))
        if in_place and b is not x:
            x[...] = b.reshape(x.shape)
        return b

    def dot_solve(self, x):
        self._require_computed()
        x = np.ascontiguousarray(x, dtype=np.float64)
        if x.shape != (self._n,):
            raise ValueError("dimension mismatch")
        out = C.c_double()
        _lib.check(self._lib.bgp_hodlr_dot_solve(self._ptr, _lib.ptr(x), C.byref(out)))
        return out.value

    def get_inverse(self):
        self._require_computed()
        out = np.empty((self._n, self._n), dtype=np.float64)
        _lib.check(self._lib.bgp_hodlr_get_inverse(self._ptr, _lib.ptr(out)))
        return out.T

    def nodes(self):
        n = C.c_int64()
        _lib.check(self._lib.bgp_hodlr_num_nodes(self._ptr, C.byref(n)))
        arr = (HodlrNodeInfo * n.value)()
        _lib.check(self._lib.bgp_hodlr_node_info(self._ptr, arr))
        names = [f[0] for f in HodlrNodeInfo._fields_]
        return [dict((k, getattr(a, k)) for k in names) for a in arr]

    def pivots(self, node, rank):
        rows = np.zeros(max(rank, 1), dtype=np.int32)
        cols = np.zeros(max(rank, 1), dtype=np.int32)
        _lib.check(self._lib.bgp_hodlr_node_pivots(self._ptr, node, _lib.ptr(rows), _lib.ptr(cols)))
        return rows[:rank], cols[:rank]

    def factors(self, node):
        self._require_computed()
        nodes = self.nodes()
        if not 0 <= node < len(nodes):
            raise IndexError("node index out of range")
        nd = nodes[node]
        out = np.zeros((nd["size"], nd["rank"]), dtype=np.float64, order="F")
        _lib.check(self._lib.bgp_hodlr_node_factors(self._ptr, node, _lib.ptr(out)))
        return out[:nd["half"]], out[nd["half"]:]

    def draw_paths(self):
        self._require_computed()
        c = (C.c_uint64 * 4)()
        _lib.check(self._lib.bgp_hodlr_last_draw_paths(self._ptr, c))
        return dict(zip(("lemire_redos", "truncated_batches", "sequential_draws", "partial_commits"), (int(v) for v in c)))

    def eval_units(self):
        self._require_computed()
        c = (C.c_uint64 * 2)()
        _lib.check(self._lib.bgp_hodlr_last_eval_units(self._ptr, c))
        return dict(zip(("pulled", "live"), (int(v) for v in c)))

    def timing(self):
        t = (C.c_double * 5)()
        _lib.check(self._lib.bgp_hodlr_last_timing(self._ptr, t))
        return dict(zip(("leaves_ms", "aca_ms", "upsweep_ms", "compute_ms", "solve_ms"), list(t)))

    def grad_timing(self):
        t = (C.c_double * 4)()
        _lib.check(self._lib.bgp_hodlr_last_grad_timing(self._ptr, t))
        out = dict(zip(("solve_ms", "contract_ms", "slabs", "slab_cols"), list(t)))
        out["slabs"], out["slab_cols"] = int(out["slabs"]), int(out["slab_cols"])
        return out

    def grad_terms_local(self, alpha_dev, which, diag_dev=None):
        self._require_computed()
        which = np.ascontiguousarray(which, dtype=np.uint32)
        g = np.zeros(max(which.size, 1), dtype=np.float64)
        _lib.check(self._lib.bgp_hodlr_grad_terms_local_dev(self._ptr, _lib.ptr(which), alpha_dev, _lib.ptr(g),
                                                            diag_dev))
        return g[:which.size]

    def predict_local(self, kernel, xs, what, w_dev, ldw, add_prior):
        self._require_computed()

        def call(ptr, spec, xs_p, ns, kind, out):
            return self._lib.bgp_hodlr_predict_local_dev(ptr, spec, xs_p, ns, kind, w_dev, int(ldw),
                                                         1 if add_prior else 0, out)
        return BasicSolver._predictive_call(call, self._ptr, kernel, xs, what)

    def set_profiling(self, on=True):
        _lib.check(self._lib.bgp_hodlr_set_profiling(self._ptr, 1 if on else 0))

    def aca_profile(self):
        p = (C.c_double * 12)()
        _lib.check(self._lib.bgp_hodlr_last_aca_profile(self._ptr, p))
        out = dict(zip(("eval_ms", "eval_launches", "evals", "update_fmas", "candidates", "evaluated"), list(p)[:6]))
        out["kernel_ms"] = dict(zip(("a2_eval", "a2_decide", "a2_vrow", "a2_pivot", "a2_vnorm_ucol", "a2_finish"), list(p)[6:]))
        return out

    def work(self):
        w = (C.c_double * 6)()
        _lib.check(self._lib.bgp_hodlr_last_work(self._ptr, w))
        return dict(zip(("evals", "bytes", "flops", "R", "leaf", "levels"), list(w)))
```

include/bgp.h:

```cpp
#ifndef BGP_B200_H_
#define BGP_B200_H_

#include <stdint.h>
#include <stddef.h>

#ifdef __cplusplus
extern "C" {
#endif

enum {
  BGP_OK = 0,
  BGP_ERR_INVALID = 1,
  BGP_ERR_DIM = 2,
  BGP_ERR_NOT_COMPUTED = 3,
  BGP_ERR_LINALG = 4,
  BGP_ERR_CUDA = 5,
  BGP_ERR_NO_DEVICE = 6,
  BGP_ERR_RANK_CAPACITY = 7,
  BGP_ERR_INDEX = 8,
  BGP_ERR_NOMEM = 9
};

const char* bgp_last_error(void);
int bgp_version(void);
// ... 50 lines not shown
                                double* out );
int bgp_kmat_gradient_general(const bgp_kernel_spec_t* spec, const uint32_t* which, const double* x1, int64_t n1,
                              const double* x2, int64_t n2, double* out );
int bgp_kmat_x1_gradient_general(const bgp_kernel_spec_t* spec, const double* x1, int64_t n1, const double* x2,
                                 int64_t n2, double* out );
int bgp_kmat_x2_gradient_general(const bgp_kernel_spec_t* spec, const double* x1, int64_t n1, const double* x2,
                                 int64_t n2, double* out );
int bgp_kmat_symmetric_dev(const bgp_kernel_spec_t* spec, const double* x_dev, int64_t n, const double* diag_add_dev,
                           double* out_dev, int64_t ld);
int bgp_kmat_general_dev(const bgp_kernel_spec_t* spec, const double* x1_dev, int64_t n1, const double* x2_dev,
                         int64_t n2, double* out_dev, int64_t ld);

int bgp_kmat_matvec(const bgp_kernel_spec_t* spec, const double* x1, int64_t n1, const double* x2, int64_t n2,
                    const double* diag, const double* v, int64_t nrhs, double* out);
int bgp_kmat_matvec_dev(const bgp_kernel_spec_t* spec, const double* x1_dev, int64_t n1, const double* x2_dev,
                        int64_t n2, const double* diag_dev, const double* v_dev, int64_t nrhs, double* out_dev);
int bgp_kmat_gradient_contract(const bgp_kernel_spec_t* spec, const uint32_t* which, const double* x, int64_t n,
                               const double* A, double* out );
int bgp_kmat_x1_gradient_matvec(const bgp_kernel_spec_t* spec, const double* x1, int64_t n1, const double* x2,
                                int64_t n2, const double* v, int64_t ldv, double scale, int32_t add_prior,
                                double* out );
int bgp_kmat_x1_gradient_matvec_dev(const bgp_kernel_spec_t* spec, const double* x1_dev, int64_t n1,
                                    const double* x2_dev, int64_t n2, const double* v_dev, int64_t ldv, double scale,
                                    int32_t add_prior, double* out_dev);

typedef struct bgp_dense bgp_dense_t;
int bgp_dense_create(bgp_dense_t** out);
void bgp_dense_destroy(bgp_dense_t* h);
int bgp_dense_compute(bgp_dense_t* h, const bgp_kernel_spec_t* spec, const double* x, int64_t n, int32_t ndim,
                      const double* yerr);
int bgp_dense_computed(const bgp_dense_t* h);
int bgp_dense_log_determinant(const bgp_dense_t* h, double* out);
int bgp_dense_apply_inverse(bgp_dense_t* h, double* b, int64_t nrhs, int64_t ldb);
int bgp_dense_dot_solve(bgp_dense_t* h, const double* y, double* out);
int bgp_dense_apply_sqrt(bgp_dense_t* h, const double* r, int64_t nr, double* out);
int bgp_dense_get_inverse(bgp_dense_t* h, double* out);
int bgp_dense_export_factor(bgp_dense_t* h, double* out);
int bgp_dense_import_factor(bgp_dense_t* h, const double* factor, int64_t n, double log_det);
int bgp_dense_grad_terms(bgp_dense_t* h, const uint32_t* which, const double* r, double* alpha_out, double* g_out,
                         double* diag_out);
int bgp_dense_last_timing(const bgp_dense_t* h, double* ms2);

enum { BGP_PREDICT_VAR = 0, BGP_PREDICT_COV = 1 };
int bgp_dense_predict(bgp_dense_t* h, const bgp_kernel_spec_t* spec, const double* xs, int64_t ns, int32_t what,
                      double* out);
int bgp_dense_predict_grad(bgp_dense_t* h, const bgp_kernel_spec_t* spec, const double* xs, int64_t ns, double* var,
                           double* dvar);

typedef struct bgp_dense_batch bgp_dense_batch_t;
int bgp_dense_batch_create(bgp_dense_batch_t** out);
void bgp_dense_batch_destroy(bgp_dense_batch_t* h);
int bgp_dense_batch_log_likelihood(bgp_dense_batch_t* h, const bgp_kernel_spec_t* spec, const double* params,
                                   int64_t B, int64_t P, const double* x, int64_t n, int32_t ndim,
                                   const double* yerr, const double* r,
                                   double* log_det, double* quad, int32_t* info);
int bgp_dense_batch_grad_terms(bgp_dense_batch_t* h, const bgp_kernel_spec_t* spec, const double* params,
                               int64_t B, int64_t P, const double* x, int64_t n, int32_t ndim,
                               const double* yerr, const double* r,
                               const uint32_t* which,
                               double* log_det, double* quad,
                               double* alpha, double* diag,
                               double* g,
                               int32_t* info);
int bgp_dense_batch_predict(bgp_dense_batch_t* h, const bgp_kernel_spec_t* spec, const double* params,
                            int64_t B, int64_t P, const double* x, int64_t n, int32_t ndim,
                            const double* yerr, const double* r,
                            const double* xs, int64_t ns, int32_t what,
                            double* mean,
                            double* out,
                            int32_t* info);
int bgp_dense_batch_sample(bgp_dense_batch_t* h, const bgp_kernel_spec_t* spec, const double* params,
                           int64_t B, int64_t P, const double* x, int64_t n, int32_t ndim,
                           const double* yerr, const double* r,
                           const double* xs, int64_t ns,
                           const double* mean_add,
                           const double* z, int64_t size, double jitter,
                           double* draws,
                           int32_t* info, int32_t* draw_info);

typedef struct bgp_hodlr bgp_hodlr_t;

enum {
  BGP_RNG_PER_NODE = 0,
  BGP_RNG_REFERENCE = 1
};

typedef struct bgp_hodlr_opts {
  int32_t min_size;
  int32_t seed;
  double  tol;
  int32_t rng_mode;
  int32_t rank_capacity;
  int32_t shard_rank;
  int32_t shard_count;
  int32_t exhaust_mode;
} bgp_hodlr_opts_t;
enum { BGP_EXHAUST_DENSE = 0, BGP_EXHAUST_LOWRANK = 1 };

void bgp_hodlr_default_opts(bgp_hodlr_opts_t* o);
int bgp_hodlr_create(bgp_hodlr_t** out);
void bgp_hodlr_destroy(bgp_hodlr_t* h);
int bgp_hodlr_compute(bgp_hodlr_t* h, const bgp_kernel_spec_t* spec, const double* x, int64_t n, int32_t ndim,
                      const double* yerr, const bgp_hodlr_opts_t* opts);
int bgp_hodlr_compute_dev(bgp_hodlr_t* h, const bgp_kernel_spec_t* spec, const double* x_dev, int64_t n,
                          int32_t ndim, const double* yerr_dev, const bgp_hodlr_opts_t* opts);
int bgp_hodlr_computed(const bgp_hodlr_t* h);
int bgp_hodlr_log_determinant(const bgp_hodlr_t* h, double* out);
int bgp_hodlr_apply_inverse(bgp_hodlr_t* h, double* b, int64_t nrhs, int64_t ldb);
int bgp_hodlr_dot_solve(bgp_hodlr_t* h, const double* y, double* out);
int bgp_hodlr_dot_solve_dev(bgp_hodlr_t* h, const double* y_dev, double* out);
int bgp_hodlr_get_inverse(bgp_hodlr_t* h, double* out);

int bgp_hodlr_grad_terms(bgp_hodlr_t* h, const uint32_t* which, const double* r, double* alpha_out, double* g_out,
                         double* diag_out);
int bgp_hodlr_grad_terms_local_dev(bgp_hodlr_t* h, const uint32_t* which, const double* alpha_dev, double* g_part_out,
                                   double* diag_dev);
int bgp_hodlr_predict(bgp_hodlr_t* h, const bgp_kernel_spec_t* spec, const double* xs, int64_t ns, int32_t what,
                      double* out);
int bgp_hodlr_predict_grad(bgp_hodlr_t* h, const bgp_kernel_spec_t* spec, const double* xs, int64_t ns, double* var,
                           double* dvar);
int bgp_hodlr_predict_local_dev(bgp_hodlr_t* h, const bgp_kernel_spec_t* spec, const double* xs, int64_t ns,
                                int32_t what, const double* w_dev, int64_t ldw, int32_t add_prior, double* out);

#define BGP_SAMPLE_DMMA_ROWS 8
int bgp_mvn_sample(const double* cov, int64_t ns, const double* mean, const double* z, int64_t size, double jitter,
                   double* out);
int bgp_dense_sample(bgp_dense_t* h, const bgp_kernel_spec_t* spec, const double* xs, int64_t ns, const double* mean,
                     const double* z, int64_t size, double jitter, double* out);
int bgp_hodlr_sample(bgp_hodlr_t* h, const bgp_kernel_spec_t* spec, const double* xs, int64_t ns, const double* mean,
                     const double* z, int64_t size, double jitter, double* out);
int bgp_sample_last_timing(double* ms3);

typedef struct bgp_hodlr_node_info {
  int32_t start, size, half;
  int32_t is_leaf;
  int32_t parent;
  int32_t direction;
  int32_t depth;
  int32_t rank;
  int32_t rng_draws;
  int32_t dense_fallback;
} bgp_hodlr_node_info_t;
int bgp_hodlr_num_nodes(const bgp_hodlr_t* h, int64_t* out);
int bgp_hodlr_node_info(const bgp_hodlr_t* h, bgp_hodlr_node_info_t* out );
int bgp_hodlr_node_pivots(const bgp_hodlr_t* h, int64_t node, int32_t* rows, int32_t* cols);
int bgp_hodlr_node_factors(const bgp_hodlr_t* h, int64_t node, double* out);
int bgp_hodlr_last_draw_paths(const bgp_hodlr_t* h, uint64_t* out4);
int bgp_hodlr_last_eval_units(const bgp_hodlr_t* h, uint64_t* out2);
int bgp_hodlr_last_timing(const bgp_hodlr_t* h, double* ms5);
int bgp_hodlr_last_grad_timing(const bgp_hodlr_t* h, double* out4);
int bgp_hodlr_last_work(const bgp_hodlr_t* h, double* w6);
int bgp_hodlr_set_profiling(bgp_hodlr_t* h, int on);
int bgp_hodlr_last_aca_profile(const bgp_hodlr_t* h, double* p12);

int bgp_selftest_lu(int32_t n, int32_t nrhs, const double* S_host, double* R_host, double* logdet);
int bgp_selftest_gemm(int32_t a_kcontig, int32_t b_kcontig, int32_t m, int32_t n, int32_t k, const double* A_host,
                      int64_t lda, const double* B_host, int64_t ldb, double* C_host, int64_t ldc, int32_t mode);

int bgp_hodlr_top_panel(bgp_hodlr_t* h, double** ptr_dev, int64_t* row0, int64_t* rows, int64_t* cols, int64_t* ld);
int bgp_hodlr_export_top(bgp_hodlr_t* h, double* buf_dev, int64_t rows_pad);
int bgp_hodlr_import_top(bgp_hodlr_t* h, const double* all_buf_dev, int64_t rows_pad);
int bgp_hodlr_shard_rows(const bgp_hodlr_t* h, int32_t s, int64_t* row0, int64_t* rows);
int bgp_hodlr_finish_top(bgp_hodlr_t* h);
int bgp_comm_unique_id(void* out128, const char* nccl_path);
int bgp_comm_init(const void* id128, int rank, int world, const char* nccl_path);
int bgp_comm_destroy(void);
int bgp_comm_size(void);
int bgp_hodlr_solve_local_dev(bgp_hodlr_t* h, double* b_dev, int64_t nrhs, int64_t ldb);
int bgp_hodlr_solve_top_dev(bgp_hodlr_t* h, double* b_dev, int64_t nrhs, int64_t ldb);

int bgp_dev_alloc(void** ptr_dev, size_t bytes);
int bgp_dev_free(void* ptr_dev);
int bgp_dev_upload(void* dst_dev, const void* src_host, size_t bytes);
int bgp_dev_download(void* dst_host, const void* src_dev, size_t bytes);
int bgp_dev_synchronize(void);
int bgp_host_alloc_pinned(void** ptr, size_t bytes);
int bgp_host_free_pinned(void* ptr);

#ifdef __cplusplus
}
#endif
#endif
```

Measured before the change: 22.68 million.

## Rewrite MT19937 fill as ring-buffer recurrence and precompute per-chunk vmax for culling

Replaces the cooperative Mersenne Twister twist/fill/skip with a single ring-buffer recurrence that produces 227 words per synchronised step instead of twisting the whole state in phases. Skipping now goes through the same path. The change also maintains a per-chunk max vnorm (cvmax), updated with atomicMax, so the culling test reads one value instead of looping over groups. It adds a row_xu accumulator and per-iteration profiling instrumentation (a census kernel, clock stamps and a Python accessor), and adds a larger shared-memory ring per node block, which may reduce occupancy.

```diff
diff --git a/george_b200/_lib.py b/george_b200/_lib.py
--- a/george_b200/_lib.py
+++ b/george_b200/_lib.py
@@ -109,8 +109,10 @@
     "bgp_hodlr_last_work": (C.c_int, [_p, _dp]),
     "bgp_hodlr_set_profiling": (C.c_int, [_p, C.c_int]),
     "bgp_hodlr_last_aca_profile": (C.c_int, [_p, _dp]),
+    "bgp_hodlr_last_aca_iterations": (C.c_int, [_p, _i32, _dp, C.POINTER(_i32)]),
     "bgp_selftest_lu": (C.c_int, [_i32, _i32, _p, _p, _p]),
     "bgp_selftest_gemm": (C.c_int, [_i32, _i32, _i32, _i32, _i32, _p, _i64, _p, _i64, _p, _i64, _i32]),
+    "bgp_selftest_mt_fill": (C.c_int, [C.c_uint32, _i32, _p, _p, _p]),
     "bgp_hodlr_top_panel": (C.c_int, [_p, C.POINTER(_p), C.POINTER(_i64), C.POINTER(_i64), C.POINTER(_i64),
                                       C.POINTER(_i64)]),
     "bgp_hodlr_export_top": (C.c_int, [_p, _p, _i64]),
diff --git a/george_b200/csrc/hodlr.cu b/george_b200/csrc/hodlr.cu
--- a/george_b200/csrc/hodlr.cu
+++ b/george_b200/csrc/hodlr.cu
@@ -125,8 +125,9 @@
   DevBuf<A2EPart> d_epart;
   DevBuf<int> d_cand, d_cand_k, d_cand_words, d_cand_L, d_cand_next, d_cand_live, d_cchunk_node, d_rchunk_node, d_nactive;
   DevBuf<double> d_node_box;
-  DevBuf<double2> d_cand_xu, d_gbox, d_cbox;
-  DevBuf<unsigned long long> d_cmax, d_stats;
+  DevBuf<double2> d_cand_xu, d_row_xu, d_gbox, d_cbox;
+  DevBuf<unsigned long long> d_cmax, d_stats, d_cvmax, d_clk;
+  DevBuf<int> d_census;
   DevBuf<int4> d_work;
   DevBuf<int> d_work_count, d_iter;
   AcaGraphKey aca_key;
@@ -136,6 +137,7 @@
   bool profile = false;
   std::vector<cudaEvent_t> prof_events;
   double prof[12] = {0, 0, 0, 0, 0, 0, 0, 0, 0, 0, 0, 0};
+  std::vector<double> prof_iters;
   uint64_t draw_paths[4] = {0, 0, 0, 0};
   uint64_t eval_units[2] = {0, 0};
   DevBuf<double> d_vpart, d_upart, d_vmax;
@@ -396,8 +398,10 @@
   if (cull) {
     BGP_TRY(h->d_vmax.reserve((size_t)ncc * A2_NGROUP, s));
     BGP_TRY(h->d_cand_xu.reserve((size_t)cand_total, s));
+    BGP_TRY(h->d_row_xu.reserve((size_t)nrc * A2_CHUNK, s));
     BGP_TRY(h->d_gbox.reserve((size_t)ncc * A2_NGROUP, s));
     BGP_TRY(h->d_cbox.reserve((size_t)ncc, s));
+    BGP_TRY(h->d_cvmax.reserve((size_t)ncc, s));
   }
   BGP_TRY(h->d_nactive.reserve(2, s));
   int n_top = 0;
@@ -428,8 +432,10 @@
   a.cchunk_node = h->d_cchunk_node.p; a.rchunk_node = h->d_rchunk_node.p; a.vpart = h->d_vpart.p; a.upart = h->d_upart.p;
   a.vmax = cull ? h->d_vmax.p : nullptr;
   a.cand_xu = cull ? h->d_cand_xu.p : nullptr;
+  a.row_xu = cull ? h->d_row_xu.p : nullptr;
   a.gbox = cull ? h->d_gbox.p : nullptr;
   a.cbox = cull ? h->d_cbox.p : nullptr;
+  a.cvmax = cull ? h->d_cvmax.p : nullptr;
   a.cand_L = h->d_cand_L.p; a.cand_next = h->d_cand_next.p; a.cand_live = h->d_cand_live.p; a.node_box = h->d_node_box.p;
   a.capmax = capmax; a.n_active = h->d_nactive.p; a.stats = h->d_stats.p;
   a.work = h->d_work.p; a.work_count = h->d_work_count.p; a.work_cursor = h->d_work_count.p + 2; a.work_cap = (int)work_cap; a.iter_ptr = h->d_iter.p;
@@ -475,11 +481,29 @@
     a2_finish_kernel<<<nn, A2_NODE_THREADS, sizeof(A2NodeSmem), st>>>(a);
     BGP_LAUNCH_CHECK();
     BGP_TRY(mark(6));
+    if (it_prof >= 0) {
+      a2_census_kernel<<<1, 1024, 0, st>>>(a, h->d_census.p + 2 * (it_prof % A2_CLK_ROWS));
+      BGP_LAUNCH_CHECK();
+    }
     a2_tick_kernel<<<1, 1, 0, st>>>(a.iter_ptr, a.n_active, hnd, use_hnd);
     BGP_LAUNCH_CHECK();
     return BGP_OK;
   };
   const bool use_graph = !h->profile && !getenv("BGP_NO_GRAPH");
+  std::vector<int> census;
+  std::vector<unsigned long long> slow;
+  const size_t clk_row = (size_t)nn * A2_CLK_STAMPS;
+  std::vector<unsigned long long> clk_host;
+  h->prof_iters.clear();
+  if (h->profile) {
+    BGP_TRY(h->d_census.reserve((size_t)2 * A2_CLK_ROWS, s));
+#ifdef BGP_ACA_CLOCKS
+    BGP_TRY(h->d_clk.reserve(A2_CLK_ROWS * clk_row, s));
+    BGP_CUDA(cudaMemsetAsync(h->d_clk.p, 0, sizeof(unsigned long long) * A2_CLK_ROWS * clk_row, s));
+    a.clk = h->d_clk.p;
+    clk_host.resize(A2_CLK_ROWS * clk_row);
+#endif
+  }
   if (use_graph) {
     AcaGraphKey key;
     memset(&key, 0, sizeof(key));
@@ -518,12 +542,36 @@
     if (act2[0] > 0) { set_error("ACA did not terminate"); return BGP_ERR_CUDA; }
   } else {
     while (active > 0) {
+      const int it0 = iters;
       for (int rep = 0; rep < 8; ++rep) {
         BGP_TRY(launch_iteration(s, 0, 0, h->profile ? iters : -1));
         iters++;
       }
       int act2[2] = {0, 0};
       BGP_CUDA(cudaMemcpyAsync(act2, h->d_nactive.p, sizeof(int) * 2, cudaMemcpyDeviceToHost, s));
+      if (h->profile) {
+        int c16[2 * A2_CLK_ROWS];
+        BGP_CUDA(cudaMemcpyAsync(c16, h->d_census.p, sizeof(c16), cudaMemcpyDeviceToHost, s));
+        if (a.clk) {
+          BGP_CUDA(cudaMemcpyAsync(clk_host.data(), a.clk, sizeof(unsigned long long) * clk_host.size(), cudaMemcpyDeviceToHost, s));
+          BGP_CUDA(cudaStreamSynchronize(s));
+          BGP_CUDA(cudaMemsetAsync(a.clk, 0, sizeof(unsigned long long) * clk_host.size(), s));
+        }
+        BGP_CUDA(cudaStreamSynchronize(s));
+        for (int i = it0; i < iters; ++i) {
+          census.push_back(c16[2 * (i % A2_CLK_ROWS)]);
+          census.push_back(c16[2 * (i % A2_CLK_ROWS) + 1]);
+          unsigned long long best[A2_CLK_STAMPS] = {0, 0, 0, 0, 0, 0, 0, 0};
+          if (a.clk) {
+            const unsigned long long* rows = clk_host.data() + (size_t)((i + 1) % A2_CLK_ROWS) * clk_row;
+            for (int n = 0; n < nn; ++n) {
+              const unsigned long long* r = rows + (size_t)n * A2_CLK_STAMPS;
+              if (r[0] && r[6] - r[0] > best[6] - best[0]) std::copy(r, r + A2_CLK_STAMPS, best);
+            }
+          }
+          slow.insert(slow.end(), best, best + A2_CLK_STAMPS);
+        }
+      }
       BGP_CUDA(cudaStreamSynchronize(s));
       active = act2[0];
       if (iters > (1 << 22)) { set_error("ACA did not terminate"); return BGP_ERR_CUDA; }
@@ -548,6 +596,19 @@
         }
       h->prof[0] = tot[0];
       for (int k = 0; k < 6; ++k) h->prof[6 + k] = tot[k];
+      h->prof_iters.assign((size_t)iters * BGP_ACA_ITER_COLS, 0.0);
+      for (int i = 0; i < iters; ++i) {
+        double* row = h->prof_iters.data() + (size_t)i * BGP_ACA_ITER_COLS;
+        for (int k = 0; k < 6; ++k) {
+          float ms = 0;
+          cudaEventElapsedTime(&ms, h->prof_events[(size_t)7 * i + k], h->prof_events[(size_t)7 * i + k + 1]);
+          row[k] = ms;
+        }
+        row[6] = census[2 * i]; row[7] = census[2 * i + 1];
+        const unsigned long long* b = slow.data() + (size_t)i * A2_CLK_STAMPS;
+        row[8] = (double)b[7];
+        for (int k = 0; k < 6; ++k) row[9 + k] = b[0] ? (double)(b[k + 1] - b[k]) : 0.0;
+      }
     }
   }
   if (h->opts.exhaust_mode == BGP_EXHAUST_DENSE) {
@@ -1093,9 +1154,9 @@
   h->lu_ws.d_nodes.release(); h->lu_ws.d_trsm.release(); h->lu_ws.d_gemm.release(); h->d_gram_desc.release(); h->d_upd_desc.release();
   h->d_ticket.release(); h->d_chain_done.release(); h->d_ncols_by_depth.release(); h->d_chain_state.release();
   h->d_a2nodes.release(); h->d_a2states.release(); h->d_a2rngs.release(); h->d_epart.release(); h->d_cand.release(); h->d_cand_k.release();
-  h->d_cand_words.release(); h->d_cand_L.release(); h->d_cand_next.release(); h->d_cand_live.release(); h->d_node_box.release(); h->d_cand_xu.release(); h->d_gbox.release(); h->d_cbox.release(); h->d_cchunk_node.release(); h->d_rchunk_node.release(); h->d_nactive.release();
+  h->d_cand_words.release(); h->d_cand_L.release(); h->d_cand_next.release(); h->d_cand_live.release(); h->d_node_box.release(); h->d_cand_xu.release(); h->d_row_xu.release(); h->d_gbox.release(); h->d_cbox.release(); h->d_cchunk_node.release(); h->d_rchunk_node.release(); h->d_nactive.release();
   h->d_inv.release(); h->d_gscratch.release(); h->d_which.release(); h->d_xsend.release(); h->d_xrecv.release();
-  h->d_vpart.release(); h->d_upart.release(); h->d_vmax.release(); h->d_cmax.release(); h->d_stats.release(); h->d_work.release(); h->d_work_count.release();
+  h->d_vpart.release(); h->d_upart.release(); h->d_vmax.release(); h->d_cvmax.release(); h->d_clk.release(); h->d_census.release(); h->d_cmax.release(); h->d_stats.release(); h->d_work.release(); h->d_work_count.release();
   for (cudaEvent_t e : h->prof_events) cudaEventDestroy(e);
   h->d_iter.release();
   if (h->aca_exec) cudaGraphExecDestroy(h->aca_exec);
@@ -1678,6 +1739,14 @@
   for (int i = 0; i < 12; ++i) p12[i] = h->prof[i];
   return BGP_OK;
 }
+int bgp_hodlr_last_aca_iterations(const bgp_hodlr_t* h, int32_t cap, double* rows, int32_t* n_iters) {
+  if (!h || !n_iters || (cap > 0 && !rows)) { set_error("bgp_hodlr_last_aca_iterations: null argument"); return BGP_ERR_INVALID; }
+  const int32_t n = (int32_t)(h->prof_iters.size() / BGP_ACA_ITER_COLS);
+  *n_iters = n;
+  const size_t m = (size_t)std::min(std::max(cap, 0), n) * BGP_ACA_ITER_COLS;
+  std::copy(h->prof_iters.begin(), h->prof_iters.begin() + m, rows);
+  return BGP_OK;
+}
 int bgp_hodlr_last_work(const bgp_hodlr_t* h, double* w6) {
   if (!h) { set_error("null handle"); return BGP_ERR_INVALID; }
   for (int i = 0; i < 6; ++i) w6[i] = h->work[i];
@@ -1701,6 +1770,42 @@
   BGP_TRY(lu_solve_batch(ws, nodes, n, dR.p, 0, n, nrhs, false, s));
   if (nrhs) BGP_CUDA(cudaMemcpyAsync(R_host, dR.p, sizeof(double) * n * nrhs, cudaMemcpyDeviceToHost, s));
   BGP_CUDA(cudaMemcpyAsync(logdet, dld.p, sizeof(double), cudaMemcpyDeviceToHost, s));
+  BGP_CUDA(cudaStreamSynchronize(s));
+  return BGP_OK;
+}
+
+__global__ void __launch_bounds__(A2_NODE_THREADS) a2_selftest_mt_fill_kernel(uint32_t seed, int n_calls, const int* lens,
+                                                                              uint32_t* words, uint32_t* state) {
+  __shared__ MT19937 g;
+  __shared__ uint32_t ring[A2_RING];
+  if (threadIdx.x == 0) mt_seed(g, seed);
+  int64_t off = 0;
+  for (int i = 0; i < n_calls; ++i) {
+    const int n = lens[i];
+    mt_fill_coop(g, ring, n >= 0 ? words + off : nullptr, n >= 0 ? n : -n);
+    if (n > 0) off += n;
+  }
+  __syncthreads();
+  for (int i = threadIdx.x; i < 624; i += blockDim.x) state[i] = g.mt[i];
+  if (threadIdx.x == 0) state[624] = (uint32_t)g.idx;
+}
+int bgp_selftest_mt_fill(uint32_t seed, int32_t n_calls, const int32_t* lens, uint32_t* words, uint32_t* state) {
+  BGP_TRY(require_device());
+  if (n_calls < 0 || (n_calls && !lens) || !state) { set_error("bgp_selftest_mt_fill: bad arguments"); return BGP_ERR_INVALID; }
+  int64_t n_out = 0;
+  for (int i = 0; i < n_calls; ++i) n_out += std::max(lens[i], 0);
+  if (n_out && !words) { set_error("bgp_selftest_mt_fill: null words"); return BGP_ERR_INVALID; }
+  cudaStream_t s = 0;
+  DevBuf<int> dl;
+  DevBuf<uint32_t> dw, ds;
+  BGP_TRY(dl.alloc(std::max(n_calls, 1), s));
+  BGP_TRY(dw.alloc((size_t)std::max<int64_t>(n_out, 1), s));
+  BGP_TRY(ds.alloc(625, s));
+  if (n_calls) BGP_CUDA(cudaMemcpyAsync(dl.p, lens, sizeof(int) * n_calls, cudaMemcpyHostToDevice, s));
+  a2_selftest_mt_fill_kernel<<<1, A2_NODE_THREADS, 0, s>>>(seed, n_calls, dl.p, dw.p, ds.p);
+  BGP_LAUNCH_CHECK();
+  if (n_out) BGP_CUDA(cudaMemcpyAsync(words, dw.p, sizeof(uint32_t) * n_out, cudaMemcpyDeviceToHost, s));
+  BGP_CUDA(cudaMemcpyAsync(state, ds.p, sizeof(uint32_t) * 625, cudaMemcpyDeviceToHost, s));
   BGP_CUDA(cudaStreamSynchronize(s));
   return BGP_OK;
 }
diff --git a/george_b200/csrc/hodlr_aca2.cuh b/george_b200/csrc/hodlr_aca2.cuh
--- a/george_b200/csrc/hodlr_aca2.cuh
+++ b/george_b200/csrc/hodlr_aca2.cuh
@@ -56,27 +56,6 @@
   for (int i = threadIdx.x; i < (int)(sizeof(MT19937) / 4); i += blockDim.x) d[i] = s[i];
 }
 
-__device__ __forceinline__ void mt_twist_coop(MT19937& g) {
-  auto value = [&](uint32_t a, uint32_t b, uint32_t m) {
-    const uint32_t y = (a & 0x80000000u) | (b & 0x7fffffffu);
-    return m ^ (y >> 1) ^ ((y & 1u) ? 0x9908b0dfu : 0u);
-  };
-  auto phase = [&](int lo, int hi, int moff) {
-    for (int base = lo; base < hi; base += blockDim.x) {
-      const int i = base + threadIdx.x;
-      uint32_t v = 0;
-      if (i < hi) v = value(g.mt[i], g.mt[i + 1], g.mt[i + moff]);
-      __syncthreads();
-      if (i < hi) g.mt[i] = v;
-      __syncthreads();
-    }
-  };
-  phase(0, 227, 397);
-  phase(227, 454, -227);
-  phase(454, 623, -227);
-  if (threadIdx.x == 0) { g.mt[623] = value(g.mt[623], g.mt[0], g.mt[396]); g.idx = 0; }
-  __syncthreads();
-}
 __device__ __forceinline__ uint32_t mt_temper(uint32_t y) {
   y ^= (y >> 11);
   y ^= (y << 7) & 0x9d2c5680u;
@@ -84,31 +63,35 @@
   y ^= (y >> 18);
   return y;
 }
-__device__ inline void mt_fill_coop(MT19937& g, uint32_t* out, int n) {
-  int done = 0;
-  __syncthreads();
-  while (done < n) {
-    if (g.idx >= 624) mt_twist_coop(g);
-    const int idx = g.idx;
-    const int take = min(n - done, 624 - idx);
-    for (int t = threadIdx.x; t < take; t += blockDim.x) out[done + t] = mt_temper(g.mt[idx + t]);
-    __syncthreads();
-    if (threadIdx.x == 0) g.idx = idx + take;
-    __syncthreads();
-    done += take;
-  }
-}
-__device__ inline void mt_skip_coop(MT19937& g, int n) {
-  __syncthreads();
-  while (n > 0) {
-    if (g.idx >= 624) mt_twist_coop(g);
-    const int idx = g.idx;
-    const int take = min(n, 624 - idx);
-    __syncthreads();
-    if (threadIdx.x == 0) g.idx = idx + take;
-    __syncthreads();
-    n -= take;
-  }
+constexpr int A2_RING = 1024;
+static_assert(A2_RING >= 624 + 227 && (A2_RING & (A2_RING - 1)) == 0, "one step of the recurrence fits the ring");
+__device__ inline void mt_fill_coop(MT19937& g, uint32_t* ring, uint32_t* out, int n) {
+  __syncthreads();
+  if (n <= 0) return;
+  const int idx0 = g.idx;
+  const int end = idx0 + n;
+  const int gens = (end - 1) / 624;
+  for (int i = threadIdx.x; i < 624; i += blockDim.x) {
+    const uint32_t v = g.mt[i];
+    ring[i] = v;
+    if (out && i >= idx0 && i < end) out[i - idx0] = mt_temper(v);
+  }
+  __syncthreads();
+  const int gend = 624 * (gens + 1);
+  for (int m0 = 624; m0 < gend; m0 += 227) {
+    const int m = m0 + (int)threadIdx.x;
+    if (threadIdx.x < 227 && m < gend) {
+      const uint32_t y = (ring[(m - 624) & (A2_RING - 1)] & 0x80000000u) | (ring[(m - 623) & (A2_RING - 1)] & 0x7fffffffu);
+      const uint32_t v = ring[(m - 227) & (A2_RING - 1)] ^ (y >> 1) ^ ((y & 1u) ? 0x9908b0dfu : 0u);
+      ring[m & (A2_RING - 1)] = v;
+      if (out && m >= idx0 && m < end) out[m - idx0] = mt_temper(v);
+    }
+    __syncthreads();
+  }
+  if (gens > 0)
+    for (int i = threadIdx.x; i < 624; i += blockDim.x) g.mt[i] = ring[(624 * gens + i) & (A2_RING - 1)];
+  if (threadIdx.x == 0) g.idx = end - 624 * gens;
+  __syncthreads();
 }
 
 struct A2Args {
@@ -138,7 +121,9 @@
   double* vpart;
   double* upart;
   double* vmax;
+  unsigned long long* cvmax;
   double2* cand_xu;
+  double2* row_xu;
   double2* gbox;
   double2* cbox;
   int capmax;
@@ -149,6 +134,7 @@
   int work_cap;
   int* iter_ptr;
   int shard_rank, shard_count;
+  unsigned long long* clk;
   unsigned long long* stats;
 };
 enum {
@@ -163,6 +149,7 @@
 
 struct A2NodeSmem {
   MT19937 rng;
+  uint32_t ring[A2_RING];
   int k[A2_BMAX];
   int ol[A2_BMAX];
   int hkey[A2_HASH];
@@ -233,7 +220,17 @@
   return before + inc - v;
 }
 
-__device__ inline void a2_generate(const A2Args& a, A2State& st, A2NodeSmem& S, const A2Node& nd, int nid, int nb) {
+#ifdef BGP_ACA_CLOCKS
+#define A2_CLK(k) do { __syncthreads(); if (threadIdx.x == 0) clk[k] = clock64(); } while (0)
+#else
+#define A2_CLK(k) do { } while (0)
+#endif
+constexpr int A2_CLK_ROWS = 16, A2_CLK_STAMPS = 8;
+__device__ inline void a2_generate(const A2Args& a, A2State& st, A2NodeSmem& S, const A2Node& nd, int nid, int it) {
+  const int nb = (it + 1) & 1;
+#ifdef BGP_ACA_CLOCKS
+  unsigned long long clk[7] = {0, 0, 0, 0, 0, 0, 0};
+#endif
   int* __restrict__ index = a.idx_ws + nd.idx_off;
   int* __restrict__ cand = a.cand + nd.cand_off;
   int* __restrict__ cand_k = a.cand_k + nd.cand_off;
@@ -247,7 +244,9 @@
   MT19937* rng_commit = a.rngs + 2 * (int64_t)nid;
   MT19937* rng_end = rng_commit + 1;
   if (threadIdx.x == 0) { S.flag = 0x7fffffff; S.n_live = 0; S.extra = 0; }
-  mt_fill_coop(S.rng, S.raw, B);
+  A2_CLK(0);
+  mt_fill_coop(S.rng, S.ring, S.raw, B);
+  A2_CLK(1);
   int start = 0;
   bool truncated = false;
   while (true) {
@@ -299,11 +298,12 @@
     }
     {
       const int grown = S.extra - extra;
-      mt_fill_coop(S.rng, S.raw + B + extra, grown);
+      mt_fill_coop(S.rng, S.ring, S.raw + B + extra, grown);
     }
     start = c0 + 1;
   }
   __syncthreads();
+  A2_CLK(2);
   mt_copy(rng_end, &S.rng);
   if (threadIdx.x == 0) {
     st.ncand = B;
@@ -319,6 +319,7 @@
     S.hval[h] = (unsigned short)c;
   }
   __syncthreads();
+  A2_CLK(3);
   int* wl = reinterpret_cast<int*>(S.raw);
   for (int c = threadIdx.x; c < B; c += blockDim.x) wl[c] = a2_prev_writer(S, n_index - 1 - c, c);
   __syncthreads();
@@ -336,15 +337,14 @@
     cand_L[c] = last_value(c);
     cand_next[c] = a2_next_writer(S, pos, c);
   }
+  A2_CLK(4);
   const bool cull = a.vmax != nullptr;
-  const int rank = st.rank;
   if (!cull) {
     for (int c = threadIdx.x; c < B; c += blockDim.x) live[c] = c;
     if (threadIdx.x == 0) S.n_live = B;
   } else {
     const double clo = a.node_box[2 * nid], chi = a.node_box[2 * nid + 1];
-    const double* Ucol = nd.vbase + nd.row0;
-    const double* xr = a.x + nd.row0;
+    const double2* rxu = a.row_xu + (int64_t)nd.rchunk0 * A2_CHUNK;
     constexpr int G = 4;
     for (int t0 = 0; t0 < B; t0 += G * blockDim.x) {
       const int c0 = t0 + threadIdx.x;
@@ -353,16 +353,7 @@
 #pragma unroll
       for (int j = 0; j < G; ++j) { const int c = c0 + j * blockDim.x; row[j] = (c < B) ? cand[c] : 0; }
 #pragma unroll
-      for (int j = 0; j < G; ++j) xi[j] = xr[row[j]];
-#pragma unroll
-      for (int j = 0; j < G; ++j) b[j] = 0.0;
-      for (int q = 0; q < rank; ++q) {
-        double u[G];
-#pragma unroll
-        for (int j = 0; j < G; ++j) u[j] = __ldcg(Ucol + (int64_t)q * nd.ld + row[j]);
-#pragma unroll
-        for (int j = 0; j < G; ++j) b[j] += fabs(u[j]);
-      }
+      for (int j = 0; j < G; ++j) { const double2 xu = __ldcg(rxu + row[j]); xi[j] = xu.x; b[j] = xu.y; }
       unsigned keep = 0u;
 #pragma unroll
       for (int j = 0; j < G; ++j) {
@@ -388,6 +379,7 @@
     }
   }
   __syncthreads();
+  A2_CLK(5);
   {
     int n_live = S.n_live;
     const bool defer = (B == 1 && n_live == 1);
@@ -445,16 +437,9 @@
         for (int k = 0; k < R; ++k) {
           const int t = r0 + k * blockDim.x + threadIdx.x;
           if (t >= n_items) break;
-          const int4 w = item(t);
-          const int lc = w.x - nd.cchunk0, pi = w.y / ipc;
-          const double2 cb = __ldcg(a.cbox + w.x);
-          double vm = 0.0;
-          bool vnan = false;
-          for (int g = 0; g < A2_NGROUP && lc * A2_CHUNK + g * A2_GROUP < nd.n_cols; ++g) {
-            const double v = __ldcg(a.vmax + ((int64_t)w.x * A2_NGROUP + g));
-            vm = fmax(vm, v); vnan |= (v != v);
-          }
-          if (vnan) vm = __longlong_as_double(0x7ff8000000000000ll);
+          const int ch = item(t).x, pi = t % per_chunk;
+          const double2 cb = __ldcg(a.cbox + ch);
+          const double vm = __longlong_as_double((long long)__ldcg(a.cvmax + ch));
           const double lo = s_blo[pi], hi = s_bhi[pi];
           const double bb = program_bound(a.prog, fmax(0.0, fmax(cb.x - hi, lo - cb.y)), fmax(hi - cb.x, cb.y - lo)) + s_bu[pi] * vm;
           if (!(bb * 1.00001 < 1e-14)) keep |= 1u << k;
@@ -478,7 +463,16 @@
     }
   }
   __syncthreads();
-}
+#ifdef BGP_ACA_CLOCKS
+  A2_CLK(6);
+  if (threadIdx.x == 0 && a.clk) {
+    unsigned long long* row = a.clk + ((int64_t)((it + 1) % A2_CLK_ROWS) * a.n_nodes + nid) * A2_CLK_STAMPS;
+    for (int k = 0; k < 7; ++k) row[k] = clk[k];
+    row[7] = (unsigned long long)B;
+  }
+#endif
+}
+#undef A2_CLK
 
 __global__ void __launch_bounds__(A2_NODE_THREADS) a2_init_kernel(A2Args a) {
   extern __shared__ __align__(16) unsigned char a2_smem_raw[];
@@ -488,6 +482,9 @@
   A2State& st = a.states[nid];
   int* index = a.idx_ws + nd.idx_off;
   for (int n = threadIdx.x; n < nd.n_rows; n += blockDim.x) index[n] = n;
+  if (a.row_xu)
+    for (int n = threadIdx.x; n < nd.n_rows; n += blockDim.x)
+      a.row_xu[(int64_t)nd.rchunk0 * A2_CHUNK + n] = make_double2(a.x[nd.row0 + n], 0.0);
   if (threadIdx.x == 0) {
     mt_seed(S.rng, node_seed(a.seed, nd.pre_id));
     st.rank = 0; st.draws = 0; st.n_index = nd.n_rows; st.fallback = 0; st.status = 0; st.active = 1;
@@ -534,10 +531,18 @@
       }
       if (cnan) clo = chi = __longlong_as_double(0x7ff8000000000000ll);
       a.cbox[nd.cchunk0 + c] = make_double2(clo, chi);
-    }
-    __syncthreads();
-  }
-  a2_generate(a, st, S, nd, nid, 0);
+      double vm = 0.0;
+      bool vnan = false;
+      for (int g = 0; g < A2_NGROUP && c * A2_CHUNK + g * A2_GROUP < nd.n_cols; ++g) {
+        const double v = a.vmax[(int64_t)(nd.cchunk0 + c) * A2_NGROUP + g];
+        vm = fmax(vm, v); vnan |= (v != v);
+      }
+      if (vnan) vm = __longlong_as_double(0x7ff8000000000000ll);
+      a.cvmax[nd.cchunk0 + c] = (unsigned long long)__double_as_longlong(vm);
+    }
+    __syncthreads();
+  }
+  a2_generate(a, st, S, nd, nid, -1);
 }
 
 template <class KFn, bool CULL>
@@ -742,7 +747,7 @@
       if (threadIdx.x == 0) atomicAdd(a.stats + A2_PATH_PARTIAL, 1ull);
       mt_copy(&S.rng, rng_commit);
       __syncthreads();
-      mt_skip_coop(S.rng, w);
+      mt_fill_coop(S.rng, S.ring, nullptr, w);
     }
     if (threadIdx.x == 0) st.draws += w;
     __syncthreads();
@@ -780,7 +785,7 @@
   }
   __syncthreads();
   if (st.n_index == 0) return;
-  a2_generate(a, st, S, nd, nid, (*a.iter_ptr + 1) & 1);
+  a2_generate(a, st, S, nd, nid, *a.iter_ptr);
 }
 
 constexpr int A2_KU = 8;
@@ -895,11 +900,16 @@
     if (oi == 0x7fffffff) continue;
     if (a2_pivot_better(ov, oi, bval, bidx)) { bval = ov; bidx = oi; }
   }
+  bool late_reject = false;
   if (lane == 0) {
     st.piv_j = bidx; st.pivot = bval;
     if (a.vmax && !(fabs(bval) <= DBL_MAX)) a.node_box[2 * nid] = a.node_box[2 * nid + 1] = __longlong_as_double(0x7ff8000000000000ll);
-    if (st.deferred && fabs(bval) < 1e-14) st.phase = A2_LATE_REJECT;
-  }
+    late_reject = st.deferred && fabs(bval) < 1e-14;
+    if (late_reject) st.phase = A2_LATE_REJECT;
+  }
+  late_reject = __shfl_sync(0xffffffffu, late_reject, 0);
+  if (a.vmax && st.rank == 0 && !late_reject)
+    for (int c = lane; c < nd.n_cchunks; c += 32) a.cvmax[nd.cchunk0 + c] = 0ull;
 }
 
 __device__ __forceinline__ void a2_partial_dots(const double* __restrict__ pbase, int64_t ld, int rank, const double* s_vec,
@@ -963,6 +973,7 @@
     const double m = fmax(fmax(red[16 + 4 * g], red[17 + 4 * g]), fmax(red[18 + 4 * g], red[19 + 4 * g]));
     double* slot = a.vmax + ((int64_t)chunk * A2_NGROUP + sub * 2 + g);
     if (rank == 0 || m > *slot || m != m) *slot = m;
+    atomicMax(a.cvmax + chunk, (unsigned long long)__double_as_longlong(m));
   }
   double* part = a.vpart + ((int64_t)chunk * A2_NSUB + sub) * (a.capmax + 1);
   if (threadIdx.x == 0) part[0] = vn2;
@@ -1004,6 +1015,7 @@
   if (act) {
     Vcols[(int64_t)rank * nd.ld + nd.row0 + r_lo + n] = val;
     un2 = val * val;
+    if (a.row_xu) a.row_xu[(int64_t)nd.rchunk0 * A2_CHUNK + r_lo + n].y += fabs(val);
   }
   s_u[n] = act ? val : 0.0;
   un2 = block_sum(un2, red);
@@ -1042,7 +1054,7 @@
     if (st.phase == A2_DONE) return;
     mt_copy(&S.rng, a.rngs + 2 * (int64_t)nid);
     __syncthreads();
-    a2_generate(a, st, S, nd, nid, (*a.iter_ptr + 1) & 1);
+    a2_generate(a, st, S, nd, nid, *a.iter_ptr);
     return;
   }
   if (st.phase != A2_ACCEPT) return;
@@ -1095,7 +1107,19 @@
   }
   __syncthreads();
   if (s_done) return;
-  a2_generate(a, st, S, nd, nid, (*a.iter_ptr + 1) & 1);
+  a2_generate(a, st, S, nd, nid, *a.iter_ptr);
+}
+
+__global__ void __launch_bounds__(1024) a2_census_kernel(A2Args a, int* out) {
+  __shared__ int s_n, s_b;
+  if (threadIdx.x == 0) { s_n = 0; s_b = 0; }
+  __syncthreads();
+  for (int n = threadIdx.x; n < a.n_nodes; n += blockDim.x) {
+    const A2State& st = a.states[n];
+    if (st.active) { atomicAdd(&s_n, 1); atomicMax(&s_b, st.ncand); }
+  }
+  __syncthreads();
+  if (threadIdx.x == 0) { out[0] = s_n; out[1] = s_b; }
 }
 
 __global__ void a2_tick_kernel(int* iter_ptr, const int* n_active, cudaGraphConditionalHandle handle, int use_handle) {
diff --git a/george_b200/solvers/_hodlr.py b/george_b200/solvers/_hodlr.py
--- a/george_b200/solvers/_hodlr.py
+++ b/george_b200/solvers/_hodlr.py
@@ -199,7 +199,24 @@
         _lib.check(self._lib.bgp_hodlr_last_aca_profile(self._ptr, p))
         out = dict(zip(("eval_ms", "eval_launches", "evals", "update_fmas", "candidates", "evaluated"), list(p)[:6]))
         out["kernel_ms"] = dict(zip(("a2_eval", "a2_decide", "a2_vrow", "a2_pivot", "a2_vnorm_ucol", "a2_finish"), list(p)[6:]))
+        out["iterations"] = self._aca_iterations()
         return out
+
+    ACA_ITER_KERNELS = ("a2_eval", "a2_decide", "a2_vrow", "a2_pivot", "a2_vnorm_ucol", "a2_finish")
+    ACA_GENERATE_PHASES = ("rng_fill", "lemire", "multimap", "chains", "bound_live", "publish")
+
+    def _aca_iterations(self):
+        n = C.c_int32(0)
+        _lib.check(self._lib.bgp_hodlr_last_aca_iterations(self._ptr, 0, None, C.byref(n)))
+        cols = 15
+        buf = (C.c_double * max(1, n.value * cols))()
+        _lib.check(self._lib.bgp_hodlr_last_aca_iterations(self._ptr, n.value, buf, C.byref(n)))
+        rows = []
+        for i in range(n.value):
+            r = list(buf[i * cols:(i + 1) * cols])
+            rows.append({"kernel_ms": dict(zip(self.ACA_ITER_KERNELS, r[:6])), "active": int(r[6]), "max_batch": int(r[7]),
+                         "slowest_batch": int(r[8]), "generate_cycles": dict(zip(self.ACA_GENERATE_PHASES, r[9:15]))})
+        return rows
 
     def work(self):
         w = (C.c_double * 6)()
diff --git a/include/bgp.h b/include/bgp.h
--- a/include/bgp.h
+++ b/include/bgp.h
@@ -226,10 +226,13 @@
 int bgp_hodlr_last_work(const bgp_hodlr_t* h, double* w6);
 int bgp_hodlr_set_profiling(bgp_hodlr_t* h, int on);
 int bgp_hodlr_last_aca_profile(const bgp_hodlr_t* h, double* p12);
+#define BGP_ACA_ITER_COLS 15
+int bgp_hodlr_last_aca_iterations(const bgp_hodlr_t* h, int32_t cap, double* rows, int32_t* n_iters);
 
 int bgp_selftest_lu(int32_t n, int32_t nrhs, const double* S_host, double* R_host, double* logdet);
 int bgp_selftest_gemm(int32_t a_kcontig, int32_t b_kcontig, int32_t m, int32_t n, int32_t k, const double* A_host,
                       int64_t lda, const double* B_host, int64_t ldb, double* C_host, int64_t ldc, int32_t mode);
+int bgp_selftest_mt_fill(uint32_t seed, int32_t n_calls, const int32_t* lens, uint32_t* words, uint32_t* state);
 
 int bgp_hodlr_top_panel(bgp_hodlr_t* h, double** ptr_dev, int64_t* row0, int64_t* rows, int64_t* cols, int64_t* ld);
 int bgp_hodlr_export_top(bgp_hodlr_t* h, double* buf_dev, int64_t rows_pad);
```

Result: faster. 23.95 million (median of 6 runs) (+5.6%).
